# utiasASRL/mm_masking

Hardware: AMD Instinct MI355X
Metric: scan-pairs/s (mask-CNN + 10-iter dICP fwd+bwd) (higher is better)
Workload: dtype bf16; 1 GPU; BASELINE configs[2]: train_icp_weights step fwd+bwd, batch=32 per GPU, 10 dICP iters, point-to-plane Huber, dim=2; 400x3360 polar radar -> GO-CFAR + peaks + polar->Cartesian 640x640 -> U-Net (hand-written NHWC bf16 MFMA kernels, fp32 masters) -> dICP (fp32 points, fp64 normal equations) -> rot+trans+mask_pts loss -> Adam; batch_per_gpu=32, global_batch=32, scan_pts_pad=5120, map_pts=20000, map_pts_pad=20480, icp_iters=10, parallelism=dp1, scene_density=survey (SURVEY.md 8d: 3 500-5 000 valid scan points of 5 120)

## Files before the change

### include/mmk.h

```cpp
#ifndef MMK_H_
#define MMK_H_

#include <stddef.h>
#include <stdint.h>

#ifdef __cplusplus
extern "C" {
#endif

#define MMK_VERSION 502

#define MMK_OK 0
#define MMK_ERR_ARG (-1)
#define MMK_ERR_HIP (-2)
#define MMK_ERR_WORKSPACE (-3)

#define MMK_ICP_PT2PT 0
#define MMK_ICP_PT2PL 1

#define MMK_NN_BRUTE 0
#define MMK_NN_GRID 1

#define MMK_LOSS_NONE 0
#define MMK_LOSS_CAUCHY 1
// ... 36 lines not shown
                     void *workspace, size_t workspace_bytes, void *stream);

size_t mmk_icp_backward_points_workspace_bytes(const mmk_icp_params *p, int32_t with_target);
int mmk_icp_backward_points(const mmk_icp_params *p, const float *source, const float *target,
                            const float *weight, const int32_t *idx_hist, const float *T_hist,
                            const double *delta_hist, const double *A_hist,
                            const int32_t *active_hist, const float *grad_T ,
                            float *grad_weight , float *grad_T_init ,
                            float *grad_source , float *grad_target ,
                            void *workspace, size_t workspace_bytes, void *stream);

#define MMK_ICP_STATUS_UNARMED_KEY 1
int mmk_icp_status(const mmk_icp_params *p, const void *workspace, size_t workspace_bytes,
                   int32_t *status_out, void *stream);

size_t mmk_icp_partials_count(const mmk_icp_params *p);
int mmk_icp_accumulate(const mmk_icp_params *p, const float *source, const float *target,
                       const float *weight , const float *T ,
                       const uint64_t *nn_keys , int32_t *idx_out , double *partials,
                       int32_t *status , void *stream);
int mmk_icp_solve_update(const mmk_icp_params *p, const double *partials, const float *T_in ,
                         float *T_out , double *delta_out , double *A_out ,
                         const int32_t *active_in , int32_t *active_out , void *stream);

int32_t mmk_nn_padded_m(int32_t M);
int mmk_pack_target(const float *target , int32_t B, int32_t M,
                    int32_t tgt_cols, int32_t dim, float *target_planar, void *stream);
size_t mmk_nn_workspace_bytes(int32_t B, int32_t N, int32_t M, int32_t dim);
int mmk_nn_search(const float *source , const float *target_planar,
                  const float *T , int32_t B, int32_t N, int32_t M, int32_t dim,
                  int32_t *idx, float *d2, void *workspace, size_t workspace_bytes,
                  void *stream);

int mmk_nn_profile_begin(int32_t capacity);
int mmk_nn_profile_end(float *ms_out , int32_t max_out, int32_t *n_out );

int mmk_pose_loss_fwd(const float *T_pred , int32_t B, float *out2, void *stream);
int mmk_pose_loss_bwd(const float *T_pred, int32_t B, const float *g_rot, const float *g_trans,
                      float *grad_T , void *stream);
size_t mmk_bce_ws_bytes(void);
int mmk_bce_mean_fwd(const float *x, const float *target, int64_t n, void *ws, size_t ws_bytes,
                     float *out, void *stream);
int mmk_bce_mean_bwd(const float *x, const float *target, int64_t n, const float *grad_out,
                     float *grad_x, void *stream);

int mmk_pose_loss_gt_fwd(const float *T_pred , const float *T_gt , int32_t B, float *out2, void *stream);
int mmk_pose_loss_gt_bwd(const float *T_pred, const float *T_gt, int32_t B, const float *g_rot, const float *g_trans,
                         float *grad_T , void *stream);
int mmk_val_metric(const float *T_pred , const float *T_gt , int32_t B, float *out3, void *stream);
size_t mmk_fft_threshold_ws_bytes(int32_t B);
int mmk_fft_threshold_mask(const float *fft, int32_t B, int64_t hw, void *ws, size_t ws_bytes, float *mask_out,
                           void *stream);
int mmk_bce_fft_threshold_fwd(const float *x, const float *fft, int32_t B, int64_t hw, void *ws, size_t ws_bytes,
                              float *thr_out , float *out, void *stream);
int mmk_bce_fft_threshold_bwd(const float *x, const float *fft, int32_t B, int64_t hw, const float *thr ,
                              const float *grad_out, float *grad_x, void *stream);


int mmk_cfar_mask(const float *raw, int32_t B, int32_t A, int32_t R, int32_t w2,
                  int32_t guard, int32_t mincol, int32_t maxcol, float a_thresh,
                  float b_thresh, int32_t diff, float steep_fact, float *mask,
                  void *stream);

int mmk_cfar_mask_bwd(const float *raw, const float *grad_mask , int32_t B, int32_t A, int32_t R, int32_t w2,
                      int32_t guard, int32_t mincol, int32_t maxcol, float a_thresh, float b_thresh, float steep_fact,
                      float *grad_raw , void *stream);

int mmk_cfar_mask_p(const float *raw, int32_t B, int32_t A, int32_t R, int32_t w2, int32_t guard, int32_t mincol,
                    int32_t maxcol, const float *a_thresh, const float *b_thresh, int32_t per_scan, int32_t diff,
                    float steep_fact, float *mask, void *stream);

size_t mmk_cfar_mask_bwd_p_ws_bytes(int32_t B, int32_t A);
int mmk_cfar_mask_bwd_p(const float *raw, const float *grad_mask , int32_t B, int32_t A, int32_t R, int32_t w2,
                        int32_t guard, int32_t mincol, int32_t maxcol, const float *a_thresh, const float *b_thresh,
                        int32_t per_scan, float steep_fact, float *grad_raw , float *grad_a,
                        float *grad_b , void *workspace, size_t workspace_bytes, void *stream);

size_t mmk_extract_peaks_workspace_bytes(int32_t B, int32_t A, int32_t R, int32_t max_pts);
int mmk_extract_peaks(const float *mask, int32_t B, int32_t A, int32_t R, float res,
                      const float *azimuths , const float *times ,
                      const float *T_ab, int32_t diff, float steep_fact, int32_t max_pts,
                      float *out_pc, int32_t *out_count, void *workspace,
                      size_t workspace_bytes, void *stream);
size_t mmk_extract_peaks_bwd_workspace_bytes(int32_t B, int32_t A, int32_t R, int32_t max_pts);
int mmk_extract_peaks_bwd(const float *mask, int32_t B, int32_t A, int32_t R, float res, const float *azimuths ,
                          const float *T_ab, int32_t diff, float steep_fact, int32_t max_pts,
                          const float *grad_pc , float *grad_mask , void *workspace,
                          size_t workspace_bytes, void *stream);

int mmk_polar_to_cart(const float *polar, const float *azimuths ,
                      const float *range_grid, const float *angle_grid, int32_t B,
                      int32_t A, int32_t R, int32_t W, float radar_resolution,
                      int32_t interpolate_crossover, int32_t fix_wobble, float *cart,
                      void *stream);
int mmk_polar_to_cart_pair(const float *polar, const float *polar2, const float *azimuths,
                           const float *range_grid, const float *angle_grid, int32_t B, int32_t A,
                           int32_t R, int32_t W, float radar_resolution, int32_t interpolate_crossover,
                           int32_t fix_wobble, float *cart, float *cart2, void *stream);

int mmk_cart_to_polar(const double *cart, const double *sin_az, const double *cos_az, const double *range_coords,
                      int32_t B, int32_t A, int32_t R, int32_t H, int32_t W, double cart_resolution, double *polar,
                      void *stream);

size_t mmk_polar_to_cart_bwd_ws_bytes(int32_t B, int32_t A, int32_t R, int32_t W);
int mmk_polar_to_cart_bwd(const float *grad_cart , const float *azimuths , const float *range_grid,
                          const float *angle_grid, int32_t B, int32_t A, int32_t R, int32_t W, float radar_resolution,
                          int32_t interpolate_crossover, int32_t fix_wobble, float *grad_polar , void *ws,
                          size_t ws_bytes, void *stream);

size_t mmk_cart_to_polar_bwd_ws_bytes(int32_t B, int32_t A, int32_t R, int32_t H, int32_t W);
int mmk_cart_to_polar_bwd(const double *grad_polar , const double *sin_az, const double *cos_az,
                          const double *range_coords, int32_t B, int32_t A, int32_t R, int32_t H, int32_t W,
                          double radar_resolution, double cart_resolution, double *grad_cart , void *ws,
                          size_t ws_bytes, void *stream);

int mmk_mask_polar_scan(const float *scan , const float *mask_cart , const double *sin_az,
                        const double *cos_az, const double *range_coords, int32_t B, int32_t A, int32_t R, int32_t H,
                        int32_t W, double cart_resolution, float *out , void *stream);

size_t mmk_mask_polar_scan_bwd_ws_bytes(int32_t B, int32_t A, int32_t R, int32_t H, int32_t W);
int mmk_mask_polar_scan_bwd(const float *grad_out , const float *scan , const float *mask_cart ,
                            const double *sin_az, const double *cos_az, const double *range_coords, int32_t B, int32_t A,
                            int32_t R, int32_t H, int32_t W, double radar_resolution, double cart_resolution,
                            float *grad_scan , float *grad_mask , void *ws, size_t ws_bytes,
                            void *stream);

int mmk_sample_weights_fwd(const float *mask , const float *pc ,
                           int32_t B, int32_t N, int32_t pc_cols, int32_t H, int32_t W,
                           int32_t cart_pixel_width, float cart_resolution,
                           float *weights , void *stream);
size_t mmk_sample_weights_bwd_ws_bytes(int32_t B, int32_t N);
int mmk_sample_weights_bwd(const float *grad_weights , const float *pc, int32_t B,
                           int32_t N, int32_t pc_cols, int32_t H, int32_t W,
                           int32_t cart_pixel_width, float cart_resolution, float *grad_mask,
                           void *ws, size_t ws_bytes, void *stream);
int mmk_sample_weights_bwd_pc(const float *grad_weights , const float *mask , const float *pc,
                              int32_t B, int32_t N, int32_t pc_cols, int32_t H, int32_t W,
                              int32_t cart_pixel_width, float cart_resolution, float *grad_pc, void *stream);

int mmk_host_read_rows(const char *path, int64_t header_bytes, int32_t rows, int32_t row_bytes, int32_t col0,
                       int32_t ncols, int32_t roll, void *dst);
typedef struct mmk_read_job {
    const char *path;
    int64_t header_bytes;
    int32_t rows, row_bytes, col0, ncols, roll, reserved;
    void *dst;
} mmk_read_job;
int mmk_host_read_rows_batch(const mmk_read_job *jobs, int32_t n_jobs, int32_t threads);
int mmk_u8_to_float(const void *in , const float *lut256, int64_t n, float *out, void *stream);

int mmk_weight_stats(const float *weights , const float *pc , int32_t B, int32_t N,
                     int32_t pc_cols, float *partial, float *out, void *stream);

int mmk_bev_raster(const float *pc , int32_t B, int32_t M, int32_t pc_cols,
                   int32_t W, float cart_resolution, float *bev , void *stream);

typedef struct {
    const void *x1;
    const void *x2;
    int32_t C1, C2;
    const void *wpack;
    const float *bias;
    void *y1;
    const void *relu_src1;
    int32_t O1, accumulate1;
    float scale1;
// ... 121 lines not shown
```

### mm_masking_amd/_lib.py

```python
import ctypes
import os
import sys
import subprocess

import torch

_HERE = os.path.dirname(os.path.abspath(__file__))
_ROOT = os.path.dirname(_HERE)
SO_PATH = os.environ.get("MMK_LIB", os.path.join(_HERE, "libmmk_hip.so"))
SOURCES = ["mmk_api.hip", "mmk_icp.hip", "mmk_radar.hip", "mmk_unet.hip", "mmk_unet_driver.hip", "mmk_loader.hip", "mmk_loss.hip"]

_lib = None

c_f32p = ctypes.c_void_p
c_vp = ctypes.c_void_p


class MmkError(RuntimeError):
    pass


class ReadJob(ctypes.Structure):
    _fields_ = [("path", ctypes.c_char_p), ("header_bytes", ctypes.c_int64), ("rows", ctypes.c_int32),
                ("row_bytes", ctypes.c_int32), ("col0", ctypes.c_int32), ("ncols", ctypes.c_int32), ("roll", ctypes.c_int32),
# ... 79 lines not shown
    P = ctypes.POINTER(IcpParams)
    sig = {
        "mmk_version": (ctypes.c_int, []),
        "mmk_last_error": (ctypes.c_char_p, []),
        "mmk_icp_workspace_bytes": (sz, [P]),
        "mmk_icp_forward": (ctypes.c_int, [P] + [c_vp] * 10 + [c_vp, sz, ctypes.POINTER(ctypes.c_int), c_vp]),
        "mmk_icp_backward": (ctypes.c_int, [P] + [c_vp] * 11 + [c_vp, sz, c_vp]),
        "mmk_icp_backward_points_workspace_bytes": (sz, [P, i32]),
        "mmk_icp_backward_points": (ctypes.c_int, [P] + [c_vp] * 13 + [c_vp, sz, c_vp]),
        "mmk_icp_status": (ctypes.c_int, [P, c_vp, sz, c_vp, c_vp]),
        "mmk_pose_loss_fwd": (ctypes.c_int, [c_vp, i32, c_vp, c_vp]),
        "mmk_pose_loss_bwd": (ctypes.c_int, [c_vp, i32, c_vp, c_vp, c_vp, c_vp]),
        "mmk_bce_ws_bytes": (sz, []),
        "mmk_bce_mean_fwd": (ctypes.c_int, [c_vp, c_vp, ctypes.c_int64, c_vp, sz, c_vp, c_vp]),
        "mmk_bce_mean_bwd": (ctypes.c_int, [c_vp, c_vp, ctypes.c_int64, c_vp, c_vp, c_vp]),
        "mmk_pose_loss_gt_fwd": (ctypes.c_int, [c_vp, c_vp, i32, c_vp, c_vp]),
        "mmk_pose_loss_gt_bwd": (ctypes.c_int, [c_vp, c_vp, i32, c_vp, c_vp, c_vp, c_vp]),
        "mmk_val_metric": (ctypes.c_int, [c_vp, c_vp, i32, c_vp, c_vp]),
        "mmk_fft_threshold_ws_bytes": (sz, [i32]),
        "mmk_fft_threshold_mask": (ctypes.c_int, [c_vp, i32, ctypes.c_int64, c_vp, sz, c_vp, c_vp]),
        "mmk_bce_fft_threshold_fwd": (ctypes.c_int, [c_vp, c_vp, i32, ctypes.c_int64, c_vp, sz, c_vp, c_vp, c_vp]),
        "mmk_bce_fft_threshold_bwd": (ctypes.c_int, [c_vp, c_vp, i32, ctypes.c_int64, c_vp, c_vp, c_vp, c_vp]),
        "mmk_icp_partials_count": (sz, [P]),
        "mmk_icp_accumulate": (ctypes.c_int, [P] + [c_vp] * 8 + [c_vp]),
        "mmk_icp_solve_update": (ctypes.c_int, [P] + [c_vp] * 7 + [c_vp]),
        "mmk_nn_padded_m": (i32, [i32]),
        "mmk_pack_target": (ctypes.c_int, [c_vp, i32, i32, i32, i32, c_vp, c_vp]),
        "mmk_nn_workspace_bytes": (sz, [i32, i32, i32, i32]),
        "mmk_nn_search": (ctypes.c_int, [c_vp, c_vp, c_vp, i32, i32, i32, i32, c_vp, c_vp, c_vp, sz, c_vp]),
        "mmk_nn_profile_begin": (ctypes.c_int, [i32]),
        "mmk_nn_profile_end": (ctypes.c_int, [ctypes.POINTER(ctypes.c_float), i32, ctypes.POINTER(ctypes.c_int32)]),
        "mmk_conv3x3_packed_elems": (sz, [i32, i32, i32]),
        "mmk_conv3x3_pack_weights": (ctypes.c_int, [c_vp, i32, i32, i32, c_vp, c_vp]),
        "mmk_conv3x3_pack_weights_batch": (ctypes.c_int, [i32, c_vp, c_vp, c_vp, i32, c_vp, c_vp]),
        "mmk_conv3x3": (ctypes.c_int, [ctypes.POINTER(ConvDesc), c_vp]),
        "mmk_conv3x3_wgrad_unpack_batch": (ctypes.c_int, [i32, c_vp, c_vp, c_vp, c_vp, c_vp, c_vp, c_vp]),
        "mmk_conv3x3_wgrad_slices": (i32, [i32, i32, i32, i32, i32, i32]),
        "mmk_conv3x3_wgrad_partial": (ctypes.c_int, [c_vp, c_vp, i32, i32, c_vp, i32, i32, i32, i32, c_vp, i32, c_vp]),
        "mmk_conv_bwd_fused": (ctypes.c_int, [c_vp, c_vp, c_vp, ctypes.c_float, i32, i32, i32, i32, c_vp, c_vp, i32, c_vp]),
        "mmk_conv8x16_bwd_fused": (ctypes.c_int, [c_vp, c_vp, c_vp, ctypes.c_float, i32, i32, i32, c_vp, c_vp, i32, c_vp]),
        "mmk_conv16x8_bwd_fused": (ctypes.c_int, [c_vp, c_vp, c_vp, c_vp, ctypes.c_float, i32, i32, i32, c_vp, c_vp, c_vp, i32, c_vp]),
        "mmk_conv3x3_pool_fusable": (ctypes.c_int32, [i32, i32, i32, i32, i32]),
        "mmk_channel_minmax": (ctypes.c_int, [c_vp, i32, i32, ctypes.c_int64, c_vp, c_vp, c_vp, c_vp]),
        "mmk_channel_meanstd": (ctypes.c_int, [c_vp, i32, i32, ctypes.c_int64, c_vp, c_vp, c_vp]),
        "mmk_conv_first": (ctypes.c_int, [c_vp, i32, c_vp, c_vp, c_vp, i32, i32, i32, f32, c_vp, c_vp]),
        "mmk_conv_first_wgrad_ws_bytes": (sz, [i32]),
        "mmk_conv_first_wgrad": (ctypes.c_int, [c_vp, i32, c_vp, c_vp, i32, i32, i32, c_vp, c_vp, c_vp, sz, c_vp]),
        "mmk_conv_first_dgrad_ws_bytes": (sz, [i32]),
        "mmk_conv_first_dgrad": (ctypes.c_int, [c_vp, i32, c_vp, c_vp, c_vp, c_vp, i32, i32, i32, c_vp, c_vp, sz, c_vp]),
        "mmk_input_norm_bwd": (ctypes.c_int, [c_vp, c_vp, i32, c_vp, c_vp, i32, i32, i32, i32, c_vp, sz, c_vp]),
        "mmk_maxpool2_fwd": (ctypes.c_int, [c_vp, i32, i32, i32, i32, c_vp, c_vp]),
        "mmk_maxpool2_bwd": (ctypes.c_int, [c_vp, c_vp, i32, i32, i32, i32, f32, f32, c_vp, c_vp]),
        "mmk_maxpool2_fwd_arg": (ctypes.c_int, [c_vp, i32, i32, i32, i32, c_vp, c_vp, c_vp]),
        "mmk_maxpool2_bwd_arg": (ctypes.c_int, [c_vp, c_vp, i32, i32, i32, i32, f32, c_vp, c_vp]),
        "mmk_upsample_fwd": (ctypes.c_int, [c_vp, i32, i32, i32, i32, i32, i32, c_vp, c_vp]),
        "mmk_upsample_bwd": (ctypes.c_int, [c_vp, i32, i32, i32, i32, i32, i32, c_vp, f32, f32, c_vp, c_vp]),
        "mmk_final_fwd": (ctypes.c_int, [c_vp, c_vp, c_vp, ctypes.c_int64, c_vp, c_vp]),
        "mmk_final_bwd": (ctypes.c_int, [c_vp, c_vp, c_vp, c_vp, ctypes.c_int64, f32, f32, c_vp, c_vp, c_vp, c_vp, c_vp]),
        "mmk_mask_normalize": (ctypes.c_int, [c_vp, i32, ctypes.c_int64, c_vp, c_vp, c_vp, c_vp]),
        "mmk_final_bwd_normalized": (ctypes.c_int, [c_vp, c_vp, c_vp, c_vp, c_vp, c_vp, i32, ctypes.c_int64, f32, f32, c_vp, c_vp,
                                                    c_vp, c_vp, c_vp, c_vp, c_vp]),
        "mmk_bn_forward_stats": (ctypes.c_int, [c_vp, ctypes.c_int64, i32, c_vp, c_vp, f32, f32, c_vp, c_vp, c_vp, c_vp, c_vp, c_vp]),
        "mmk_bn_apply": (ctypes.c_int, [c_vp, ctypes.c_int64, i32, c_vp, f32, ctypes.c_uint32, c_vp, c_vp]),
        "mmk_bn_backward": (ctypes.c_int, [c_vp, c_vp, f32, c_vp, ctypes.c_int64, i32, c_vp, c_vp, c_vp, f32, i32, c_vp, c_vp, c_vp,
                                           c_vp, c_vp, c_vp]),
        "mmk_unet_workspace_bytes": (sz, [i32, i32, i32, i32]),
        "mmk_unet_scratch_bytes": (sz, [i32, i32, i32, i32]),
        "mmk_unet_forward": (ctypes.c_int, [ctypes.POINTER(UNetDesc), c_vp]),
        "mmk_unet_backward": (ctypes.c_int, [ctypes.POINTER(UNetDesc), c_vp, ctypes.POINTER(ctypes.c_void_p), c_vp, sz, c_vp]),
        "mmk_unet_backward_buckets": (ctypes.c_int, [ctypes.POINTER(UNetDesc), c_vp, ctypes.POINTER(ctypes.c_void_p), c_vp, sz,
                                                     ctypes.POINTER(ctypes.c_void_p), c_vp]),
        "mmk_unet_backward_input": (ctypes.c_int, [ctypes.POINTER(UNetDesc), c_vp, ctypes.POINTER(ctypes.c_void_p), c_vp, i32, c_vp,
                                                   c_vp, sz, ctypes.POINTER(ctypes.c_void_p), c_vp]),
        "mmk_unet_grad_bucket": (i32, [i32, ctypes.POINTER(i32), ctypes.POINTER(i32)]),
        "mmk_unet_tensor": (ctypes.c_int, [i32, i32, i32, i32, i32, ctypes.POINTER(sz), ctypes.POINTER(i32), ctypes.POINTER(i32),
                                           ctypes.POINTER(i32)]),
        "mmk_cfar_mask": (ctypes.c_int, [c_vp, i32, i32, i32, i32, i32, i32, i32, f32, f32, i32, f32, c_vp, c_vp]),
        "mmk_cfar_mask_bwd": (ctypes.c_int, [c_vp, c_vp, i32, i32, i32, i32, i32, i32, i32, f32, f32, f32, c_vp, c_vp]),
        "mmk_cfar_mask_p": (ctypes.c_int, [c_vp, i32, i32, i32, i32, i32, i32, i32, c_vp, c_vp, i32, i32, f32, c_vp, c_vp]),
        "mmk_cfar_mask_bwd_p_ws_bytes": (sz, [i32, i32]),
        "mmk_cfar_mask_bwd_p": (ctypes.c_int, [c_vp, c_vp, i32, i32, i32, i32, i32, i32, i32, c_vp, c_vp, i32, f32, c_vp, c_vp, c_vp,
                                               c_vp, sz, c_vp]),
        "mmk_extract_peaks_workspace_bytes": (sz, [i32, i32, i32, i32]),
        "mmk_extract_peaks_bwd_workspace_bytes": (sz, [i32, i32, i32, i32]),
        "mmk_extract_peaks_bwd": (ctypes.c_int, [c_vp, i32, i32, i32, f32, c_vp, c_vp, i32, f32, i32, c_vp, c_vp, c_vp, sz, c_vp]),
        "mmk_extract_peaks": (ctypes.c_int, [c_vp, i32, i32, i32, f32, c_vp, c_vp, c_vp, i32, f32, i32, c_vp, c_vp,
                                             c_vp, sz, c_vp]),
        "mmk_polar_to_cart": (ctypes.c_int, [c_vp, c_vp, c_vp, c_vp, i32, i32, i32, i32, f32, i32, i32, c_vp, c_vp]),
        "mmk_polar_to_cart_pair": (ctypes.c_int, [c_vp, c_vp, c_vp, c_vp, c_vp, i32, i32, i32, i32, f32, i32, i32, c_vp, c_vp,
                                                  c_vp]),
        "mmk_cart_to_polar": (ctypes.c_int, [c_vp, c_vp, c_vp, c_vp, i32, i32, i32, i32, i32, ctypes.c_double, c_vp, c_vp]),
        "mmk_polar_to_cart_bwd_ws_bytes": (sz, [i32, i32, i32, i32]),
        "mmk_polar_to_cart_bwd": (ctypes.c_int, [c_vp, c_vp, c_vp, c_vp, i32, i32, i32, i32, f32, i32, i32, c_vp, c_vp, sz, c_vp]),
        "mmk_cart_to_polar_bwd_ws_bytes": (sz, [i32, i32, i32, i32, i32]),
        "mmk_cart_to_polar_bwd": (ctypes.c_int, [c_vp, c_vp, c_vp, c_vp, i32, i32, i32, i32, i32, ctypes.c_double, ctypes.c_double,
                                                 c_vp, c_vp, sz, c_vp]),
        "mmk_mask_polar_scan": (ctypes.c_int, [c_vp, c_vp, c_vp, c_vp, c_vp, i32, i32, i32, i32, i32, ctypes.c_double, c_vp, c_vp]),
        "mmk_mask_polar_scan_bwd_ws_bytes": (sz, [i32, i32, i32, i32, i32]),
        "mmk_mask_polar_scan_bwd": (ctypes.c_int, [c_vp, c_vp, c_vp, c_vp, c_vp, c_vp, i32, i32, i32, i32, i32, ctypes.c_double,
                                                   ctypes.c_double, c_vp, c_vp, c_vp, sz, c_vp]),
        "mmk_sample_weights_fwd": (ctypes.c_int, [c_vp, c_vp, i32, i32, i32, i32, i32, i32, f32, c_vp, c_vp]),
        "mmk_host_read_rows": (ctypes.c_int, [ctypes.c_char_p, ctypes.c_int64, i32, i32, i32, i32, i32, c_vp]),
        "mmk_host_read_rows_batch": (ctypes.c_int, [ctypes.POINTER(ReadJob), i32, i32]),
        "mmk_u8_to_float": (ctypes.c_int, [c_vp, c_vp, ctypes.c_int64, c_vp, c_vp]),
        "mmk_sample_weights_bwd_ws_bytes": (sz, [i32, i32]),
        "mmk_sample_weights_bwd": (ctypes.c_int, [c_vp, c_vp, i32, i32, i32, i32, i32, i32, f32, c_vp, c_vp, sz, c_vp]),
        "mmk_sample_weights_bwd_pc": (ctypes.c_int, [c_vp, c_vp, c_vp, i32, i32, i32, i32, i32, i32, f32, c_vp, c_vp]),
        "mmk_weight_stats": (ctypes.c_int, [c_vp, c_vp, i32, i32, i32, c_vp, c_vp, c_vp]),
        "mmk_bev_raster": (ctypes.c_int, [c_vp, i32, i32, i32, i32, f32, c_vp, c_vp]),
    }
    for name, (res, args) in sig.items():
        fn = getattr(lib, name)
        fn.restype = res
        fn.argtypes = args
    return sig


EXPORTED = None


def lib():
    global _lib, EXPORTED
    if _lib is None:
        if not os.path.exists(SO_PATH):
            raise MmkError("libmmk_hip.so is not built: run `python -c 'import __graft_entry__ as g; g.build()'` "
                           "(hipcc --offload-arch=gfx950).  The HIP path has no CPU fallback.")
        try:
            loaded = ctypes.CDLL(SO_PATH)
        except OSError as e:
            raise MmkError("cannot load %s: %s" % (SO_PATH, e)) from e
        EXPORTED = _declare(loaded)
        _lib = loaded
    return _lib


def check(rc):
    if rc != 0:
        raise MmkError("libmmk_hip: %s (code %d)" % (lib().mmk_last_error().decode(errors="replace"), rc))


def stream_ptr(device=None):
    if device is not None:
        idx = device.index if isinstance(device, torch.device) else int(device)
        if idx is not None and idx != torch.cuda.current_device():
            raise MmkError("tensors live on cuda:%d but the current HIP device is cuda:%d: call torch.cuda.set_device() "
                           "(one process per GPU) or wrap the call in `with torch.cuda.device(...)`"
                           % (idx, torch.cuda.current_device()))
    return ctypes.c_void_p(torch.cuda.current_stream(device).cuda_stream)


def ptr(t, dtype=None, name="tensor"):
    if t is None:
        return ctypes.c_void_p(0)
    if not t.is_cuda:
        raise MmkError("%s must live on a HIP device (got %s); the kernels have no CPU path" % (name, t.device))
    if dtype is not None and t.dtype != dtype:
        raise MmkError("%s must be %s (got %s)" % (name, dtype, t.dtype))
    if not t.is_contiguous():
        raise MmkError("%s must be contiguous" % name)
    return ctypes.c_void_p(t.data_ptr())


def dev_f32(t, device):
    return t.detach().to(device=device, dtype=torch.float32).contiguous()
```

### mm_masking_amd/csrc/mmk_icp.hip

```cpp
#include <math.h>
#include <stdio.h>
#include <stdlib.h>

#include <algorithm>

#include "mmk_common.h"

namespace {

constexpr int NN_THREADS = 256;
constexpr int NN_TILE = 1024;
constexpr float NN_PAD = 3.0e18f;
constexpr int ACC_THREADS = 256;
constexpr int PART_ROWS = 32;

__host__ __device__ constexpr int nacc(int dim) { return dim == 2 ? 9 : 27; }
__host__ __device__ constexpr int npose(int dim) { return dim == 2 ? 6 : 12; }

template <int DIM>
__device__ __forceinline__ void transform_point(const float *T, const float s[3], float p[DIM])
{
    if constexpr (DIM == 2) {
        p[0] = (T[0] * s[0] + T[1] * s[1]) + T[3];
        p[1] = (T[4] * s[0] + T[5] * s[1]) + T[7];
    } else {
        p[0] = ((T[0] * s[0] + T[1] * s[1]) + T[2] * s[2]) + T[3];
        p[1] = ((T[4] * s[0] + T[5] * s[1]) + T[6] * s[2]) + T[7];
        p[2] = ((T[8] * s[0] + T[9] * s[1]) + T[10] * s[2]) + T[11];
    }
}

template <int DIM>
__device__ __forceinline__ float nn_dist(float tx, float ty, float tz, const float p[DIM])
{
    float dx = tx - p[0];
    float dy = ty - p[1];
    float d = __builtin_fmaf(dy, dy, dx * dx);
    if constexpr (DIM == 3) {
        float dz = tz - p[2];
        d = __builtin_fmaf(dz, dz, d);
    }
    return d;
}

__global__ void pack_target_kernel(const float *__restrict__ tgt, int M, int cols, int dim, int Mpad,
                                   float *__restrict__ out, float *__restrict__ dec, int dec_stride)
{
    int j = blockIdx.x * blockDim.x + threadIdx.x;
    int b = blockIdx.y;
    if (j >= Mpad) return;
    for (int c = 0; c < dim; ++c) {
        float v = NN_PAD;
        if (j < M) v = tgt[((size_t)b * M + j) * cols + c];
        out[((size_t)b * dim + c) * Mpad + j] = v;
        if (dec != nullptr && j % dec_stride == 0) dec[((size_t)b * dim + c) * (Mpad / dec_stride) + j / dec_stride] = v;
    }
}

constexpr int PF_CH = 32;

__global__ __launch_bounds__(NN_THREADS) void src_zero_scan_kernel(const float *__restrict__ src, int N, int pts, int nsb,
                                                                  int32_t *__restrict__ allzero, int32_t *__restrict__ zrep)
{
    const int sb = blockIdx.x, b = blockIdx.y;
    int first = N;
    int nonzero = 0;
    for (int q = threadIdx.x; q < pts; q += blockDim.x) {
        const int i = sb * pts + q;
        if (i < N) {
            const float *sp = src + ((size_t)b * N + i) * 3;
            const bool z = sp[0] == 0.f && sp[1] == 0.f && sp[2] == 0.f;
            nonzero |= z ? 0 : 1;
            if (z && i < first) first = i;
        }
    }
    const int any = __syncthreads_or(nonzero);
#pragma unroll
    for (int off = 32; off > 0; off >>= 1) first = min(first, __shfl_down(first, off, 64));
    if ((threadIdx.x & 63) == 0 && first < N) atomicMin(&zrep[b], first);
    if (threadIdx.x == 0) allzero[(size_t)b * nsb + sb] = any ? 0 : 1;
}

__global__ void src_units_kernel(const int32_t *__restrict__ allzero, const int32_t *__restrict__ zrep, int B, int nsb, int pts,
                                 int cap, int32_t *__restrict__ ulist, int32_t *__restrict__ ucnt)
{
    const int c = threadIdx.x;
    int n = 0;
// ... 540 lines not shown
template <int DIM, int TYPE>
struct PointTerms {
    static constexpr int P = (DIM == 2) ? 3 : 6;
    static constexpr int NR = (TYPE == MMK_ICP_PT2PT) ? DIM : 1;
    float s[3];
    float p[DIM];
    float ev[DIM];
    float n[DIM];
    float J[NR][P];
    float er[NR];
    float d2, r2, keep, rho, w, omega;
};

template <int DIM, int TYPE>
__device__ __forceinline__ void point_terms(PointTerms<DIM, TYPE> &t, const float *T, const float *srow,
                                            const float *trow, float omega, int loss, float k, float k2,
                                            float trim2)
{
    constexpr int P = PointTerms<DIM, TYPE>::P;
    constexpr int NR = PointTerms<DIM, TYPE>::NR;
    t.s[0] = srow[0];
    t.s[1] = srow[1];
    t.s[2] = srow[2];
    transform_point<DIM>(T, t.s, t.p);
#pragma unroll
    for (int c = 0; c < DIM; ++c) t.ev[c] = trow[c] - t.p[c];
    float d2 = t.ev[0] * t.ev[0] + t.ev[1] * t.ev[1];
    if constexpr (DIM == 3) d2 = d2 + t.ev[2] * t.ev[2];
    t.d2 = d2;
    t.keep = (d2 < trim2) ? 1.f : 0.f;
    if (TYPE == MMK_ICP_PT2PL) {
#pragma unroll
        for (int c = 0; c < DIM; ++c) t.n[c] = trow[3 + c];
        float e = t.n[0] * t.ev[0] + t.n[1] * t.ev[1];
        if constexpr (DIM == 3) e = e + t.n[2] * t.ev[2];
        t.er[0] = e;
        t.r2 = e * e;
        if (DIM == 2) {
            t.J[0][0] = t.n[0];
            t.J[0][1] = t.n[1];
            t.J[0][2] = t.n[1] * t.p[0] - t.n[0] * t.p[1];
        } else {
            t.J[0][0] = t.n[0];
            t.J[0][1] = t.n[1];
            t.J[0][2] = t.n[DIM - 1];
            t.J[0][P - 3] = t.p[1] * t.n[DIM - 1] - t.p[DIM - 1] * t.n[1];
            t.J[0][P - 2] = t.p[DIM - 1] * t.n[0] - t.p[0] * t.n[DIM - 1];
            t.J[0][P - 1] = t.p[0] * t.n[1] - t.p[1] * t.n[0];
        }
    } else {
        t.r2 = d2;
#pragma unroll
        for (int r = 0; r < NR; ++r) {
            t.er[r] = t.ev[r];
#pragma unroll
            for (int c = 0; c < P; ++c) t.J[r][c] = 0.f;
            t.J[r][r] = 1.f;
        }
        if (DIM == 2) {
            t.J[0][2] = -t.p[1];
            t.J[NR - 1][2] = t.p[0];
        } else {
            const float px = t.p[0], py = t.p[1], pz = t.p[DIM - 1];
            t.J[0][P - 2] = pz;
            t.J[0][P - 1] = -py;
            t.J[1 % NR][P - 3] = -pz;
            t.J[1 % NR][P - 1] = px;
            t.J[2 % NR][P - 3] = py;
            t.J[2 % NR][P - 2] = -px;
        }
    }
    float rho = 1.f;
    if (loss == MMK_LOSS_CAUCHY) {
        rho = 1.0f / (1.0f + t.r2 / k2);
    } else if (loss == MMK_LOSS_HUBER) {
        const float r = sqrtf(t.r2);
        rho = (r <= k) ? 1.f : k / r;
    }
    t.rho = rho;
    t.omega = omega;
    t.w = (omega * t.keep) * rho;
}

template <int DIM, int TYPE>
__global__ __launch_bounds__(ACC_THREADS) void icp_accumulate_kernel(
    const float *__restrict__ src, const float *__restrict__ tgt, int tgt_cols,
    const float *__restrict__ weight, const float *__restrict__ Tk, const int32_t *__restrict__ active,
    const unsigned long long *__restrict__ packed, unsigned long long *__restrict__ packed_next,
    const int32_t *__restrict__ allzero, const int32_t *__restrict__ zrep, int nn_pts, int nn_nsb,
    int32_t *__restrict__ idx_out, int N, int M, int loss, float k,
    float k2, float trim2, double *__restrict__ partials, int32_t *__restrict__ status)
{
    constexpr int P = PointTerms<DIM, TYPE>::P;
    constexpr int NR = PointTerms<DIM, TYPE>::NR;
    constexpr int NACC = nacc(DIM);
    const int b = blockIdx.y;
    if (active != nullptr && active[b] == 0) return;
    const int i = blockIdx.x * ACC_THREADS + threadIdx.x;
    double acc[NACC];
#pragma unroll
    for (int a = 0; a < NACC; ++a) acc[a] = 0.0;

    if (i < N) {
        float T[16];
#pragma unroll
        for (int q = 0; q < 16; ++q) T[q] = Tk[(size_t)b * 16 + q];
        int isrc = i;
        if (allzero != nullptr && allzero[(size_t)b * nn_nsb + i / nn_pts] != 0 && zrep[b] < (i / nn_pts) * nn_pts) isrc = zrep[b];
        const unsigned long long key = packed[(size_t)b * N + isrc];
        if (packed_next != nullptr) packed_next[(size_t)b * N + i] = NN_KEY_INIT;
        const unsigned jraw = (unsigned)(key & 0xffffffffull);
        if ((key == NN_KEY_INIT || jraw >= (unsigned)M) && status != nullptr) atomicOr(status, (int32_t)MMK_ICP_STATUS_UNARMED_KEY);
        const int j = (int)min(jraw, (unsigned)(M - 1));
        idx_out[(size_t)b * N + i] = j;
        const float omega = weight ? weight[(size_t)b * N + i] : 1.f;
        PointTerms<DIM, TYPE> t;
        point_terms<DIM, TYPE>(t, T, src + ((size_t)b * N + i) * 3, tgt + ((size_t)b * M + j) * tgt_cols, omega,
                               loss, k, k2, trim2);
        int a = 0;
#pragma unroll
        for (int m = 0; m < P; ++m) {
#pragma unroll
            for (int n = m; n < P; ++n) {
                double v = 0.0;
#pragma unroll
                for (int r = 0; r < NR; ++r) v += (double)(t.w * t.J[r][m]) * (double)t.J[r][n];
                acc[a++] = v;
            }
        }
#pragma unroll
        for (int m = 0; m < P; ++m) {
            double v = 0.0;
#pragma unroll
            for (int r = 0; r < NR; ++r) v += (double)(t.w * t.J[r][m]) * (double)t.er[r];
            acc[a++] = v;
        }
    }

    __shared__ double red[ACC_THREADS / 64][NACC];
    const int lane = threadIdx.x & 63, wv = threadIdx.x >> 6;
#pragma unroll
    for (int a = 0; a < NACC; ++a) {
        double v = wave_sum(acc[a]);
        if (lane == 0) red[wv][a] = v;
    }
    __syncthreads();
    if (threadIdx.x < NACC) {
        double v = 0.0;
#pragma unroll
        for (int w = 0; w < ACC_THREADS / 64; ++w) v += red[w][threadIdx.x];
        partials[((size_t)b * gridDim.x + blockIdx.x) * NACC + threadIdx.x] = v;
    }
}

template <int P>
__device__ bool chol_solve(const double *A , const double *rhs, double *x, double *ws)
{
    double (*L)[P] = reinterpret_cast<double (*)[P]>(ws);
    double *y = ws + P * P;
    bool ok = true;
    for (int i = 0; i < P; ++i)
        for (int j = 0; j < P; ++j) {
            L[i][j] = 0.0;
            if (!isfinite(A[i * P + j])) ok = false;
        }
    for (int j = 0; j < P && ok; ++j) {
        double d = A[j * P + j];
        for (int q = 0; q < j; ++q) d -= L[j][q] * L[j][q];
        if (!(d > 0.0)) {
            ok = false;
            break;
        }
        d = sqrt(d);
        L[j][j] = d;
        for (int i = j + 1; i < P; ++i) {
            double v = A[i * P + j];
            for (int q = 0; q < j; ++q) v -= L[i][q] * L[j][q];
            L[i][j] = v / d;
        }
    }
    if (!ok) {
        for (int i = 0; i < P; ++i) x[i] = 0.0;
        return false;
    }
    for (int i = 0; i < P; ++i) {
        double v = rhs[i];
        for (int q = 0; q < i; ++q) v -= L[i][q] * y[q];
        y[i] = v / L[i][i];
    }
    for (int i = P - 1; i >= 0; --i) {
        double v = y[i];
        for (int q = i + 1; q < P; ++q) v -= L[q][i] * x[q];
        x[i] = v / L[i][i];
    }
    return true;
}

template <int DIM>
__device__ void se_exp(const double *dl, double E[16])
{
    for (int i = 0; i < 16; ++i) E[i] = 0.0;
    E[0] = E[5] = E[10] = E[15] = 1.0;
    if (DIM == 2) {
        const double x = dl[0], y = dl[1], th = dl[2];
        const double th2 = th * th;
        double a, bb;
        if (th2 < 1e-8) {
            a = 1.0 - th2 / 6.0 + th2 * th2 / 120.0;
            bb = th * (0.5 - th2 / 24.0 + th2 * th2 / 720.0);
        } else {
            a = sin(th) / th;
            bb = (1.0 - cos(th)) / th;
        }
        const double c = cos(th), s = sin(th);
        E[0] = c; E[1] = -s; E[3] = a * x - bb * y;
        E[4] = s; E[5] = c;  E[7] = bb * x + a * y;
    } else {
        const double *rho = dl, *phi = dl + 3;
        const double th2 = phi[0] * phi[0] + phi[1] * phi[1] + phi[2] * phi[2];
        double A_, B_, C_;
        if (th2 < 1e-8) {
            A_ = 1.0 - th2 / 6.0 + th2 * th2 / 120.0;
            B_ = 0.5 - th2 / 24.0 + th2 * th2 / 720.0;
            C_ = 1.0 / 6.0 - th2 / 120.0 + th2 * th2 / 5040.0;
        } else {
            const double th = sqrt(th2);
            A_ = sin(th) / th;
            B_ = (1.0 - cos(th)) / th2;
            C_ = (th - sin(th)) / (th2 * th);
        }
        const double K[9] = {0.0, -phi[2], phi[1], phi[2], 0.0, -phi[0], -phi[1], phi[0], 0.0};
        double K2[9];
        for (int i = 0; i < 3; ++i)
            for (int j = 0; j < 3; ++j) {
                double v = 0.0;
                for (int q = 0; q < 3; ++q) v += K[i * 3 + q] * K[q * 3 + j];
                K2[i * 3 + j] = v;
            }
        for (int i = 0; i < 3; ++i) {
            double tv = 0.0;
            for (int j = 0; j < 3; ++j) {
                const double id = (i == j) ? 1.0 : 0.0;
                E[i * 4 + j] = id + A_ * K[i * 3 + j] + B_ * K2[i * 3 + j];
                tv += (id + B_ * K[i * 3 + j] + C_ * K2[i * 3 + j]) * rho[j];
            }
            E[i * 4 + 3] = tv;
        }
    }
}

template <int DIM>
__global__ __launch_bounds__(64) void icp_solve_kernel(const double *__restrict__ partials, int nblk,
                                                       const float *__restrict__ T_in, float *__restrict__ T_out,
                                                       double *__restrict__ delta_out, double *__restrict__ A_out,
                                                       const int32_t *__restrict__ active_in,
                                                       int32_t *__restrict__ active_out, float tol)
{
    constexpr int P = (DIM == 2) ? 3 : 6;
    constexpr int NACC = nacc(DIM);
    const int b = blockIdx.x;
    const int lane = threadIdx.x;
    __shared__ double acc[NACC];
    __shared__ double stage[PART_ROWS * NACC];
    const bool act = active_in[b] != 0;
    {
        double v = 0.0;
        if (act) {
            const double *base = partials + (size_t)b * nblk * NACC;
            for (int r0 = 0; r0 < nblk; r0 += PART_ROWS) {
                const int nr = min(PART_ROWS, nblk - r0);
                for (int e = lane; e < nr * NACC; e += 64) stage[e] = base[(size_t)r0 * NACC + e];
                __syncthreads();
                if (lane < NACC)
                    for (int q = 0; q < nr; ++q) v += stage[q * NACC + lane];
                __syncthreads();
            }
        }
        if (lane < NACC) acc[lane] = v;
    }
    __syncthreads();
    if (lane != 0) return;
    __shared__ double A[P * P], rhs[P], dl[6], E[16], ws[P * P + P];
    for (int q = 0; q < 6; ++q) dl[q] = 0.0;
    int a = 0;
    for (int m = 0; m < P; ++m)
        for (int n = m; n < P; ++n) {
            A[m * P + n] = acc[a];
            A[n * P + m] = acc[a];
            ++a;
        }
    for (int m = 0; m < P; ++m) rhs[m] = acc[a++];
    for (int q = 0; q < 36; ++q) A_out[(size_t)b * 36 + q] = (q < P * P) ? A[q] : 0.0;
    if (act) chol_solve<P>(A, rhs, dl, ws);
    for (int q = 0; q < 6; ++q) delta_out[(size_t)b * 6 + q] = dl[q];
    if (!act) {
        for (int q = 0; q < 16; ++q) T_out[(size_t)b * 16 + q] = T_in[(size_t)b * 16 + q];
        active_out[b] = 0;
        return;
    }
    se_exp<DIM>(dl, E);
    for (int i = 0; i < 4; ++i)
        for (int j = 0; j < 4; ++j) {
            double v = 0.0;
            for (int q = 0; q < 4; ++q) v += E[i * 4 + q] * (double)T_in[(size_t)b * 16 + q * 4 + j];
            T_out[(size_t)b * 16 + i * 4 + j] = (float)v;
        }
    double nrm = 0.0;
    for (int q = 0; q < P; ++q) nrm += dl[q] * dl[q];
    active_out[b] = (sqrt(nrm) < (double)tol) ? 0 : 1;
}

__global__ __launch_bounds__(256) void icp_init_kernel(unsigned long long *__restrict__ keys, size_t nkeys, int32_t *__restrict__ status,
                                                       int32_t *__restrict__ active0, const float *__restrict__ T_init,
                                                       float *__restrict__ T0, int32_t *__restrict__ zrep, int B, int N)
{
    const size_t i0 = (size_t)blockIdx.x * blockDim.x + threadIdx.x, stride = (size_t)gridDim.x * blockDim.x;
    for (size_t i = i0; i < nkeys; i += stride) keys[i] = ~0ull;
    if (i0 < 16) status[i0] = 0;
    if (i0 < (size_t)B) {
        active0[i0] = 1;
        if (zrep != nullptr) zrep[i0] = N;
    }
    if (i0 < (size_t)B * 16) T0[i0] = T_init[i0];
}

__global__ void fill_i32_kernel(int32_t *p, int n, int32_t v)
{
    int i = blockIdx.x * blockDim.x + threadIdx.x;
    if (i < n) p[i] = v;
}

template <int DIM>
__global__ __launch_bounds__(64) void icp_bwd_pair_kernel(
    const double *__restrict__ Gdir_in, const double *__restrict__ pparts, int nparts,
    const float *__restrict__ Tk, const double *__restrict__ delta, const double *__restrict__ Amat,
    const int32_t *__restrict__ active, double *__restrict__ Gdir_out, double *__restrict__ lam_out)
{
    constexpr int P = (DIM == 2) ? 3 : 6;
    constexpr int NP = npose(DIM);
    const int b = blockIdx.x;
    const int lane = threadIdx.x;
    __shared__ double G[16], Eb[16], X[16], M0[64], R0[64], R1[64];
    __shared__ double stage[PART_ROWS * NP];

    {
        double v = (lane < 16) ? Gdir_in[(size_t)b * 16 + lane] : 0.0;
        const int r = lane >> 2, c = lane & 3;
        int slot = -1;
        if (lane < 16 && r < DIM && c < DIM) slot = r * DIM + c;
        if (lane < 16 && r < DIM && c == 3) slot = DIM * DIM + r;
        const double *base = pparts + (size_t)b * nparts * NP;
        for (int r0 = 0; r0 < nparts; r0 += PART_ROWS) {
            const int nr = min(PART_ROWS, nparts - r0);
            for (int e = lane; e < nr * NP; e += 64) stage[e] = base[(size_t)r0 * NP + e];
            __syncthreads();
            if (slot >= 0)
                for (int q = 0; q < nr; ++q) v += stage[q * NP + slot];
            __syncthreads();
        }
        if (lane < 16) G[lane] = v;
    }
    __syncthreads();
    const bool act = (active != nullptr) && active[b] != 0;
    if (!act) {
        if (lane < 16) Gdir_out[(size_t)b * 16 + lane] = G[lane];
        if (lane < 6 && lam_out) lam_out[(size_t)b * 6 + lane] = 0.0;
        return;
    }
    const double *dl = delta + (size_t)b * 6;
    if (lane < 16) {
        const int r = lane >> 2, c = lane & 3;
        double v = 0.0;
        for (int q = 0; q < 4; ++q) v += G[r * 4 + q] * (double)Tk[(size_t)b * 16 + c * 4 + q];
        Eb[lane] = v;
        double x = 0.0;
        if (DIM == 2) {
            if (r == 0 && c == 3) x = dl[0];
            if (r == 1 && c == 3) x = dl[1];
            if (r == 1 && c == 0) x = dl[2];
            if (r == 0 && c == 1) x = -dl[2];
        } else {
            if (c == 3 && r < 3) x = dl[r];
            if (r == 2 && c == 1) x = dl[3];
            if (r == 1 && c == 2) x = -dl[3];
            if (r == 0 && c == 2) x = dl[4];
            if (r == 2 && c == 0) x = -dl[4];
            if (r == 1 && c == 0) x = dl[5];
            if (r == 0 && c == 1) x = -dl[5];
        }
        X[lane] = x;
    }
    __syncthreads();
    const int i8 = lane >> 3, j8 = lane & 7;
    {
        double m = 0.0;
        const double sc = 1.0 / 64.0;
        if (i8 < 4 && j8 < 4) m = X[j8 * 4 + i8] * sc;
        else if (i8 >= 4 && j8 >= 4) m = X[(j8 - 4) * 4 + (i8 - 4)] * sc;
        else if (i8 < 4 && j8 >= 4) m = Eb[i8 * 4 + (j8 - 4)] * sc;
        M0[lane] = m;
        R0[lane] = ((i8 == j8) ? 1.0 : 0.0) + m / 13.0;
    }
    __syncthreads();
    double *cur = R0, *nxt = R1;
    for (int n = 12; n >= 1; --n) {
        double v = 0.0;
#pragma unroll
        for (int q = 0; q < 8; ++q) v += M0[i8 * 8 + q] * cur[q * 8 + j8];
        nxt[lane] = ((i8 == j8) ? 1.0 : 0.0) + v / (double)n;
        __syncthreads();
        double *t = cur; cur = nxt; nxt = t;
    }
    for (int sq = 0; sq < 6; ++sq) {
        double v = 0.0;
#pragma unroll
        for (int q = 0; q < 8; ++q) v += cur[i8 * 8 + q] * cur[q * 8 + j8];
        nxt[lane] = v;
        __syncthreads();
        double *t = cur; cur = nxt; nxt = t;
    }
    if (lane < 16) {
        const int r = lane >> 2, c = lane & 3;
        double v = 0.0;
        for (int q = 0; q < 4; ++q) v += cur[r * 8 + q] * G[q * 4 + c];
        Gdir_out[(size_t)b * 16 + lane] = v;
    }
    if (lane == 0) {
        auto xb = [&](int r, int c) { return cur[r * 8 + 4 + c]; };
        __shared__ double db[P], A[P * P], lam[P], ws[P * P + P];
        if (DIM == 2) {
            db[0] = xb(0, 3);
            db[1] = xb(1, 3);
            db[2] = xb(1, 0) - xb(0, 1);
        } else {
            db[0] = xb(0, 3);
            db[1] = xb(1, 3);
            db[2] = xb(2, 3);
            db[P - 3] = xb(2, 1) - xb(1, 2);
            db[P - 2] = xb(0, 2) - xb(2, 0);
            db[P - 1] = xb(1, 0) - xb(0, 1);
        }
        for (int q = 0; q < P * P; ++q) A[q] = Amat[(size_t)b * 36 + q];
        chol_solve<P>(A, db, lam, ws);
        for (int q = 0; q < 6; ++q) lam_out[(size_t)b * 6 + q] = (q < P) ? lam[q] : 0.0;
    }
}

__host__ __device__ constexpr int tgt_row_cols(int dim, int type) { return type == MMK_ICP_PT2PL ? 2 * dim : dim; }
__host__ __device__ constexpr int tgt_acc_cols(int c) { return c <= 2 ? 2 : (c <= 4 ? 4 : 8); }

template <int DIM, int TYPE, bool PTS>
__global__ __launch_bounds__(ACC_THREADS) void icp_bwd_point_kernel(
    const float *__restrict__ src, const float *__restrict__ tgt, int tgt_cols,
    const float *__restrict__ weight, const float *__restrict__ Tk, const int32_t *__restrict__ active,
    const int32_t *__restrict__ idx, const double *__restrict__ lam64, const double *__restrict__ delta64, int N,
    int M, int loss, float k, float k2, float trim2, float *__restrict__ gw, double *__restrict__ pparts,
    float *__restrict__ gsrc, float *__restrict__ rows, unsigned *__restrict__ pmax)
{
    constexpr int P = PointTerms<DIM, TYPE>::P;
    constexpr int NR = PointTerms<DIM, TYPE>::NR;
    constexpr int NP = npose(DIM);
    constexpr int C = tgt_row_cols(DIM, TYPE);
    const int b = blockIdx.y;
    const int i = blockIdx.x * ACC_THREADS + threadIdx.x;
    double acc[NP];
#pragma unroll
    for (int a = 0; a < NP; ++a) acc[a] = 0.0;
    const bool act = active[b] != 0;
    unsigned mbits = 0u;

    if (act && i < N) {
        float T[16];
#pragma unroll
        for (int q = 0; q < 16; ++q) T[q] = Tk[(size_t)b * 16 + q];
        float lam[P], dl[P];
#pragma unroll
        for (int q = 0; q < P; ++q) {
            lam[q] = (float)lam64[(size_t)b * 6 + q];
            dl[q] = (float)delta64[(size_t)b * 6 + q];
        }
        const int j = idx[(size_t)b * N + i];
        const float omega = weight ? weight[(size_t)b * N + i] : 1.f;
        PointTerms<DIM, TYPE> t;
        point_terms<DIM, TYPE>(t, T, src + ((size_t)b * N + i) * 3, tgt + ((size_t)b * M + j) * tgt_cols, omega,
                               loss, k, k2, trim2);
        float wbar = 0.f;
        float ebar[NR];
        float Jbar[NR][P];
#pragma unroll
        for (int r = 0; r < NR; ++r) {
            float u = 0.f, v = 0.f;
#pragma unroll
            for (int c = 0; c < P; ++c) {
                u += t.J[r][c] * lam[c];
                v += t.J[r][c] * dl[c];
            }
            const float res = t.er[r] - v;
            wbar += u * res;
            ebar[r] = t.w * u;
#pragma unroll
            for (int c = 0; c < P; ++c) Jbar[r][c] = t.w * (res * lam[c] - u * dl[c]);
        }
        const float gomega = wbar * t.keep * t.rho;
        const float rhobar = wbar * t.omega * t.keep;
        float r2bar = 0.f;
        if (loss == MMK_LOSS_CAUCHY) {
            r2bar = rhobar * (-(t.rho * t.rho) / k2);
        } else if (loss == MMK_LOSS_HUBER) {
            if (sqrtf(t.r2) > k) r2bar = rhobar * (-t.rho / (2.f * t.r2));
        }
#pragma unroll
        for (int r = 0; r < NR; ++r) ebar[r] += 2.f * t.er[r] * r2bar;
        gw[(size_t)b * N + i] += gomega;

        float pbar[DIM];
#pragma unroll
        for (int c = 0; c < DIM; ++c) pbar[c] = 0.f;
        if (TYPE == MMK_ICP_PT2PT) {
#pragma unroll
            for (int c = 0; c < DIM; ++c) pbar[c] -= ebar[c % NR];
            if (DIM == 2) {
                pbar[1] -= Jbar[0][2];
                pbar[0] += Jbar[NR - 1][2];
            } else {
                pbar[DIM - 1] += Jbar[0][P - 2];
                pbar[1] -= Jbar[0][P - 1];
                pbar[DIM - 1] -= Jbar[1 % NR][P - 3];
                pbar[0] += Jbar[1 % NR][P - 1];
                pbar[1] += Jbar[2 % NR][P - 3];
                pbar[0] -= Jbar[2 % NR][P - 2];
            }
        } else {
#pragma unroll
            for (int c = 0; c < DIM; ++c) pbar[c] -= t.n[c] * ebar[0];
            if (DIM == 2) {
                pbar[0] += t.n[1] * Jbar[0][2];
                pbar[1] -= t.n[0] * Jbar[0][2];
            } else {
                const float nx = t.n[0], ny = t.n[1], nz = t.n[DIM - 1];
                const float j3 = Jbar[0][P - 3], j4 = Jbar[0][P - 2], j5 = Jbar[0][P - 1];
                pbar[0] += -nz * j4 + ny * j5;
                pbar[1] += nz * j3 - nx * j5;
                pbar[DIM - 1] += -ny * j3 + nx * j4;
            }
        }
#pragma unroll
        for (int r = 0; r < DIM; ++r) {
#pragma unroll
            for (int c = 0; c < DIM; ++c) acc[r * DIM + c] = (double)pbar[r] * (double)t.s[c];
            acc[DIM * DIM + r] = (double)pbar[r];
        }
        if constexpr (PTS) {
            if (gsrc != nullptr) {
                float *gs = gsrc + ((size_t)b * N + i) * 3;
#pragma unroll
                for (int c = 0; c < DIM; ++c) {
                    float v = T[c] * pbar[0];
#pragma unroll
                    for (int r = 1; r < DIM; ++r) v += T[r * 4 + c] * pbar[r];
                    gs[c] += v;
                }
            }
            if (rows != nullptr) {
                float q[C];
                if constexpr (TYPE == MMK_ICP_PT2PT) {
#pragma unroll
                    for (int c = 0; c < DIM; ++c) q[c] = ebar[c];
                } else {
                    const float eb = ebar[0];
#pragma unroll
                    for (int c = 0; c < DIM; ++c) {
                        q[c] = t.n[c] * eb;
                        q[DIM + c] = eb * t.ev[c] + Jbar[0][c];
                    }
                    if constexpr (DIM == 2) {
                        q[DIM + 0] -= t.p[1] * Jbar[0][2];
                        q[DIM + 1] += t.p[0] * Jbar[0][2];
                    } else {
                        const float px = t.p[0], py = t.p[1], pz = t.p[DIM - 1];
                        const float j3 = Jbar[0][P - 3], j4 = Jbar[0][P - 2], j5 = Jbar[0][P - 1];
                        q[DIM + 0] += j4 * pz - j5 * py;
                        q[DIM + 1] += j5 * px - j3 * pz;
                        q[DIM + DIM - 1] += j3 * py - j4 * px;
                    }
                }
                float *row = rows + ((size_t)b * N + i) * C;
#pragma unroll
                for (int c = 0; c < C; ++c) {
                    row[c] = q[c];
                    mbits = max(mbits, __float_as_uint(fabsf(q[c])));
                }
            }
        }
    }

    __shared__ double red[ACC_THREADS / 64][NP];
    __shared__ unsigned wmax[ACC_THREADS / 64];
    const int lane = threadIdx.x & 63, wv = threadIdx.x >> 6;
    if constexpr (PTS) {
#pragma unroll
        for (int off = 32; off > 0; off >>= 1) mbits = max(mbits, __shfl_xor(mbits, off, 64));
        if (lane == 0) wmax[wv] = mbits;
    }
#pragma unroll
    for (int a = 0; a < NP; ++a) {
        double v = wave_sum(acc[a]);
        if (lane == 0) red[wv][a] = v;
    }
    __syncthreads();
    if constexpr (PTS) {
        if (rows != nullptr && threadIdx.x == 0) {
            unsigned m = 0u;
#pragma unroll
            for (int w = 0; w < ACC_THREADS / 64; ++w) m = max(m, wmax[w]);
            if (m != 0u) atomicMax(&pmax[b], m);
        }
    }
    if (threadIdx.x < NP) {
        double v = 0.0;
#pragma unroll
        for (int w = 0; w < ACC_THREADS / 64; ++w) v += red[w][threadIdx.x];
        pparts[((size_t)b * gridDim.x + blockIdx.x) * NP + threadIdx.x] = v;
    }
}

__global__ void f32_to_f64_kernel(const float *in, double *out, int n)
{
    int i = blockIdx.x * blockDim.x + threadIdx.x;
    if (i < n) out[i] = (double)in[i];
}

template <int DIM>
__global__ void bwd_final_kernel(const double *__restrict__ Gdir, const double *__restrict__ pparts, int nparts,
                                 float *__restrict__ out)
{
    constexpr int NP = npose(DIM);
    __shared__ double stage[PART_ROWS * NP];
    const int b = blockIdx.x, lane = threadIdx.x;
    double v = (lane < 16) ? Gdir[(size_t)b * 16 + lane] : 0.0;
    const int r = lane >> 2, c = lane & 3;
    int slot = -1;
    if (lane < 16 && r < DIM && c < DIM) slot = r * DIM + c;
    if (lane < 16 && r < DIM && c == 3) slot = DIM * DIM + r;
    const double *base = pparts + (size_t)b * nparts * NP;
    for (int r0 = 0; r0 < nparts; r0 += PART_ROWS) {
        const int nr = min(PART_ROWS, nparts - r0);
        for (int e = lane; e < nr * NP; e += blockDim.x) stage[e] = base[(size_t)r0 * NP + e];
        __syncthreads();
        if (slot >= 0)
            for (int q = 0; q < nr; ++q) v += stage[q * NP + slot];
        __syncthreads();
    }
    if (lane < 16) out[(size_t)b * 16 + lane] = (float)v;
}

__device__ __forceinline__ double tgt_fixed_scale(unsigned mbits, int cnt_bits)
{
    if (mbits >= 0x7f800000u) return 0.0;
    if (mbits == 0u) return 1.0;
    return ldexp(1.0, 62 - cnt_bits - ((int)(mbits >> 23) - 126));
}

template <int C>
__global__ __launch_bounds__(ACC_THREADS) void icp_bwd_target_scatter_kernel(
    const float *__restrict__ rows, const int32_t *__restrict__ idx_hist, const int32_t *__restrict__ active_hist,
    const unsigned *__restrict__ pmax, int B, int N, int M, int cnt_bits, unsigned long long *__restrict__ acc)
{
    constexpr int L = tgt_acc_cols(C);
    const int b = blockIdx.y, k = blockIdx.z;
    const double scale = tgt_fixed_scale(pmax[b], cnt_bits);
    if (active_hist[(size_t)k * B + b] == 0 || scale == 0.0) return;
    const int t = blockIdx.x * ACC_THREADS + threadIdx.x, i = t / L, c = t % L;
    const bool valid = i < N;
    const size_t r = ((size_t)k * B + b) * N + i;
    const int j = valid ? idx_hist[r] : -1;
    long long v = 0;
    if (valid && c < C) v = llrint((double)rows[r * C + c] * scale);
    const unsigned long long vmask = __ballot(valid);
    if (vmask == 0ull) return;
    unsigned long long *ab = acc + (size_t)b * M * L;
    const int j0 = __shfl(j, __ffsll(vmask) - 1, 64);
    if (__ballot(valid && j != j0) == 0ull) {
#pragma unroll
        for (int off = 32; off >= L; off >>= 1) v += __shfl_xor(v, off, 64);
        if ((threadIdx.x & 63) < L && v != 0) atomicAdd(&ab[(size_t)j0 * L + c], (unsigned long long)v);
    } else if (v != 0) {
        atomicAdd(&ab[(size_t)j * L + c], (unsigned long long)v);
    }
}

__global__ void icp_bwd_target_final_kernel(const unsigned long long *__restrict__ acc, const unsigned *__restrict__ pmax,
                                            int cnt_bits, int M, int dim, int C, int L, int cols, float *__restrict__ gtgt)
{
    const int j = blockIdx.x * blockDim.x + threadIdx.x, b = blockIdx.y;
    if (j >= M) return;
    const double scale = tgt_fixed_scale(pmax[b], cnt_bits);
    const unsigned long long *a = acc + ((size_t)b * M + j) * L;
    float *out = gtgt + ((size_t)b * M + j) * cols;
    for (int c = 0; c < cols; ++c) {
        const int e = c < dim ? c : (C > dim && c >= 3 && c < 3 + dim ? dim + (c - 3) : -1);
        float v = 0.f;
        if (e >= 0) v = scale == 0.0 ? __builtin_nanf("") : (float)((double)(long long)a[e] / scale);
        out[c] = v;
    }
}

struct NNPlan {
    int Mpad, ntiles, nsb, ntu, tiles_per_unit, total_units, grid, P, ucap;
};


NNPlan nn_plan(int B, int N, int M, int dim)
{
    NNPlan pl;
    pl.P = 2;
    pl.Mpad = (int)mmk::align_up((size_t)M, NN_TILE);
    pl.ntiles = pl.Mpad / NN_TILE;
    pl.nsb = (N + NN_THREADS * pl.P - 1) / (NN_THREADS * pl.P);
    pl.tiles_per_unit = std::min(4, pl.ntiles);
    pl.ntu = (pl.ntiles + pl.tiles_per_unit - 1) / pl.tiles_per_unit;
    const int Bpad = (B + 7) / 8 * 8;
    pl.total_units = Bpad * pl.nsb * pl.ntu;
    pl.ucap = (Bpad / 8) * pl.nsb;
    pl.grid = std::min(pl.total_units, dim == 2 ? 1024 : 768);
    return pl;
}

struct NNProf {
    bool on = false;
    int cap = 0, n = 0;
    hipEvent_t *ev = nullptr;
};
thread_local NNProf g_prof;

int launch_nn(int dim, const float *src, const float *tgtp, const float *Tk, const int32_t *active,
              const int32_t *prev_idx, const int32_t *ulist, const int32_t *ucnt, int B, int N, const NNPlan &pl,
              unsigned long long *packed, int32_t *seed_buf, const int32_t *allzero, const int32_t *zrep, const float *dec,
              hipStream_t st)
{
    const bool rec = g_prof.on && g_prof.n < g_prof.cap;
    if (rec) MMK_CHECK_HIP(hipEventRecord(g_prof.ev[2 * g_prof.n], st));
    if (prev_idx == nullptr && seed_buf != nullptr && pl.Mpad >= 4 * NN_COARSE_STRIDE) {
        const dim3 grid((N + NN_COARSE_THREADS - 1) / NN_COARSE_THREADS, B);
        const int nn_pts = NN_THREADS * pl.P;
        if (dim == 2)
            hipLaunchKernelGGL(nn_coarse_seed_kernel<2>, grid, dim3(NN_COARSE_THREADS), 0, st, src, tgtp, Tk, active, allzero, zrep, nn_pts, pl.nsb, N,
                               pl.Mpad, dec, seed_buf);
        else
            hipLaunchKernelGGL(nn_coarse_seed_kernel<3>, grid, dim3(NN_COARSE_THREADS), 0, st, src, tgtp, Tk, active, allzero, zrep, nn_pts, pl.nsb, N,
                               pl.Mpad, dec, seed_buf);
        MMK_LAUNCH_CHECK();
        prev_idx = seed_buf;
    }
    constexpr float U = 5.9604645e-8f;
    if (dim == 2) {
        hipLaunchKernelGGL((nn_mfma_kernel<2>), dim3(pl.grid), dim3(NN_THREADS), 0, st, src, tgtp, Tk, active, prev_idx, ulist, ucnt,
                           pl.ucap, B, N, pl.Mpad, pl.nsb, pl.ntu, pl.tiles_per_unit, pl.total_units, 360.0f * U, packed);
    } else {
        hipLaunchKernelGGL((nn_mfma_kernel<3>), dim3(pl.grid), dim3(NN_THREADS), 0, st, src, tgtp, Tk, active, prev_idx, ulist, ucnt,
                           pl.ucap, B, N, pl.Mpad, pl.nsb, pl.ntu, pl.tiles_per_unit, pl.total_units, 496.0f * U, packed);
    }
    MMK_LAUNCH_CHECK();
    if (rec) {
        MMK_CHECK_HIP(hipEventRecord(g_prof.ev[2 * g_prof.n + 1], st));
        g_prof.n++;
    }
    return MMK_OK;
}

int check_params(const mmk_icp_params *p)
{
    MMK_REQUIRE(p != nullptr, "mmk_icp: params is NULL");
    MMK_REQUIRE(p->B >= 1 && p->N >= 1 && p->M >= 1, "mmk_icp: B, N, M must be >= 1 (got %d, %d, %d)", p->B, p->N, p->M);
    MMK_REQUIRE(p->dim == 2 || p->dim == 3, "mmk_icp: dim must be 2 or 3 (got %d)", p->dim);
    MMK_REQUIRE(p->tgt_cols == 3 || p->tgt_cols == 6, "mmk_icp: target must have 3 or 6 columns (got %d)", p->tgt_cols);
    MMK_REQUIRE(p->icp_type == MMK_ICP_PT2PT || p->icp_type == MMK_ICP_PT2PL, "mmk_icp: bad icp_type %d", p->icp_type);
    MMK_REQUIRE(p->icp_type != MMK_ICP_PT2PL || p->tgt_cols == 6, "mmk_icp: pt2pl needs target normals (B,M,6)");
    MMK_REQUIRE(p->loss >= MMK_LOSS_NONE && p->loss <= MMK_LOSS_HUBER, "mmk_icp: bad loss %d", p->loss);
    MMK_REQUIRE(p->max_iter >= 1, "mmk_icp: max_iter must be >= 1");
    MMK_REQUIRE(p->loss == MMK_LOSS_NONE || p->loss_k > 0.f, "mmk_icp: loss metric must be > 0");
    MMK_REQUIRE(p->nn_method == MMK_NN_BRUTE || p->nn_method == MMK_NN_GRID, "mmk_icp: bad nn_method %d", p->nn_method);
    return MMK_OK;
}

struct IcpWs {
    float *tgtp;
    unsigned long long *packed;
    int32_t *allzero, *zrep;
    int32_t *ulist, *ucnt;
    int32_t *seed0;
    float *tdec;
    double *partials;
    double *G0, *G1;
    double *lam;
    int32_t *status;
    int32_t *g_counts, *g_cursor, *g_starts;
    float4 *g_sorted;
    size_t bytes;
};

IcpWs carve(const mmk_icp_params *p, void *ws, size_t cap)
{
    const NNPlan pl = nn_plan(p->B, p->N, p->M, p->dim);
    const int nblk = (p->N + ACC_THREADS - 1) / ACC_THREADS;
    mmk::Arena ar(ws, cap);
    IcpWs w;
    w.tgtp = ar.take<float>((size_t)p->B * p->dim * pl.Mpad);
    w.packed = ar.take<unsigned long long>((size_t)2 * p->B * p->N);
    w.allzero = ar.take<int32_t>((size_t)p->B * pl.nsb);
    w.zrep = ar.take<int32_t>((size_t)p->B);
    w.ulist = ar.take<int32_t>((size_t)8 * pl.ucap);
    w.ucnt = ar.take<int32_t>(16);
    w.seed0 = ar.take<int32_t>((size_t)p->B * p->N);
    w.tdec = ar.take<float>((size_t)p->B * p->dim * (pl.Mpad / NN_COARSE_STRIDE));
    w.partials = ar.take<double>((size_t)p->B * nblk * 27);
    w.G0 = ar.take<double>((size_t)p->B * 16);
    w.G1 = ar.take<double>((size_t)p->B * 16);
    w.lam = ar.take<double>((size_t)p->B * 6);
    w.status = ar.take<int32_t>(16);
    w.g_counts = w.g_cursor = w.g_starts = nullptr;
    w.g_sorted = nullptr;
    if (p->nn_method == MMK_NN_GRID) {
        w.g_counts = ar.take<int32_t>((size_t)p->B * GRID_NC * 2);
        w.g_cursor = w.g_counts + (size_t)p->B * GRID_NC;
        w.g_starts = ar.take<int32_t>((size_t)p->B * (GRID_NC + 1));
        w.g_sorted = ar.take<float4>((size_t)p->B * p->M);
    }
    w.bytes = mmk::align_up(ar.off, 256);
    return w;
}

struct IcpPtsWs {
    float *rows;
    unsigned long long *acc;
    unsigned *pmax;
    size_t bytes;
};

IcpPtsWs carve_points(const mmk_icp_params *p, bool with_target, void *ws, size_t cap)
{
    mmk::Arena ar(ws, cap);
    ar.off = carve(p, nullptr, 0).bytes;
    IcpPtsWs w{nullptr, nullptr, nullptr, 0};
    if (with_target) {
        const int C = tgt_row_cols(p->dim, p->icp_type);
        w.rows = ar.take<float>((size_t)p->max_iter * p->B * p->N * C);
        w.acc = ar.take<unsigned long long>((size_t)p->B * p->M * tgt_acc_cols(C));
        w.pmax = ar.take<unsigned>((size_t)p->B);
    }
    w.bytes = mmk::align_up(ar.off, 256);
    return w;
}

template <int DIM, int TYPE>
int run_forward(const mmk_icp_params *p, const float *src, const float *tgt, const float *weight, float *T_hist,
                int32_t *idx_hist, double *delta_hist, double *A_hist, int32_t *active_hist, const IcpWs &w,
                int *iters_run, hipStream_t st)
{
    const int B = p->B, N = p->N, M = p->M;
    const NNPlan pl = nn_plan(B, N, M, DIM);
    const int nblk = (N + ACC_THREADS - 1) / ACC_THREADS;
    const float k = p->loss_k, k2 = p->loss_k * p->loss_k, trim2 = p->trim_dist * p->trim_dist;
    int k_done = 0;
    const bool use_grid = p->nn_method == MMK_NN_GRID;
    const int nn_pts = NN_THREADS * pl.P;
    const bool dedup = !use_grid && pl.nsb <= 0xfff && B < (1 << 19);
    if (dedup) {
        hipLaunchKernelGGL(src_zero_scan_kernel, dim3(pl.nsb, B), dim3(NN_THREADS), 0, st, src, N, nn_pts, pl.nsb, w.allzero, w.zrep);
        MMK_LAUNCH_CHECK();
        hipLaunchKernelGGL(src_units_kernel, dim3(1), dim3(64), 0, st, w.allzero, w.zrep, B, pl.nsb, nn_pts, pl.ucap, w.ulist, w.ucnt);
        MMK_LAUNCH_CHECK();
    }
    const int32_t *az = dedup ? w.allzero : nullptr, *zr = dedup ? w.zrep : nullptr;
    if (use_grid) {
        MMK_CHECK_HIP(hipMemsetAsync(w.g_counts, 0, sizeof(int32_t) * (size_t)B * GRID_NC * 2, st));
        hipLaunchKernelGGL(grid_count_kernel, dim3((M + 255) / 256, B), dim3(256), 0, st, tgt, M, p->tgt_cols, w.g_counts);
        MMK_LAUNCH_CHECK();
        hipLaunchKernelGGL(grid_scan_kernel, dim3(B), dim3(256), 0, st, w.g_counts, w.g_starts);
        MMK_LAUNCH_CHECK();
        hipLaunchKernelGGL(grid_fill_kernel, dim3((M + 255) / 256, B), dim3(256), 0, st, tgt, M, p->tgt_cols, DIM, w.g_starts,
                           w.g_cursor, w.g_sorted);
        MMK_LAUNCH_CHECK();
    }
    for (int it = 0; it < p->max_iter; ++it) {
        const float *Tk = T_hist + (size_t)it * B * 16;
        const int32_t *act = active_hist + (size_t)it * B;
        int32_t *idx = idx_hist + (p->save_state ? (size_t)it * B * N : 0);
        unsigned long long *keys = w.packed + (size_t)(it & 1) * B * N, *keys_next = w.packed + (size_t)((it + 1) & 1) * B * N;
        if (use_grid) {
            const bool rec = g_prof.on && g_prof.n < g_prof.cap;
            if (rec) MMK_CHECK_HIP(hipEventRecord(g_prof.ev[2 * g_prof.n], st));
            const int32_t *prev = (it > 0) ? idx_hist + (p->save_state ? (size_t)(it - 1) * B * N : 0) : nullptr;
            hipLaunchKernelGGL(grid_nn_kernel<DIM>, dim3((N + 255) / 256, B), dim3(256), 0, st, src, Tk, act, w.g_starts,
                               w.g_sorted, N, M, tgt, p->tgt_cols, prev, keys);
            MMK_LAUNCH_CHECK();
            if (rec) {
                MMK_CHECK_HIP(hipEventRecord(g_prof.ev[2 * g_prof.n + 1], st));
                g_prof.n++;
            }
        } else {
            const int32_t *prev = (it > 0) ? idx_hist + (p->save_state ? (size_t)(it - 1) * B * N : 0) : nullptr;
            int rc = launch_nn(DIM, src, w.tgtp, Tk, act, prev, dedup ? w.ulist : nullptr, w.ucnt, B, N, pl, keys, w.seed0, az, zr, w.tdec, st);
            if (rc != MMK_OK) return rc;
        }
        hipLaunchKernelGGL((icp_accumulate_kernel<DIM, TYPE>), dim3(nblk, B), dim3(ACC_THREADS), 0, st, src, tgt,
                           p->tgt_cols, weight, Tk, act, keys, keys_next, az, zr, nn_pts, pl.nsb, idx, N, M, p->loss, k, k2, trim2,
                           w.partials, w.status);
        MMK_LAUNCH_CHECK();
        hipLaunchKernelGGL(icp_solve_kernel<DIM>, dim3(B), dim3(64), 0, st, w.partials, nblk, Tk,
                           T_hist + (size_t)(it + 1) * B * 16, delta_hist + (size_t)it * B * 6,
                           A_hist + (size_t)it * B * 36, act, active_hist + (size_t)(it + 1) * B, p->tolerance);
        MMK_LAUNCH_CHECK();
        k_done = it + 1;
        if (p->check_every > 0 && (k_done % p->check_every) == 0 && k_done < p->max_iter) {
            static thread_local int32_t host_act[1 << 16];
            MMK_REQUIRE(B <= (1 << 16), "mmk_icp_forward: check_every needs B <= 65536");
            MMK_CHECK_HIP(hipMemcpyAsync(host_act, active_hist + (size_t)k_done * B, sizeof(int32_t) * B,
                                         hipMemcpyDeviceToHost, st));
            MMK_CHECK_HIP(hipStreamSynchronize(st));
            bool any = false;
            for (int b = 0; b < B; ++b) any = any || host_act[b] != 0;
            if (!any) break;
        }
    }
    for (int it = k_done; it < p->max_iter; ++it) {
        MMK_CHECK_HIP(hipMemcpyAsync(T_hist + (size_t)(it + 1) * B * 16, T_hist + (size_t)it * B * 16,
                                     sizeof(float) * B * 16, hipMemcpyDeviceToDevice, st));
        MMK_CHECK_HIP(hipMemsetAsync(active_hist + (size_t)(it + 1) * B, 0, sizeof(int32_t) * B, st));
        MMK_CHECK_HIP(hipMemsetAsync(delta_hist + (size_t)it * B * 6, 0, sizeof(double) * B * 6, st));
    }
    if (iters_run) *iters_run = k_done;
    return MMK_OK;
}

template <int DIM, int TYPE>
int run_backward(const mmk_icp_params *p, const float *src, const float *tgt, const float *weight,
                 const int32_t *idx_hist, const float *T_hist, const double *delta_hist, const double *A_hist,
                 const int32_t *active_hist, const float *grad_T, float *gw, float *grad_T_init, float *gsrc, float *gtgt,
                 const IcpWs &w, const IcpPtsWs &pw, hipStream_t st)
{
    const int B = p->B, N = p->N, M = p->M;
    const int nblk = (N + ACC_THREADS - 1) / ACC_THREADS;
    const float k = p->loss_k, k2 = p->loss_k * p->loss_k, trim2 = p->trim_dist * p->trim_dist;
    constexpr int C = tgt_row_cols(DIM, TYPE), L = tgt_acc_cols(C);
    MMK_CHECK_HIP(hipMemsetAsync(gw, 0, sizeof(float) * (size_t)B * N, st));
    if (gsrc) MMK_CHECK_HIP(hipMemsetAsync(gsrc, 0, sizeof(float) * (size_t)B * N * 3, st));
    if (gtgt) {
        MMK_CHECK_HIP(hipMemsetAsync(pw.acc, 0, sizeof(unsigned long long) * (size_t)B * M * L, st));
        MMK_CHECK_HIP(hipMemsetAsync(pw.pmax, 0, sizeof(unsigned) * (size_t)B, st));
    }
    hipLaunchKernelGGL(f32_to_f64_kernel, dim3((B * 16 + 255) / 256), dim3(256), 0, st, grad_T, w.G0, B * 16);
    MMK_LAUNCH_CHECK();
    double *Gin = w.G0, *Gout = w.G1;
    int nparts = 0;
    for (int it = p->max_iter - 1; it >= 0; --it) {
        const float *Tk = T_hist + (size_t)it * B * 16;
        const int32_t *act = active_hist + (size_t)it * B;
        hipLaunchKernelGGL(icp_bwd_pair_kernel<DIM>, dim3(B), dim3(64), 0, st, Gin, w.partials, nparts, Tk,
                           delta_hist + (size_t)it * B * 6, A_hist + (size_t)it * B * 36, act, Gout, w.lam);
        MMK_LAUNCH_CHECK();
        if (gsrc || gtgt)
            hipLaunchKernelGGL((icp_bwd_point_kernel<DIM, TYPE, true>), dim3(nblk, B), dim3(ACC_THREADS), 0, st, src, tgt,
                               p->tgt_cols, weight, Tk, act, idx_hist + (size_t)it * B * N, w.lam,
                               delta_hist + (size_t)it * B * 6, N, M, p->loss, k, k2, trim2, gw, w.partials, gsrc,
                               gtgt ? pw.rows + (size_t)it * B * N * C : static_cast<float *>(nullptr), pw.pmax);
        else
            hipLaunchKernelGGL((icp_bwd_point_kernel<DIM, TYPE, false>), dim3(nblk, B), dim3(ACC_THREADS), 0, st, src, tgt,
                               p->tgt_cols, weight, Tk, act, idx_hist + (size_t)it * B * N, w.lam,
                               delta_hist + (size_t)it * B * 6, N, M, p->loss, k, k2, trim2, gw, w.partials,
                               static_cast<float *>(nullptr), static_cast<float *>(nullptr), static_cast<unsigned *>(nullptr));
        MMK_LAUNCH_CHECK();
        nparts = nblk;
        double *t = Gin; Gin = Gout; Gout = t;
    }
    if (grad_T_init) {
        hipLaunchKernelGGL(bwd_final_kernel<DIM>, dim3(B), dim3(64), 0, st, Gin, w.partials, nparts, grad_T_init);
        MMK_LAUNCH_CHECK();
    }
    if (gtgt) {
        int cnt_bits = 0;
        while (((uint64_t)1 << cnt_bits) < (uint64_t)p->max_iter * (uint64_t)N) ++cnt_bits;
        const unsigned gx = (unsigned)(((size_t)N * L + ACC_THREADS - 1) / ACC_THREADS);
        hipLaunchKernelGGL(icp_bwd_target_scatter_kernel<C>, dim3(gx, B, p->max_iter), dim3(ACC_THREADS), 0, st, pw.rows, idx_hist,
                           active_hist, pw.pmax, B, N, M, cnt_bits, pw.acc);
        MMK_LAUNCH_CHECK();
        hipLaunchKernelGGL(icp_bwd_target_final_kernel, dim3((M + 255) / 256, B), dim3(256), 0, st, pw.acc, pw.pmax, cnt_bits, M, DIM, C,
                           L, p->tgt_cols, gtgt);
        MMK_LAUNCH_CHECK();
    }
    return MMK_OK;
}

int dispatch_backward(const mmk_icp_params *p, const float *src, const float *tgt, const float *weight,
                      const int32_t *idx_hist, const float *T_hist, const double *delta_hist, const double *A_hist,
                      const int32_t *active_hist, const float *grad_T, float *gw, float *grad_T_init, float *gsrc,
                      float *gtgt, const IcpWs &w, const IcpPtsWs &pw, hipStream_t st)
{
    if (p->dim == 2 && p->icp_type == MMK_ICP_PT2PT)
        return run_backward<2, MMK_ICP_PT2PT>(p, src, tgt, weight, idx_hist, T_hist, delta_hist, A_hist, active_hist, grad_T, gw,
                                              grad_T_init, gsrc, gtgt, w, pw, st);
    if (p->dim == 2)
        return run_backward<2, MMK_ICP_PT2PL>(p, src, tgt, weight, idx_hist, T_hist, delta_hist, A_hist, active_hist, grad_T, gw,
                                              grad_T_init, gsrc, gtgt, w, pw, st);
    if (p->icp_type == MMK_ICP_PT2PT)
        return run_backward<3, MMK_ICP_PT2PT>(p, src, tgt, weight, idx_hist, T_hist, delta_hist, A_hist, active_hist, grad_T, gw,
                                              grad_T_init, gsrc, gtgt, w, pw, st);
    return run_backward<3, MMK_ICP_PT2PL>(p, src, tgt, weight, idx_hist, T_hist, delta_hist, A_hist, active_hist, grad_T, gw,
                                          grad_T_init, gsrc, gtgt, w, pw, st);
}

}

extern "C" int32_t mmk_nn_padded_m(int32_t M) { return (int32_t)mmk::align_up((size_t)std::max(M, 1), NN_TILE); }

extern "C" int mmk_pack_target(const float *target, int32_t B, int32_t M, int32_t tgt_cols, int32_t dim,
                               float *target_planar, void *stream)
{
    MMK_REQUIRE(target && target_planar, "mmk_pack_target: NULL pointer");
    MMK_REQUIRE(B >= 1 && M >= 1, "mmk_pack_target: B, M must be >= 1");
    MMK_REQUIRE((dim == 2 || dim == 3) && tgt_cols >= dim, "mmk_pack_target: dim must be 2|3 and <= tgt_cols");
    const int Mpad = mmk_nn_padded_m(M);
    hipLaunchKernelGGL(pack_target_kernel, dim3(Mpad / 256, B), dim3(256), 0, (hipStream_t)stream, target, M, tgt_cols,
                       dim, Mpad, target_planar, static_cast<float *>(nullptr), 1);
    MMK_LAUNCH_CHECK();
    return MMK_OK;
}

extern "C" size_t mmk_nn_workspace_bytes(int32_t B, int32_t N, int32_t M, int32_t dim)
{
    (void)dim;
    if (B < 1 || N < 1 || M < 1) return 0;
    return mmk::align_up((size_t)B * N * sizeof(unsigned long long), 256) + mmk::align_up((size_t)B * N * sizeof(int32_t), 256) + 512;
}

extern "C" int mmk_nn_search(const float *source, const float *target_planar, const float *T, int32_t B, int32_t N,
                             int32_t M, int32_t dim, int32_t *idx, float *d2, void *workspace, size_t workspace_bytes,
                             void *stream)
{
    MMK_REQUIRE(source && target_planar && T && idx && d2, "mmk_nn_search: NULL pointer");
    MMK_REQUIRE(B >= 1 && N >= 1 && M >= 1, "mmk_nn_search: B, N, M must be >= 1");
    MMK_REQUIRE(dim == 2 || dim == 3, "mmk_nn_search: dim must be 2 or 3");
    const NNPlan pl = nn_plan(B, N, M, dim);
    mmk::Arena ar(workspace, workspace_bytes);
    unsigned long long *packed = ar.take<unsigned long long>((size_t)B * N);
    int32_t *seed0 = ar.take<int32_t>((size_t)B * N);
    if (!ar.ok() || workspace == nullptr) {
        mmk::set_error("mmk_nn_search: workspace too small (%zu < %zu)", workspace_bytes, ar.off);
        return MMK_ERR_WORKSPACE;
    }
    hipStream_t st = (hipStream_t)stream;
    MMK_CHECK_HIP(hipMemsetAsync(packed, 0xFF, sizeof(unsigned long long) * (size_t)B * N, st));
    int rc = launch_nn(dim, source, target_planar, T, nullptr, nullptr, nullptr, nullptr, B, N, pl, packed, seed0, nullptr, nullptr, nullptr, st);
    if (rc != MMK_OK) return rc;
    hipLaunchKernelGGL(nn_unpack_kernel, dim3((B * N + 255) / 256), dim3(256), 0, st, packed, B * N, idx, d2);
    MMK_LAUNCH_CHECK();
    return MMK_OK;
}

extern "C" int mmk_nn_profile_begin(int32_t capacity)
{
    MMK_REQUIRE(capacity >= 1 && capacity <= (1 << 20), "mmk_nn_profile_begin: bad capacity %d", capacity);
    if (g_prof.cap < capacity) {
        for (int i = 0; i < 2 * g_prof.cap; ++i) (void)hipEventDestroy(g_prof.ev[i]);
        delete[] g_prof.ev;
        g_prof.ev = new hipEvent_t[2 * (size_t)capacity];
        g_prof.cap = 0;
        for (int i = 0; i < 2 * capacity; ++i) MMK_CHECK_HIP(hipEventCreate(&g_prof.ev[i]));
        g_prof.cap = capacity;
    }
    g_prof.n = 0;
    g_prof.on = true;
    return MMK_OK;
}

extern "C" int mmk_nn_profile_end(float *ms_out, int32_t max_out, int32_t *n_out)
{
    MMK_REQUIRE(n_out != nullptr, "mmk_nn_profile_end: NULL n_out");
    g_prof.on = false;
    int n = g_prof.n;
    if (n > max_out) n = max_out;
    for (int i = 0; i < n; ++i) {
        MMK_CHECK_HIP(hipEventSynchronize(g_prof.ev[2 * i + 1]));
        MMK_CHECK_HIP(hipEventElapsedTime(&ms_out[i], g_prof.ev[2 * i], g_prof.ev[2 * i + 1]));
    }
    *n_out = g_prof.n;
    g_prof.n = 0;
    return MMK_OK;
}

extern "C" size_t mmk_icp_workspace_bytes(const mmk_icp_params *p)
{
    if (check_params(p) != MMK_OK) return 0;
    return carve(p, nullptr, 0).bytes;
}

extern "C" int mmk_icp_forward(const mmk_icp_params *p, const float *source, const float *target,
                               const float *weight, const float *T_init, float *T_out, int32_t *idx_hist,
                               float *T_hist, double *delta_hist, double *A_hist, int32_t *active_hist,
                               void *workspace, size_t workspace_bytes, int *iters_run, void *stream)
{
    int rc = check_params(p);
    if (rc != MMK_OK) return rc;
    MMK_REQUIRE(source && target && T_init && T_out && idx_hist && T_hist && delta_hist && A_hist && active_hist,
                "mmk_icp_forward: NULL pointer");
    const IcpWs w = carve(p, workspace, workspace_bytes);
    if (workspace == nullptr || w.bytes > workspace_bytes) {
        mmk::set_error("mmk_icp_forward: workspace too small (%zu < %zu)", workspace_bytes, w.bytes);
        return MMK_ERR_WORKSPACE;
    }
    hipStream_t st = (hipStream_t)stream;
    const int B = p->B;
    {
        const int Mpad = mmk_nn_padded_m(p->M);
        hipLaunchKernelGGL(pack_target_kernel, dim3(Mpad / 256, B), dim3(256), 0, st, target, p->M, p->tgt_cols, p->dim, Mpad, w.tgtp,
                           w.tdec, NN_COARSE_STRIDE);
        MMK_LAUNCH_CHECK();
    }
    {
        const size_t nkeys = (size_t)2 * B * p->N;
        const unsigned blocks = (unsigned)std::min<size_t>(std::max<size_t>((nkeys + 255) / 256, (size_t)(B * 16 + 255) / 256), 2048);
        hipLaunchKernelGGL(icp_init_kernel, dim3(blocks), dim3(256), 0, st, w.packed, nkeys, w.status, active_hist, T_init, T_hist, w.zrep, B,
                           p->N);
        MMK_LAUNCH_CHECK();
    }
    if (p->dim == 2 && p->icp_type == MMK_ICP_PT2PT)
        rc = run_forward<2, MMK_ICP_PT2PT>(p, source, target, weight, T_hist, idx_hist, delta_hist, A_hist, active_hist, w, iters_run, st);
    else if (p->dim == 2)
        rc = run_forward<2, MMK_ICP_PT2PL>(p, source, target, weight, T_hist, idx_hist, delta_hist, A_hist, active_hist, w, iters_run, st);
    else if (p->icp_type == MMK_ICP_PT2PT)
        rc = run_forward<3, MMK_ICP_PT2PT>(p, source, target, weight, T_hist, idx_hist, delta_hist, A_hist, active_hist, w, iters_run, st);
    else
        rc = run_forward<3, MMK_ICP_PT2PL>(p, source, target, weight, T_hist, idx_hist, delta_hist, A_hist, active_hist, w, iters_run, st);
    if (rc != MMK_OK) return rc;
    MMK_CHECK_HIP(hipMemcpyAsync(T_out, T_hist + (size_t)p->max_iter * B * 16, sizeof(float) * B * 16,
                                 hipMemcpyDeviceToDevice, st));
    return MMK_OK;
}

extern "C" int mmk_icp_status(const mmk_icp_params *p, const void *workspace, size_t workspace_bytes, int32_t *status_out,
                              void *stream)
{
    int rc = check_params(p);
    if (rc != MMK_OK) return rc;
    MMK_REQUIRE(status_out != nullptr, "mmk_icp_status: NULL status_out");
    const IcpWs w = carve(p, const_cast<void *>(workspace), workspace_bytes);
    if (workspace == nullptr || w.bytes > workspace_bytes) {
        mmk::set_error("mmk_icp_status: workspace too small (%zu < %zu)", workspace_bytes, w.bytes);
        return MMK_ERR_WORKSPACE;
    }
    MMK_CHECK_HIP(hipMemcpyAsync(status_out, w.status, sizeof(int32_t), hipMemcpyDefault, (hipStream_t)stream));
    return MMK_OK;
}

extern "C" size_t mmk_icp_partials_count(const mmk_icp_params *p)
{
    if (check_params(p) != MMK_OK) return 0;
    return (size_t)p->B * ((p->N + ACC_THREADS - 1) / ACC_THREADS) * nacc(p->dim);
}

namespace {
template <int DIM, int TYPE>
int run_accumulate(const mmk_icp_params *p, const float *src, const float *tgt, const float *weight, const float *T,
                   const unsigned long long *keys, int32_t *idx, double *partials, int32_t *status, hipStream_t st)
{
    const int nblk = (p->N + ACC_THREADS - 1) / ACC_THREADS;
    hipLaunchKernelGGL((icp_accumulate_kernel<DIM, TYPE>), dim3(nblk, p->B), dim3(ACC_THREADS), 0, st, src, tgt, p->tgt_cols, weight,
                       T, static_cast<const int32_t *>(nullptr), keys, static_cast<unsigned long long *>(nullptr),
                       static_cast<const int32_t *>(nullptr), static_cast<const int32_t *>(nullptr), 1, 1, idx, p->N, p->M, p->loss,
                       p->loss_k, p->loss_k * p->loss_k, p->trim_dist * p->trim_dist, partials, status);
    MMK_LAUNCH_CHECK();
    return MMK_OK;
}

template <int DIM>
int run_solve_update(const mmk_icp_params *p, const double *partials, const float *T_in, float *T_out, double *delta, double *A,
                     const int32_t *active_in, int32_t *active_out, hipStream_t st)
{
    const int nblk = (p->N + ACC_THREADS - 1) / ACC_THREADS;
    hipLaunchKernelGGL(icp_solve_kernel<DIM>, dim3(p->B), dim3(64), 0, st, partials, nblk, T_in, T_out, delta, A, active_in, active_out,
                       p->tolerance);
    MMK_LAUNCH_CHECK();
    return MMK_OK;
}
}

extern "C" int mmk_icp_accumulate(const mmk_icp_params *p, const float *source, const float *target, const float *weight,
                                  const float *T, const uint64_t *nn_keys, int32_t *idx_out, double *partials, int32_t *status,
                                  void *stream)
{
    int rc = check_params(p);
    if (rc != MMK_OK) return rc;
    MMK_REQUIRE(source && target && T && nn_keys && idx_out && partials && status, "mmk_icp_accumulate: NULL pointer");
    hipStream_t st = (hipStream_t)stream;
    const unsigned long long *keys = reinterpret_cast<const unsigned long long *>(nn_keys);
    if (p->dim == 2 && p->icp_type == MMK_ICP_PT2PT) return run_accumulate<2, MMK_ICP_PT2PT>(p, source, target, weight, T, keys, idx_out, partials, status, st);
    if (p->dim == 2) return run_accumulate<2, MMK_ICP_PT2PL>(p, source, target, weight, T, keys, idx_out, partials, status, st);
    if (p->icp_type == MMK_ICP_PT2PT) return run_accumulate<3, MMK_ICP_PT2PT>(p, source, target, weight, T, keys, idx_out, partials, status, st);
    return run_accumulate<3, MMK_ICP_PT2PL>(p, source, target, weight, T, keys, idx_out, partials, status, st);
}

extern "C" int mmk_icp_solve_update(const mmk_icp_params *p, const double *partials, const float *T_in, float *T_out,
                                    double *delta_out, double *A_out, const int32_t *active_in, int32_t *active_out, void *stream)
{
    int rc = check_params(p);
    if (rc != MMK_OK) return rc;
    MMK_REQUIRE(partials && T_in && T_out && delta_out && A_out && active_in && active_out, "mmk_icp_solve_update: NULL pointer");
    if (p->dim == 2) return run_solve_update<2>(p, partials, T_in, T_out, delta_out, A_out, active_in, active_out, (hipStream_t)stream);
    return run_solve_update<3>(p, partials, T_in, T_out, delta_out, A_out, active_in, active_out, (hipStream_t)stream);
}

extern "C" int mmk_icp_backward(const mmk_icp_params *p, const float *source, const float *target,
                                const float *weight, const int32_t *idx_hist, const float *T_hist,
                                const double *delta_hist, const double *A_hist, const int32_t *active_hist,
                                const float *grad_T, float *grad_weight, float *grad_T_init, void *workspace,
                                size_t workspace_bytes, void *stream)
{
    int rc = check_params(p);
    if (rc != MMK_OK) return rc;
    MMK_REQUIRE(p->save_state, "mmk_icp_backward: forward must have run with save_state = 1");
    MMK_REQUIRE(source && target && idx_hist && T_hist && delta_hist && A_hist && active_hist && grad_T && grad_weight,
                "mmk_icp_backward: NULL pointer");
    const IcpWs w = carve(p, workspace, workspace_bytes);
    if (workspace == nullptr || w.bytes > workspace_bytes) {
        mmk::set_error("mmk_icp_backward: workspace too small (%zu < %zu)", workspace_bytes, w.bytes);
        return MMK_ERR_WORKSPACE;
    }
    return dispatch_backward(p, source, target, weight, idx_hist, T_hist, delta_hist, A_hist, active_hist, grad_T, grad_weight,
                             grad_T_init, nullptr, nullptr, w, IcpPtsWs{nullptr, nullptr, nullptr, 0}, (hipStream_t)stream);
}

extern "C" size_t mmk_icp_backward_points_workspace_bytes(const mmk_icp_params *p, int32_t with_target)
{
    if (check_params(p) != MMK_OK) return 0;
    return carve_points(p, with_target != 0, nullptr, 0).bytes;
}

extern "C" int mmk_icp_backward_points(const mmk_icp_params *p, const float *source, const float *target,
                                       const float *weight, const int32_t *idx_hist, const float *T_hist,
                                       const double *delta_hist, const double *A_hist, const int32_t *active_hist,
                                       const float *grad_T, float *grad_weight, float *grad_T_init, float *grad_source,
                                       float *grad_target, void *workspace, size_t workspace_bytes, void *stream)
{
    int rc = check_params(p);
    if (rc != MMK_OK) return rc;
    MMK_REQUIRE(p->save_state, "mmk_icp_backward_points: forward must have run with save_state = 1");
    MMK_REQUIRE(source && target && idx_hist && T_hist && delta_hist && A_hist && active_hist && grad_T && grad_weight,
                "mmk_icp_backward_points: NULL pointer");
    MMK_REQUIRE(grad_target == nullptr || p->max_iter <= 65535,
                "mmk_icp_backward_points: the target gradient needs max_iter <= 65535 (got %d)", p->max_iter);
    const IcpPtsWs pw = carve_points(p, grad_target != nullptr, workspace, workspace_bytes);
    MMK_REQUIRE(workspace != nullptr && pw.bytes <= workspace_bytes, "mmk_icp_backward_points: workspace too small (%zu < %zu bytes)",
                workspace_bytes, pw.bytes);
// ... 5 lines not shown
```

### mm_masking_amd/csrc/mmk_radar.hip

```cpp
#include <math.h>

#include "mmk_common.h"

namespace {

constexpr int RT = 256;

template <int NTHR = RT>
__device__ __forceinline__ double block_excl_scan(double v, double *sm, double *total)
{
    const int lane = threadIdx.x & 63, wv = threadIdx.x >> 6;
    double inc = v;
#pragma unroll
    for (int off = 1; off < 64; off <<= 1) {
        double o = __shfl_up(inc, off, 64);
        if (lane >= off) inc += o;
    }
    if (lane == 63) sm[wv] = inc;
    __syncthreads();
    double base = 0.0, tot = 0.0;
#pragma unroll
    for (int w = 0; w < NTHR / 64; ++w) {
        if (w < wv) base += sm[w];
        tot += sm[w];
    }
    __syncthreads();
    *total = tot;
    return base + inc - v;
}

__device__ __forceinline__ int block_excl_scan_i(int v, int *sm, int *total)
{
    const int lane = threadIdx.x & 63, wv = threadIdx.x >> 6;
    int inc = v;
#pragma unroll
    for (int off = 1; off < 64; off <<= 1) {
        int o = __shfl_up(inc, off, 64);
        if (lane >= off) inc += o;
    }
    if (lane == 63) sm[wv] = inc;
    __syncthreads();
    int base = 0, tot = 0;
#pragma unroll
    for (int w = 0; w < RT / 64; ++w) {
        if (w < wv) base += sm[w];
        tot += sm[w];
    }
    __syncthreads();
    *total = tot;
    return base + inc - v;
}

constexpr int CFAR_T = 512;

struct CfarThVal {
    static constexpr bool per_row = false, params = false;
    float a, b;
    __device__ __forceinline__ int scan_of(int) const { return 0; }
    __device__ __forceinline__ float a_of(int) const { return a; }
    __device__ __forceinline__ float b_of(int) const { return b; }
};
struct CfarThPtr {
    static constexpr bool per_row = true, params = true;
    const float *a, *b;
    int stride, A;
    double *part;
    __device__ __forceinline__ int scan_of(int row) const { return row / A; }
    __device__ __forceinline__ float a_of(int scan) const { return a[scan * stride]; }
    __device__ __forceinline__ float b_of(int scan) const { return b[scan * stride]; }
};

template <class TH>
__global__ __launch_bounds__(CFAR_T) void cfar_mask_kernel(const float *__restrict__ raw, int R, int w2, int guard,
                                                       int mincol, int maxcol, TH thr, int diff,
                                                       float steep, float *__restrict__ mask)
{
    const float a_th = thr.a_of(blockIdx.y), b_th = thr.b_of(blockIdx.y);
    extern __shared__ __attribute__((aligned(16))) unsigned char smem[];
    double *cs = reinterpret_cast<double *>(smem);
    float *row = reinterpret_cast<float *>(cs + (R + 1));
    __shared__ double wsum[CFAR_T / 64];
    const size_t base = ((size_t)blockIdx.y * gridDim.x + blockIdx.x) * R;
    for (int c = threadIdx.x; c < R; c += CFAR_T) row[c] = raw[base + c];
    __syncthreads();
    const int L = (R + CFAR_T - 1) / CFAR_T;
    const int c0 = min(R, (int)threadIdx.x * L), c1 = min(R, c0 + L);
    double s = 0.0;
    for (int c = c0; c < c1; ++c) s += (double)row[c];
    double tot;
    double run = block_excl_scan<CFAR_T>(s, wsum, &tot);
    for (int c = c0; c < c1; ++c) {
        cs[c] = run;
        run += (double)row[c];
    }
    if (threadIdx.x == CFAR_T - 1) cs[R] = tot;
    __syncthreads();
    auto cell = [&](int c) -> float {
        float th = 1000.0f;
        if (c >= mincol && c < maxcol) {
            const float left = (float)(cs[c - guard] - cs[c - w2 - guard]);
            const float right = (float)(cs[min(R, c + w2 + guard + 1)] - cs[min(R, c + guard + 1)]);
            const float stat = fmaxf(left, right) / (float)w2;
            th = a_th * stat + b_th;
        }
        const float x = row[c];
        float m;
        if (diff) {
            m = 0.5f * tanhf(steep * (x - th) + 2.5f) + 0.5f;
            m = (fabsf(m) > 0.99f) ? m : 0.0f;
        } else {
            m = (x > th) ? 1.0f : 0.0f;
        }
        return m;
    };
    for (int c = threadIdx.x; c < R; c += CFAR_T) mask[base + c] = cell(c);
}

template <int NPRE, class TH>
__global__ __launch_bounds__(CFAR_T) void cfar_mask_rows_kernel(const float *__restrict__ raw, int rows, int R, int w2, int guard,
                                                                int mincol, int maxcol, TH thr, int diff,
                                                                float steep, float *__restrict__ mask)
{
    extern __shared__ __attribute__((aligned(16))) unsigned char smem[];
    double *cs = reinterpret_cast<double *>(smem);
    float *row = reinterpret_cast<float *>(cs + (R + 1));
    __shared__ double wsum[CFAR_T / 64];
    float nx[NPRE];
    int r = blockIdx.x;
    if (r >= rows) return;
    auto fetch = [&](int rr) {
        const float *src = raw + (size_t)rr * R;
#pragma unroll
        for (int i = 0; i < NPRE; ++i) {
            const int c = threadIdx.x + i * CFAR_T;
            nx[i] = src[c < R ? c : R - 1];
        }
    };
    auto stage = [&]() {
#pragma unroll
        for (int i = 0; i < NPRE; ++i) {
            const int c = threadIdx.x + i * CFAR_T;
            if (c < R) row[c] = nx[i];
        }
    };
    fetch(r);
    stage();
    __syncthreads();
    const int L = (R + CFAR_T - 1) / CFAR_T;
    const int c0 = min(R, (int)threadIdx.x * L), c1 = min(R, c0 + L);
    float a_th = thr.a_of(thr.scan_of(r)), b_th = thr.b_of(thr.scan_of(r));
    while (true) {
        const int rn = r + gridDim.x;
        fetch(rn < rows ? rn : r);
        double s = 0.0;
        for (int c = c0; c < c1; ++c) s += (double)row[c];
        double tot;
        double run = block_excl_scan<CFAR_T>(s, wsum, &tot);
        for (int c = c0; c < c1; ++c) {
            cs[c] = run;
            run += (double)row[c];
        }
        if (threadIdx.x == CFAR_T - 1) cs[R] = tot;
        __syncthreads();
        float *out = mask + (size_t)r * R;
        for (int c = threadIdx.x; c < R; c += CFAR_T) {
            float th = 1000.0f;
            if (c >= mincol && c < maxcol) {
                const float left = (float)(cs[c - guard] - cs[c - w2 - guard]);
                const float right = (float)(cs[min(R, c + w2 + guard + 1)] - cs[min(R, c + guard + 1)]);
                const float stat = fmaxf(left, right) / (float)w2;
                th = a_th * stat + b_th;
            }
            const float x = row[c];
            float m;
            if (diff) {
                m = 0.5f * tanhf(steep * (x - th) + 2.5f) + 0.5f;
                m = (fabsf(m) > 0.99f) ? m : 0.0f;
            } else {
                m = (x > th) ? 1.0f : 0.0f;
            }
            out[c] = m;
        }
        if (rn >= rows) break;
        __syncthreads();
        stage();
        __syncthreads();
        r = rn;
        if (TH::per_row) {
            a_th = thr.a_of(thr.scan_of(r));
            b_th = thr.b_of(thr.scan_of(r));
        }
    }
}

__device__ __forceinline__ float peak_value(const float *__restrict__ mrow, int j, int R, float res, int diff,
                                            float steep)
{
    const float a0 = (res * (float)j) * mrow[j];
    const float a1 = (res * (float)(j + 1)) * mrow[j + 1];
    float z0, z1;
    if (diff) {
        z0 = 1.0f - tanhf(steep * a0);
        z1 = 1.0f - tanhf(steep * a1);
    } else {
        z0 = (a0 == 0.0f) ? 1.0f : 0.0f;
        z1 = (a1 == 0.0f) ? 1.0f : 0.0f;
    }
    return a0 * z1 + a1 * z0;
}

__device__ __forceinline__ const float *stage_row(const float *__restrict__ grow, int R, float *lrow)
{
    if ((R & 3) == 0 && ((uintptr_t)grow & 15) == 0) {
        for (int c = threadIdx.x * 4; c < R; c += RT * 4) *reinterpret_cast<float4 *>(lrow + c) = *reinterpret_cast<const float4 *>(grow + c);
    } else {
        for (int c = threadIdx.x; c < R; c += RT) lrow[c] = grow[c];
    }
    __syncthreads();
    return lrow;
}

__global__ __launch_bounds__(RT) void peaks_count_kernel(const float *__restrict__ mask, int R, float res, int diff,
                                                         float steep, int32_t *__restrict__ row_count)
{
    extern __shared__ __attribute__((aligned(16))) float lrow_dyn[];
    __shared__ int sm[RT / 64];
    const int rowid = blockIdx.y * gridDim.x + blockIdx.x;
    const float *mrow = stage_row(mask + (size_t)rowid * R, R, lrow_dyn);
    int cnt = 0;
    for (int j = threadIdx.x; j < R - 1; j += RT) cnt += (peak_value(mrow, j, R, res, diff, steep) != 0.0f) ? 1 : 0;
    int tot;
    block_excl_scan_i(cnt, sm, &tot);
    if (threadIdx.x == 0) row_count[rowid] = tot;
}

__global__ __launch_bounds__(RT) void peaks_scan_kernel(const int32_t *__restrict__ row_count, int A,
                                                        int32_t *__restrict__ row_off, int32_t *__restrict__ total)
{
    __shared__ int sm[RT / 64];
    const int b = blockIdx.x;
    const int L = (A + RT - 1) / RT;
    const int a0 = min(A, (int)threadIdx.x * L), a1 = min(A, a0 + L);
    int s = 0;
    for (int a = a0; a < a1; ++a) s += row_count[b * A + a];
    int tot;
    int run = block_excl_scan_i(s, sm, &tot);
    for (int a = a0; a < a1; ++a) {
        row_off[b * A + a] = run;
        run += row_count[b * A + a];
    }
    if (threadIdx.x == 0) total[b] = tot;
}

__global__ __launch_bounds__(RT) void peaks_emit_kernel(const float *__restrict__ mask, int R, float res, int diff,
                                                        float steep, const int32_t *__restrict__ row_off, int cap,
                                                        float *__restrict__ mval, int32_t *__restrict__ mrow_out)
{
    extern __shared__ __attribute__((aligned(16))) float lrow_dyn[];
    __shared__ int sm[RT / 64];
    const int a = blockIdx.x, b = blockIdx.y, A = gridDim.x;
    const int rowid = b * A + a;
    const float *mrow = stage_row(mask + (size_t)rowid * R, R, lrow_dyn);
    const int L = (R - 1 + RT - 1) / RT;
    const int j0 = min(R - 1, (int)threadIdx.x * L), j1 = min(R - 1, j0 + L);
    int cnt = 0;
    for (int j = j0; j < j1; ++j) cnt += (peak_value(mrow, j, R, res, diff, steep) != 0.0f) ? 1 : 0;
    int tot;
    int g = row_off[rowid] + block_excl_scan_i(cnt, sm, &tot);
    if (cnt != 0) {
        for (int j = j0; j < j1; ++j) {
            const float v = peak_value(mrow, j, R, res, diff, steep);
            if (v != 0.0f) {
                if (g < cap) {
                    mval[(size_t)b * cap + g] = v;
                    mrow_out[(size_t)b * cap + g] = a;
                }
                ++g;
            }
        }
    }
}

__global__ void peaks_pair_kernel(const float *__restrict__ mval, const int32_t *__restrict__ mrow, int cap,
                                  const int32_t *__restrict__ total, const float *__restrict__ az,
                                  const float *__restrict__ T_ab, int A, int max_pts, float *__restrict__ out_pc,
                                  int32_t *__restrict__ out_count)
{
    const int k = blockIdx.x * blockDim.x + threadIdx.x;
    const int b = blockIdx.y;
    const int npts = total[b] / 2;
    if (k == 0) out_count[b] = npts;
    if (k >= max_pts) return;
    float x = 0.f, y = 0.f, z = 0.f;
    if (k < npts && 2 * k + 1 < cap) {
        const size_t m = (size_t)b * cap + 2 * k;
        const float rho = (mval[m + 1] + mval[m]) / 2.0f;
        const float phi = (az[b * A + mrow[m + 1]] + az[b * A + mrow[m]]) / 2.0f;
        x = rho * cosf(phi);
        y = rho * sinf(phi);
        if (T_ab) {
            const float *T = T_ab + (size_t)b * 16;
            const float xx = ((T[0] * x + T[1] * y) + T[2] * z) + T[3];
            const float yy = ((T[4] * x + T[5] * y) + T[6] * z) + T[7];
            const float zz = ((T[8] * x + T[9] * y) + T[10] * z) + T[11];
            x = xx; y = yy; z = zz;
        }
    }
    float *o = out_pc + ((size_t)b * max_pts + k) * 3;
    o[0] = x; o[1] = y; o[2] = z;
}

__device__ __forceinline__ float tap_polar(const float *__restrict__ img, int A, int R, int yi, int xi, int wrap)
{
    const int rows = wrap ? A + 2 : A;
    if (xi < 0 || xi >= R || yi < 0 || yi >= rows) return 0.0f;
    int r = yi;
    if (wrap) r = (yi == 0) ? (A - 1) : ((yi == A + 1) ? 0 : yi - 1);
    return img[(size_t)r * R + xi];
}

struct CartTaps {
    int xi, yi;
    double wx, wy;
    bool inimg;
};

__device__ __forceinline__ CartTaps cart_taps(double s_az, double c_az, double rc, int H, int W, double cart_resolution)
{
    const double sx = s_az * rc, sy = c_az * rc;
    double u = sx / cart_resolution, v = -sy / cart_resolution;
    u = u / (double)(W - 1) * 2.0;
    v = v / (double)(H - 1) * 2.0;
    const double ix = ((u + 1.0) / 2.0) * (double)(W - 1), iy = ((v + 1.0) / 2.0) * (double)(H - 1);
    const double x0 = floor(ix), y0 = floor(iy);
    CartTaps t;
    t.wx = ix - x0;
    t.wy = iy - y0;
    t.xi = (int)fmin(fmax(x0, -2.0), (double)W);
    t.yi = (int)fmin(fmax(y0, -2.0), (double)H);
    t.inimg = t.xi >= -1 && t.xi < W && t.yi >= -1 && t.yi < H;
    return t;
}

template <typename T>
__device__ __forceinline__ double cart_blend(const T *__restrict__ img, const CartTaps &t, int H, int W)
{
    const double ex = 1.0 - t.wx, sy1 = 1.0 - t.wy;
    auto tap = [&](int y, int x) -> double {
        return (x >= 0 && x < W && y >= 0 && y < H) ? (double)img[(size_t)y * W + x] : 0.0;
    };
    const double t0 = tap(t.yi, t.xi), t1 = tap(t.yi, t.xi + 1), t2 = tap(t.yi + 1, t.xi), t3 = tap(t.yi + 1, t.xi + 1);
    return fma(t3, t.wy * t.wx, fma(t2, t.wy * ex, fma(t1, sy1 * t.wx, t0 * (sy1 * ex))));
}

__global__ __launch_bounds__(256) void cart_to_polar_kernel(const double *__restrict__ cart, const double *__restrict__ sin_az,
                                                            const double *__restrict__ cos_az, const double *__restrict__ range_coords,
                                                            int A, int R, int H, int W, double cart_resolution,
                                                            double *__restrict__ polar)
{
    const int r = blockIdx.x * blockDim.x + threadIdx.x;
    if (r >= R) return;
// ... 745 lines not shown

__global__ __launch_bounds__(256) void mask_polar_scan_bwd_kernel(const float *__restrict__ gout, const float *__restrict__ scan,
                                                                  const float *__restrict__ mask, const double *__restrict__ sin_az,
                                                                  const double *__restrict__ cos_az,
                                                                  const double *__restrict__ range_coords, int A, int R, int H, int W,
                                                                  double cart_resolution, float *__restrict__ grad_scan,
                                                                  const unsigned *__restrict__ pmax, int cnt_bits,
                                                                  unsigned long long *__restrict__ acc)
{
    const int r = blockIdx.x * blockDim.x + threadIdx.x;
    const int a = blockIdx.y, b = blockIdx.z;
    const bool valid = r < R;
    const CartTaps t = cart_taps(sin_az[(size_t)b * A + a], cos_az[(size_t)b * A + a], range_coords[valid ? r : R - 1], H, W,
                                 cart_resolution);
    const size_t cell = ((size_t)b * A + a) * R + (valid ? r : R - 1);
    const float go = gout[cell];
    if (grad_scan != nullptr && valid) grad_scan[cell] = go * (float)cart_blend(mask + (size_t)b * H * W, t, H, W);
    if (acc == nullptr) return;
    const double scale = fixed_scale<double>(pmax[b], cnt_bits);
    if (scale == 0.0) return;
    const double g = (valid && t.inimg) ? (double)(go * scan[cell]) : 0.0;
    cart_scatter_cell(g, valid, t, H, W, scale, acc + (size_t)b * H * W);
}

__global__ __launch_bounds__(256) void mask_polar_scan_final_kernel(const unsigned long long *__restrict__ acc,
                                                                    const unsigned *__restrict__ pmax, int cnt_bits, size_t n,
                                                                    float *__restrict__ out)
{
    const int b = blockIdx.y;
    const double scale = fixed_scale<double>(pmax[b], cnt_bits);
    for (size_t i = (size_t)blockIdx.x * 256 + threadIdx.x; i < n; i += (size_t)gridDim.x * 256) {
        const long long a = (long long)acc[(size_t)b * n + i];
        out[(size_t)b * n + i] = scale == 0.0 ? __builtin_nanf("") : (float)((double)a / scale);
    }
}

int ceil_log2(double x)
{
    int bits = 0;
    while (bits < 62 && (double)(1ull << bits) < x) ++bits;
    return bits;
}

struct ResampleBwdWs {
    unsigned *pmax;
    unsigned long long *acc;
    size_t bytes;
};

ResampleBwdWs carve_resample_bwd(int B, size_t acc_words, void *ws, size_t cap_bytes)
{
    mmk::Arena ar(ws, cap_bytes);
    ResampleBwdWs w;
    w.pmax = ar.take<unsigned>((size_t)B);
    w.acc = ar.take<unsigned long long>(acc_words);
    w.bytes = mmk::align_up(ar.off, 256);
    return w;
}

inline int stream_blocks(size_t n) { return (int)std::min<size_t>((n + 2047) / 2048, 2048); }

}

extern "C" int mmk_cfar_mask(const float *raw, int32_t B, int32_t A, int32_t R, int32_t w2, int32_t guard,
                             int32_t mincol, int32_t maxcol, float a_thresh, float b_thresh, int32_t diff,
                             float steep_fact, float *mask, void *stream)
{
    MMK_REQUIRE(raw && mask, "mmk_cfar_mask: NULL pointer");
    MMK_REQUIRE(B >= 1 && A >= 1 && R >= 1, "mmk_cfar_mask: raw_scans must be 3D with non-empty dims");
    MMK_REQUIRE(w2 >= 1 && guard >= 0, "mmk_cfar_mask: bad window (w2=%d guard=%d)", w2, guard);
    MMK_REQUIRE(mincol >= w2 + guard && maxcol <= R, "mmk_cfar_mask: column range [%d,%d) outside the row", mincol, maxcol);
    const size_t smem = (size_t)(R + 1) * sizeof(double) + (size_t)R * sizeof(float);
    MMK_REQUIRE(smem <= 160 * 1024 - 64, "mmk_cfar_mask: R=%d does not fit the 160 KB LDS row buffer", R);
    if (smem > 64 * 1024)
        MMK_CHECK_HIP(hipFuncSetAttribute((const void *)cfar_mask_kernel<CfarThVal>, hipFuncAttributeMaxDynamicSharedMemorySize, (int)smem));
    const int rows = A * B;
    if (R <= 8 * CFAR_T && smem <= 40 * 1024) {
        int dev = 0, cus = 256;
        if (hipGetDevice(&dev) == hipSuccess) {
            int v = 0;
            if (hipDeviceGetAttribute(&v, hipDeviceAttributeMultiprocessorCount, dev) == hipSuccess && v > 0) cus = v;
        }
        const int grid = std::min(rows, 4 * cus);
        hipLaunchKernelGGL((cfar_mask_rows_kernel<8, CfarThVal>), dim3(grid), dim3(CFAR_T), smem, (hipStream_t)stream, raw, rows, R, w2,
                           guard, mincol, maxcol, CfarThVal{a_thresh, b_thresh}, diff, steep_fact, mask);
    } else {
        hipLaunchKernelGGL(cfar_mask_kernel<CfarThVal>, dim3(A, B), dim3(CFAR_T), smem, (hipStream_t)stream, raw, R, w2, guard, mincol,
                           maxcol, CfarThVal{a_thresh, b_thresh}, diff, steep_fact, mask);
    }
    MMK_LAUNCH_CHECK();
    return MMK_OK;
}

extern "C" int mmk_cfar_mask_p(const float *raw, int32_t B, int32_t A, int32_t R, int32_t w2, int32_t guard, int32_t mincol,
                               int32_t maxcol, const float *a_thresh, const float *b_thresh, int32_t per_scan, int32_t diff,
                               float steep_fact, float *mask, void *stream)
{
    MMK_REQUIRE(raw && mask, "mmk_cfar_mask_p: NULL pointer");
    MMK_REQUIRE(a_thresh && b_thresh, "mmk_cfar_mask_p: NULL threshold pointer");
    MMK_REQUIRE(B >= 1 && A >= 1 && R >= 1, "mmk_cfar_mask_p: raw_scans must be 3D with non-empty dims");
    MMK_REQUIRE(w2 >= 1 && guard >= 0, "mmk_cfar_mask_p: bad window (w2=%d guard=%d)", w2, guard);
    MMK_REQUIRE(mincol >= w2 + guard && maxcol <= R, "mmk_cfar_mask_p: column range [%d,%d) outside the row", mincol, maxcol);
    const size_t smem = (size_t)(R + 1) * sizeof(double) + (size_t)R * sizeof(float);
    MMK_REQUIRE(smem <= 160 * 1024 - 64, "mmk_cfar_mask_p: R=%d does not fit the 160 KB LDS row buffer", R);
    if (smem > 64 * 1024)
        MMK_CHECK_HIP(hipFuncSetAttribute((const void *)cfar_mask_kernel<CfarThPtr>, hipFuncAttributeMaxDynamicSharedMemorySize, (int)smem));
    const CfarThPtr thr{a_thresh, b_thresh, per_scan ? 1 : 0, A, nullptr};
    const int rows = A * B;
    if (R <= 8 * CFAR_T && smem <= 40 * 1024) {
        int dev = 0, cus = 256;
        if (hipGetDevice(&dev) == hipSuccess) {
            int v = 0;
            if (hipDeviceGetAttribute(&v, hipDeviceAttributeMultiprocessorCount, dev) == hipSuccess && v > 0) cus = v;
        }
        const int grid = std::min(rows, 4 * cus);
        hipLaunchKernelGGL((cfar_mask_rows_kernel<8, CfarThPtr>), dim3(grid), dim3(CFAR_T), smem, (hipStream_t)stream, raw, rows, R, w2, guard,
                           mincol, maxcol, thr, diff, steep_fact, mask);
    } else {
        hipLaunchKernelGGL(cfar_mask_kernel<CfarThPtr>, dim3(A, B), dim3(CFAR_T), smem, (hipStream_t)stream, raw, R, w2, guard, mincol,
                           maxcol, thr, diff, steep_fact, mask);
    }
    MMK_LAUNCH_CHECK();
    return MMK_OK;
}

extern "C" size_t mmk_cfar_mask_bwd_p_ws_bytes(int32_t B, int32_t A)
{
    if (B < 1 || A < 1) return 0;
    return mmk::align_up((size_t)B * A * 2 * sizeof(double), 256);
}

extern "C" int mmk_cfar_mask_bwd_p(const float *raw, const float *grad_mask, int32_t B, int32_t A, int32_t R, int32_t w2,
                                   int32_t guard, int32_t mincol, int32_t maxcol, const float *a_thresh, const float *b_thresh,
                                   int32_t per_scan, float steep_fact, float *grad_raw, float *grad_a, float *grad_b,
                                   void *workspace, size_t workspace_bytes, void *stream)
{
    MMK_REQUIRE(raw && grad_mask && grad_a && grad_b, "mmk_cfar_mask_bwd_p: NULL pointer");
    MMK_REQUIRE(a_thresh && b_thresh, "mmk_cfar_mask_bwd_p: NULL threshold pointer");
    MMK_REQUIRE(B >= 1 && A >= 1 && R >= 1, "mmk_cfar_mask_bwd_p: raw_scans must be 3D with non-empty dims");
    MMK_REQUIRE(w2 >= 1 && guard >= 0, "mmk_cfar_mask_bwd_p: bad window (w2=%d guard=%d)", w2, guard);
    MMK_REQUIRE(mincol >= w2 + guard && maxcol <= R, "mmk_cfar_mask_bwd_p: column range [%d,%d) outside the row", mincol, maxcol);
    const size_t smem = (size_t)(R + 1) * sizeof(double) + (size_t)R * sizeof(float);
    MMK_REQUIRE(smem <= 160 * 1024 - 64, "mmk_cfar_mask_bwd_p: R=%d does not fit the 160 KB LDS row buffer", R);
    const size_t need = mmk_cfar_mask_bwd_p_ws_bytes(B, A);
    if (workspace == nullptr || need > workspace_bytes) {
        mmk::set_error("mmk_cfar_mask_bwd_p: workspace too small (%zu < %zu)", workspace_bytes, need);
        return MMK_ERR_WORKSPACE;
    }
    hipStream_t st = (hipStream_t)stream;
    double *part = static_cast<double *>(workspace);
    const CfarThPtr thr{a_thresh, b_thresh, per_scan ? 1 : 0, A, part};
    if (R <= 8 * CFAR_T) {
        hipLaunchKernelGGL((cfar_mask_bwd_kernel<8, CfarThPtr>), dim3(A, B), dim3(CFAR_T), smem, st, raw, grad_mask, R, w2, guard, mincol,
                           maxcol, thr, steep_fact, grad_raw);
    } else {
        constexpr int NLONG = 27;
        if (smem > 64 * 1024)
            MMK_CHECK_HIP(hipFuncSetAttribute((const void *)(cfar_mask_bwd_kernel<NLONG, CfarThPtr>), hipFuncAttributeMaxDynamicSharedMemorySize,
                                              (int)smem));
        hipLaunchKernelGGL((cfar_mask_bwd_kernel<NLONG, CfarThPtr>), dim3(A, B), dim3(CFAR_T), smem, st, raw, grad_mask, R, w2, guard,
                           mincol, maxcol, thr, steep_fact, grad_raw);
    }
    MMK_LAUNCH_CHECK();
    hipLaunchKernelGGL(cfar_param_sum_kernel, dim3(per_scan ? B : 1), dim3(RT), 0, st, part, per_scan ? A : A * B, grad_a, grad_b);
    MMK_LAUNCH_CHECK();
    return MMK_OK;
}

extern "C" size_t mmk_extract_peaks_workspace_bytes(int32_t B, int32_t A, int32_t R, int32_t max_pts)
{
    (void)R;
    if (B < 1 || A < 1 || max_pts < 1) return 0;
    return carve_peaks(B, A, max_pts, nullptr, 0).bytes;
}

extern "C" int mmk_extract_peaks(const float *mask, int32_t B, int32_t A, int32_t R, float res, const float *azimuths,
                                 const float *times, const float *T_ab, int32_t diff, float steep_fact,
                                 int32_t max_pts, float *out_pc, int32_t *out_count, void *workspace,
                                 size_t workspace_bytes, void *stream)
{
    (void)times;
    MMK_REQUIRE(mask && azimuths && out_pc && out_count, "mmk_extract_peaks: NULL pointer");
    MMK_REQUIRE(B >= 1 && A >= 1 && R >= 2 && max_pts >= 1, "mmk_extract_peaks: bad shape");
    const PeakWs w = carve_peaks(B, A, max_pts, workspace, workspace_bytes);
    if (workspace == nullptr || w.bytes > workspace_bytes) {
        mmk::set_error("mmk_extract_peaks: workspace too small (%zu < %zu)", workspace_bytes, w.bytes);
        return MMK_ERR_WORKSPACE;
    }
    hipStream_t st = (hipStream_t)stream;
    const size_t row_lds = (size_t)R * sizeof(float);
    MMK_REQUIRE(row_lds <= 64 * 1024 - 64, "mmk_extract_peaks: R=%d does not fit the LDS row buffer", R);
    hipLaunchKernelGGL(peaks_count_kernel, dim3(A, B), dim3(RT), row_lds, st, mask, R, res, diff, steep_fact, w.row_count);
    MMK_LAUNCH_CHECK();
    hipLaunchKernelGGL(peaks_scan_kernel, dim3(B), dim3(RT), 0, st, w.row_count, A, w.row_off, w.total);
    MMK_LAUNCH_CHECK();
    hipLaunchKernelGGL(peaks_emit_kernel, dim3(A, B), dim3(RT), row_lds, st, mask, R, res, diff, steep_fact, w.row_off, w.cap,
                       w.mval, w.mrow);
    MMK_LAUNCH_CHECK();
    hipLaunchKernelGGL(peaks_pair_kernel, dim3((max_pts + 255) / 256, B), dim3(256), 0, st, w.mval, w.mrow, w.cap,
                       w.total, azimuths, T_ab, A, max_pts, out_pc, out_count);
    MMK_LAUNCH_CHECK();
    return MMK_OK;
}

extern "C" int mmk_cfar_mask_bwd(const float *raw, const float *grad_mask, int32_t B, int32_t A, int32_t R, int32_t w2,
                                 int32_t guard, int32_t mincol, int32_t maxcol, float a_thresh, float b_thresh,
                                 float steep_fact, float *grad_raw, void *stream)
{
    MMK_REQUIRE(raw && grad_mask && grad_raw, "mmk_cfar_mask_bwd: NULL pointer");
    MMK_REQUIRE(B >= 1 && A >= 1 && R >= 1, "mmk_cfar_mask_bwd: raw_scans must be 3D with non-empty dims");
    MMK_REQUIRE(w2 >= 1 && guard >= 0, "mmk_cfar_mask_bwd: bad window (w2=%d guard=%d)", w2, guard);
    MMK_REQUIRE(mincol >= w2 + guard && maxcol <= R, "mmk_cfar_mask_bwd: column range [%d,%d) outside the row", mincol, maxcol);
    const size_t smem = (size_t)(R + 1) * sizeof(double) + (size_t)R * sizeof(float);
    MMK_REQUIRE(smem <= 160 * 1024 - 64, "mmk_cfar_mask_bwd: R=%d does not fit the 160 KB LDS row buffer", R);
    hipStream_t st = (hipStream_t)stream;
    if (R <= 8 * CFAR_T) {
        hipLaunchKernelGGL((cfar_mask_bwd_kernel<8, CfarThVal>), dim3(A, B), dim3(CFAR_T), smem, st, raw, grad_mask, R, w2, guard, mincol,
                           maxcol, CfarThVal{a_thresh, b_thresh}, steep_fact, grad_raw);
    } else {
        constexpr int NLONG = 27;
        static_assert((size_t)NLONG * CFAR_T * 12 >= 160 * 1024, "cfar_mask_bwd_kernel<NLONG> must hold every row the LDS admits");
        if (smem > 64 * 1024)
            MMK_CHECK_HIP(hipFuncSetAttribute((const void *)(cfar_mask_bwd_kernel<NLONG, CfarThVal>), hipFuncAttributeMaxDynamicSharedMemorySize,
                                              (int)smem));
        hipLaunchKernelGGL((cfar_mask_bwd_kernel<NLONG, CfarThVal>), dim3(A, B), dim3(CFAR_T), smem, st, raw, grad_mask, R, w2, guard,
                           mincol, maxcol, CfarThVal{a_thresh, b_thresh}, steep_fact, grad_raw);
    }
    MMK_LAUNCH_CHECK();
    return MMK_OK;
}

extern "C" size_t mmk_extract_peaks_bwd_workspace_bytes(int32_t B, int32_t A, int32_t R, int32_t max_pts)
{
    (void)R;
    if (B < 1 || A < 1 || max_pts < 1) return 0;
    return carve_peaks_bwd(B, A, max_pts, nullptr, 0).bytes;
}

extern "C" int mmk_extract_peaks_bwd(const float *mask, int32_t B, int32_t A, int32_t R, float res, const float *azimuths,
                                     const float *T_ab, int32_t diff, float steep_fact, int32_t max_pts, const float *grad_pc,
                                     float *grad_mask, void *workspace, size_t workspace_bytes, void *stream)
{
    MMK_REQUIRE(mask && azimuths && grad_pc && grad_mask, "mmk_extract_peaks_bwd: NULL pointer");
    MMK_REQUIRE(B >= 1 && A >= 1 && R >= 2 && max_pts >= 1, "mmk_extract_peaks_bwd: bad shape");
    const PeakBwdWs w = carve_peaks_bwd(B, A, max_pts, workspace, workspace_bytes);
    if (workspace == nullptr || w.bytes > workspace_bytes) {
        mmk::set_error("mmk_extract_peaks_bwd: workspace too small (%zu < %zu)", workspace_bytes, w.bytes);
        return MMK_ERR_WORKSPACE;
    }
    hipStream_t st = (hipStream_t)stream;
    const size_t row_lds = (size_t)R * sizeof(float);
    MMK_REQUIRE(row_lds <= 64 * 1024 - 64, "mmk_extract_peaks_bwd: R=%d does not fit the LDS row buffer", R);
    if (2 * row_lds > 64 * 1024)
        MMK_CHECK_HIP(hipFuncSetAttribute((const void *)peaks_bwd_rows_kernel, hipFuncAttributeMaxDynamicSharedMemorySize,
                                          (int)(2 * row_lds)));
    hipLaunchKernelGGL(peaks_count_kernel, dim3(A, B), dim3(RT), row_lds, st, mask, R, res, diff, steep_fact, w.f.row_count);
    MMK_LAUNCH_CHECK();
    hipLaunchKernelGGL(peaks_scan_kernel, dim3(B), dim3(RT), 0, st, w.f.row_count, A, w.f.row_off, w.f.total);
    MMK_LAUNCH_CHECK();
    hipLaunchKernelGGL(peaks_emit_kernel, dim3(A, B), dim3(RT), row_lds, st, mask, R, res, diff, steep_fact, w.f.row_off, w.f.cap,
                       w.f.mval, w.f.mrow);
    MMK_LAUNCH_CHECK();
    hipLaunchKernelGGL(peaks_bwd_points_kernel, dim3((max_pts + 255) / 256, B), dim3(256), 0, st, w.f.mrow, w.f.cap, w.f.total,
                       azimuths, T_ab, A, max_pts, grad_pc, w.gv);
    MMK_LAUNCH_CHECK();
    hipLaunchKernelGGL(peaks_bwd_rows_kernel, dim3(A, B), dim3(RT), 2 * row_lds, st, mask, R, res, diff, steep_fact, w.f.row_off,
                       w.f.cap, w.gv, grad_mask);
    MMK_LAUNCH_CHECK();
    return MMK_OK;
}

extern "C" int mmk_polar_to_cart(const float *polar, const float *azimuths, const float *range_grid,
                                 const float *angle_grid, int32_t B, int32_t A, int32_t R, int32_t W,
                                 float radar_resolution, int32_t interpolate_crossover, int32_t fix_wobble, float *cart,
                                 void *stream)
{
    MMK_REQUIRE(polar && azimuths && range_grid && angle_grid && cart, "mmk_polar_to_cart: NULL pointer");
    MMK_REQUIRE(B >= 1 && A >= 2 && R >= 2 && W >= 1, "mmk_polar_to_cart: bad shape");
    MMK_REQUIRE((size_t)A * 4 <= 64 * 1024, "mmk_polar_to_cart: too many azimuths (%d)", A);
    const float half_res = (float)((double)radar_resolution / 2.0);
    hipLaunchKernelGGL(polar_to_cart_kernel, dim3(((W + 31) / 32) * ((W + 7) / 8), B), dim3(256), (size_t)A * 4, (hipStream_t)stream,
                       polar, azimuths, range_grid, angle_grid, A, R, W, radar_resolution, half_res,
                       interpolate_crossover ? 1 : 0, fix_wobble ? 1 : 0, cart, (const float *)nullptr, (float *)nullptr);
// ... 251 lines not shown
```

### mm_masking_amd/radar_utils.py

```python
import ctypes

import numpy as np
import torch

from . import _lib

__all__ = ["load_pc_from_file", "load_radar", "cfar_mask", "extract_pc", "extract_pc_padded", "extract_weights",
           "extract_bev_from_pts", "mean_peaks_parallel_fast", "pol_2_cart", "radar_polar_to_cartesian",
           "radar_polar_to_cartesian_diff", "radar_cartesian_to_polar", "mask_polar_scan", "point_to_cart_idx",
           "form_cart_range_angle_grid", "form_polar_range_grid"]


def _hip_device(t):
    if t.is_cuda:
        return t.device
    if not torch.cuda.is_available():
        raise _lib.MmkError("radar_utils needs an MI355X/HIP device: the operators are HIP kernels with no CPU path")
    return torch.device("cuda", torch.cuda.current_device())


def _back(out, like):
    return out if like.is_cuda else out.to(like.device)


_ws_cache = {}


def _workspace(nbytes, device):
    key = (device.index, torch.cuda.current_stream(device).cuda_stream, "radar")
    buf = _ws_cache.get(key)
    if buf is None or buf.numel() < nbytes:
        buf = torch.empty(max(int(nbytes), 1), dtype=torch.uint8, device=device)
        _ws_cache[key] = buf
    return buf


def load_pc_from_file(file_path, to_type=None, to_device="cpu"):
    pc = np.fromfile(file_path, dtype=np.float32)
    pc = torch.from_numpy(pc.reshape((len(pc) // 6, 6))).to(to_device)
    return pc if to_type is None else pc.type(to_type)


def load_radar(raw_img):
    raw = np.asarray(raw_img)
    timestamps = np.frombuffer(raw[:, :8].tobytes(), dtype=np.int64) * 1000
    azimuths = np.frombuffer(raw[:, 8:10].tobytes(), dtype=np.uint16) * (2 * np.pi / 5600)
    fft_data = np.divide(raw[:, 11:], 255.0, dtype=np.float32)
    return fft_data, azimuths, timestamps


def form_cart_range_angle_grid(cart_resolution=0.2384, cart_pixel_width=640, dtype=None, device="cpu"):
    if (cart_pixel_width % 2) == 0:
        cart_min_range = (cart_pixel_width / 2 - 0.5) * cart_resolution
    else:
        cart_min_range = cart_pixel_width / 2 * cart_resolution
    kw = {} if dtype is None else {"dtype": dtype}
    coords = torch.linspace(-cart_min_range, cart_min_range, cart_pixel_width, **kw)
    Y, X = torch.meshgrid(coords, -1 * coords, indexing="xy")
    sample_range = torch.sqrt(Y * Y + X * X)
    sample_angle = torch.arctan2(Y, X)
    sample_angle = sample_angle + torch.where(sample_angle < 0, 2.0 * torch.pi, 0.0)
    return sample_range.to(device), sample_angle.to(device)


def form_polar_range_grid(polar_resolution=0.2384, polar_pixel_shape=(400, 3360), dtype=None, device="cpu"):
    polar_range = (polar_pixel_shape[1] - 1) * polar_resolution
    kw = {} if dtype is None else {"dtype": dtype}
    range_coords = torch.linspace(0.0, polar_range, polar_pixel_shape[1], **kw).to(device)
    return range_coords.unsqueeze(0).expand(polar_pixel_shape[0], -1)


_grid_cache = {}


def _device_grids(width, device):
    key = (width, device.type, device.index)
    g = _grid_cache.get(key)
    if g is None:
        r, a = form_cart_range_angle_grid(cart_pixel_width=width, dtype=torch.float32)
        g = (r.contiguous().to(device), a.contiguous().to(device))
        _grid_cache[key] = g
    return g


def point_to_cart_idx(pc, cart_resolution=0.2384, cart_pixel_width=640, min_to_plus_1=False):
    grid_pc_u = -pc[:, :, 0] / cart_resolution
    grid_pc_v = pc[:, :, 1] / cart_resolution
    if min_to_plus_1:
        grid_pc = torch.stack((grid_pc_v, grid_pc_u), axis=2)
        return grid_pc / (cart_pixel_width - 1) * 2
# ... 232 lines not shown
        for need, like, val in zip(ctx.needs_input_grad[:3], ctx.like, (gx, ga, gb)):
            if not need:
                grads.append(None)
                continue
            dtype, device, shape = like
            if val.numel() != int(np.prod(shape)):
                val = val.sum()
            grads.append(val.reshape(shape).to(device=device, dtype=dtype))
        return tuple(grads) + (None,) * 4


def cfar_mask(raw_scans, res, width=101, minr=2.0, maxr=80.0, guard=5,
              a_thresh=1.0, b_thresh=0.09, diff=True, steep_fact=10.0):
    assert raw_scans.ndim == 3, "raw_scans must be 3D"
    tensors = torch.is_tensor(a_thresh) or torch.is_tensor(b_thresh)
    n = _cfar_threshold_sizes(a_thresh, b_thresh, raw_scans.shape[0]) if tensors else 0
    dev = _hip_device(raw_scans)
    w2, mincol, maxcol = cfar_cols(raw_scans.shape[2], res, width, minr, maxr, guard)
    if tensors:
        if diff and torch.is_grad_enabled() and any(torch.is_tensor(t) and t.requires_grad for t in (raw_scans, a_thresh, b_thresh)):
            return _CfarMaskP.apply(raw_scans, a_thresh, b_thresh, dev, (w2, guard, mincol, maxcol), steep_fact, n)
        x = _lib.dev_f32(raw_scans, dev)
        a, b = _cfar_threshold_dev(a_thresh, n, dev), _cfar_threshold_dev(b_thresh, n, dev)
        return _back(_cfar_forward_p(x, w2, guard, mincol, maxcol, a, b, diff, steep_fact), raw_scans)
    if diff and torch.is_grad_enabled() and raw_scans.requires_grad:
        return _CfarMask.apply(raw_scans, dev, (w2, guard, mincol, maxcol), a_thresh, b_thresh, steep_fact)
    x = _lib.dev_f32(raw_scans, dev)
    return _back(_cfar_forward(x, w2, guard, mincol, maxcol, a_thresh, b_thresh, diff, steep_fact), raw_scans)


def _peaks_forward(m, res, az, tm, Tab, diff, steep_fact, max_pts):
    B, A, R = m.shape
    dev = m.device
    L = _lib.lib()
    nbytes = L.mmk_extract_peaks_workspace_bytes(B, A, R, int(max_pts))
    ws = _workspace(nbytes, dev)
    pc = torch.empty(B, int(max_pts), 3, dtype=torch.float32, device=dev)
    cnt = torch.empty(B, dtype=torch.int32, device=dev)
    _lib.check(L.mmk_extract_peaks(_lib.ptr(m), B, A, R, float(res), _lib.ptr(az), _lib.ptr(tm), _lib.ptr(Tab),
                                   1 if diff else 0, float(steep_fact), int(max_pts), _lib.ptr(pc), _lib.ptr(cnt),
                                   _lib.ptr(ws), ws.numel(), _lib.stream_ptr(dev)))
    return pc, cnt


class _ExtractPeaks(torch.autograd.Function):

    @staticmethod
    def forward(ctx, thres_mask, m, res, az, tm, Tab, diff, steep_fact, max_pts):
        pc, cnt = _peaks_forward(m, res, az, tm, Tab, diff, steep_fact, max_pts)
        ctx.save_for_backward(m, az, Tab)
        ctx.args = (float(res), 1 if diff else 0, float(steep_fact), int(max_pts))
        ctx.like = (thres_mask.dtype, thres_mask.device)
        ctx.mark_non_differentiable(cnt)
        return pc, cnt

    @staticmethod
    def backward(ctx, gpc, _gcnt):
        m, az, Tab = ctx.saved_tensors
        res, diff, steep_fact, max_pts = ctx.args
        B, A, R = m.shape
        dev = m.device
        gpc = _lib.dev_f32(gpc, dev)
        L = _lib.lib()
        nbytes = L.mmk_extract_peaks_bwd_workspace_bytes(B, A, R, max_pts)
        ws = _workspace(nbytes, dev)
        gm = torch.empty_like(m)
        _lib.check(L.mmk_extract_peaks_bwd(_lib.ptr(m), B, A, R, res, _lib.ptr(az), _lib.ptr(Tab), diff, steep_fact, max_pts,
                                           _lib.ptr(gpc), _lib.ptr(gm), _lib.ptr(ws), ws.numel(), _lib.stream_ptr(dev)))
        return (gm.to(device=ctx.like[1], dtype=ctx.like[0]),) + (None,) * 8


def extract_pc_padded(thres_mask, res, azimuth_angles, azimuth_times, max_pts, T_ab=None, diff=True,
                      steep_fact=10.0):
    dev = _hip_device(thres_mask)
    m = _lib.dev_f32(thres_mask, dev)
    az = _lib.dev_f32(azimuth_angles, dev)
    tm = _lib.dev_f32(azimuth_times, dev) if azimuth_times is not None else None
    Tab = _lib.dev_f32(T_ab, dev).reshape(-1, 16) if T_ab is not None else None
    if torch.is_grad_enabled() and thres_mask.requires_grad:
        return _ExtractPeaks.apply(thres_mask, m, res, az, tm, Tab, diff, steep_fact, max_pts)
    return _peaks_forward(m, res, az, tm, Tab, diff, steep_fact, max_pts)


def extract_pc(thres_mask, res, azimuth_angles, azimuth_times, T_ab=None, diff=True, steep_fact=10.0):
    B, A, R = thres_mask.shape
    cap = (A * (R - 1) + 1) // 2
    cap = min(cap, 1 << 20)
    pc, cnt = extract_pc_padded(thres_mask, res, azimuth_angles, azimuth_times, cap, T_ab=T_ab, diff=diff,
                                steep_fact=steep_fact)
    counts = cnt.cpu().tolist()
    return [_back(pc[b, :min(n, cap)].clone(), thres_mask) for b, n in enumerate(counts)]


def _polar_to_cart_forward(x, az, W, radar_resolution, interpolate_crossover, fix_wobble):
    B, A, R = x.shape
    rg, ag = _device_grids(W, x.device)
    out = torch.empty(B, W, W, dtype=torch.float32, device=x.device)
    _lib.check(_lib.lib().mmk_polar_to_cart(_lib.ptr(x), _lib.ptr(az), _lib.ptr(rg), _lib.ptr(ag), B, A, R, W,
                                            float(radar_resolution), 1 if interpolate_crossover else 0,
                                            1 if fix_wobble else 0, _lib.ptr(out), _lib.stream_ptr(x.device)))
    return out


class _PolarToCart(torch.autograd.Function):

    @staticmethod
    def forward(ctx, fft_data, dev, az, W, radar_resolution, interpolate_crossover, fix_wobble):
        x = _lib.dev_f32(fft_data, dev)
        out = _polar_to_cart_forward(x, az, W, radar_resolution, interpolate_crossover, fix_wobble)
        ctx.save_for_backward(az)
        ctx.args = (tuple(x.shape), W, float(radar_resolution), 1 if interpolate_crossover else 0, 1 if fix_wobble else 0)
        ctx.like = (fft_data.dtype, fft_data.device)
        return _back(out, fft_data)

    @staticmethod
    def backward(ctx, g):
        (az,) = ctx.saved_tensors
        (B, A, R), W, radar_resolution, crossover, wobble = ctx.args
        dev = az.device
        g = _lib.dev_f32(g, dev)
        rg, ag = _device_grids(W, dev)
        L = _lib.lib()
        nbytes = int(L.mmk_polar_to_cart_bwd_ws_bytes(B, A, R, W))
        ws = _workspace(nbytes, dev)
        gx = torch.empty(B, A, R, dtype=torch.float32, device=dev)
        _lib.check(L.mmk_polar_to_cart_bwd(_lib.ptr(g), _lib.ptr(az), _lib.ptr(rg), _lib.ptr(ag), B, A, R, W, radar_resolution,
                                           crossover, wobble, _lib.ptr(gx), _lib.ptr(ws), ws.numel(), _lib.stream_ptr(dev)))
        return (gx.to(device=ctx.like[1], dtype=ctx.like[0]),) + (None,) * 6


def radar_polar_to_cartesian_diff(fft_data, azimuths, radar_resolution, cart_resolution=0.2384, cart_pixel_width=640,
                                  interpolate_crossover=True, fix_wobble=True):
    dev = _hip_device(fft_data)
    az = _lib.dev_f32(azimuths, dev)
    W = int(cart_pixel_width)
    if torch.is_grad_enabled() and fft_data.requires_grad:
        return _PolarToCart.apply(fft_data, dev, az, W, radar_resolution, interpolate_crossover, fix_wobble)
    x = _lib.dev_f32(fft_data, dev)
    return _back(_polar_to_cart_forward(x, az, W, radar_resolution, interpolate_crossover, fix_wobble), fft_data)


def _polar_to_cart_pair(img_a, img_b, azimuths, radar_resolution, cart_pixel_width=640):
    dev = _hip_device(img_a)
    a, b = _lib.dev_f32(img_a, dev), _lib.dev_f32(img_b, dev)
    az = _lib.dev_f32(azimuths, dev)
    assert a.shape == b.shape
    B, A, R = a.shape
    W = int(cart_pixel_width)
    rg, ag = _device_grids(W, dev)
    out_a = torch.empty(B, W, W, dtype=torch.float32, device=dev)
    out_b = torch.empty(B, W, W, dtype=torch.float32, device=dev)
    _lib.check(_lib.lib().mmk_polar_to_cart_pair(_lib.ptr(a), _lib.ptr(b), _lib.ptr(az), _lib.ptr(rg), _lib.ptr(ag), B, A, R, W,
                                                 float(radar_resolution), 1, 1, _lib.ptr(out_a), _lib.ptr(out_b),
                                                 _lib.stream_ptr(dev)))
    return _back(out_a, img_a), _back(out_b, img_b)


class _SampleWeights(torch.autograd.Function):

    @staticmethod
    def forward(ctx, mask, pc, cart_resolution, cart_pixel_width=640):
        B, H, W = mask.shape
        N, cols = pc.shape[1], pc.shape[2]
        out = torch.empty(B, N, dtype=torch.float32, device=mask.device)
        _lib.check(_lib.lib().mmk_sample_weights_fwd(_lib.ptr(mask, torch.float32, "mask"), _lib.ptr(pc), B, N, cols,
                                                     H, W, int(cart_pixel_width), float(cart_resolution), _lib.ptr(out),
# ... 75 lines not shown
```

### mm_masking_amd/train_icp_weights.py

```python
import time

import torch

from . import radar_utils as ru
from . import synthetic
from .icp_weight_policy import LearnICPWeightPolicy


def default_params(device=None):
    if device is None:
        device = torch.device("cuda" if torch.cuda.is_available() else "cpu")
    return {
        "device": device, "float_type": torch.float32, "gt_eye": True, "pos_std": 2.0, "rot_std": 0.6,
        "log_transform": False, "normalize": ["minmax"], "batch_size_train": 16, "batch_size_test": 32,
        "icp_type": "pt2pt", "learning_rate": 1e-4, "leaky": False, "dropout": 0.05, "batch_norm": False,
        "init_weights": True, "a_thresh": 1.0, "b_thresh": 0.09, "loss_icp_rot_weight": 1.0,
        "loss_icp_trans_weight": 1.0, "loss_fft_mask_weight": 0.0, "loss_map_pts_mask_weight": 1.0,
        "loss_cfar_mask_weight": 0.0, "num_pts_weight": 0.0, "optimizer": "adam", "icp_loss_only_iter": -1,
        "max_iter": 10, "network_input_type": "cartesian", "network_output_type": "cartesian",
        "binary_inference": False, "norm_weights": True, "fft_input": True, "cfar_input": False,
        "range_input": False, "num_epochs": 30,
    }


def loss_weights_from(params):
    return {"icp_rot": params["loss_icp_rot_weight"], "icp_trans": params["loss_icp_trans_weight"],
            "fft": params["loss_fft_mask_weight"], "mask_pts": params["loss_map_pts_mask_weight"],
            "cfar": params["loss_cfar_mask_weight"], "num_pts": params["num_pts_weight"]}


def prepare_batch(raw, params, max_loc_pts=5120, polar_res=0.0596):
    fft = raw["fft_polar"]
    az = raw["azimuths"]
    cfar = ru.cfar_mask(fft, polar_res, a_thresh=params["a_thresh"], b_thresh=params["b_thresh"], diff=False)
    pc, _ = ru.extract_pc_padded(cfar, polar_res, az, raw["az_times"], max_loc_pts, diff=False)
    if params.get("network_input_type", "cartesian") == "cartesian":
        fft_img, cfar_img = ru._polar_to_cart_pair(fft, cfar, az, polar_res)
    else:
        fft_img, cfar_img = fft, cfar
    loc_data = {"raw_pc": pc, "filtered_pc": pc, "fft_data": fft_img, "fft_cfar": cfar_img, "timestamp": 0}
    if params.get("mask_target") == "scan":
        loc_data.update({"fft_polar": fft, "azimuths": az, "az_times": raw["az_times"]})
    map_data = {"pc": raw["map_pc"], "timestamp": 0}
    T_data = {"T_ml_init": raw["T_init"], "T_ml_gt": raw["T_gt"]}
    return {"loc_data": loc_data, "map_data": map_data, "transforms": T_data}


_CONST_CACHE = {}


def _const(kind, device, dtype):
    key = (kind, device, dtype)
    t = _CONST_CACHE.get(key)
    if t is None:
        t = torch.zeros(1, dtype=dtype, device=device) if kind == "zero" else torch.eye(4, dtype=dtype, device=device)
        _CONST_CACHE[key] = t
    return t


_BCE_WS = {}


class _PoseLossFn(torch.autograd.Function):

    @staticmethod
    def forward(ctx, T_pred):
        from . import _lib
        T = T_pred.contiguous().float()
        out = torch.empty(2, dtype=torch.float32, device=T.device)
        _lib.check(_lib.lib().mmk_pose_loss_fwd(_lib.ptr(T), T.shape[0], _lib.ptr(out), _lib.stream_ptr(T.device)))
        ctx.save_for_backward(T)
        return out[0], out[1]

    @staticmethod
    def backward(ctx, g_rot, g_trans):
        from . import _lib
        (T,) = ctx.saved_tensors
        gT = torch.empty_like(T)
        gr = None if g_rot is None else g_rot.contiguous().float()
        gt = None if g_trans is None else g_trans.contiguous().float()
        _lib.check(_lib.lib().mmk_pose_loss_bwd(_lib.ptr(T), T.shape[0], _lib.ptr(gr), _lib.ptr(gt), _lib.ptr(gT), _lib.stream_ptr(T.device)))
        return gT


class _BceMeanFn(torch.autograd.Function):

    @staticmethod
    def forward(ctx, mask, target):
        from . import _lib
        L = _lib.lib()
        x, t = mask.contiguous().float(), target.contiguous().float()
        if x.shape != t.shape:
            raise _shape_mismatch(x, t)
        key = (x.device.index, torch.cuda.current_stream(x.device).cuda_stream)
        ws = _BCE_WS.get(key)
        if ws is None:
            ws = _BCE_WS[key] = torch.empty(int(L.mmk_bce_ws_bytes()), dtype=torch.uint8, device=x.device)
        out = torch.empty((), dtype=torch.float32, device=x.device)
        _lib.check(L.mmk_bce_mean_fwd(_lib.ptr(x), _lib.ptr(t), x.numel(), _lib.ptr(ws), ws.numel(), _lib.ptr(out), _lib.stream_ptr(x.device)))
        ctx.save_for_backward(x, t)
        return out

    @staticmethod
    def backward(ctx, g):
        from . import _lib
        x, t = ctx.saved_tensors
        gx = torch.empty_like(x)
        _lib.check(_lib.lib().mmk_bce_mean_bwd(_lib.ptr(x), _lib.ptr(t), x.numel(), _lib.ptr(g.contiguous().float()), _lib.ptr(gx),
                                               _lib.stream_ptr(x.device)))
        return gx, None


class _PoseLossGtFn(torch.autograd.Function):

    @staticmethod
    def forward(ctx, T_pred, T_gt):
        from . import _lib
        T = T_pred.contiguous().float()
# ... 383 lines not shown
```

Baseline: 3299 pairs/s.

## Fuse ICP solve into accumulate via last-block tickets and fuse CFAR with peak extraction

The ICP accumulate and backward point kernels now use a per-batch atomic ticket, so the last block to finish performs the normal-equation solve (or the backward pair/final step) in place. This removes the separate small solve and pair kernel launches for each iteration. Separately, the CFAR row kernel now writes per-row peak staging directly, so peak extraction skips the full mask re-scan. The cost is extra fences and atomics, a larger workspace for tickets and staging, and a serialized tail in the last block. Environment variables can turn either path off.

Measured after the change: 3280 pairs/s. No clear change (-0.6%).

```diff
diff --git a/include/mmk.h b/include/mmk.h
--- a/include/mmk.h
+++ b/include/mmk.h
@@ -142,6 +142,11 @@
                       const float *T_ab, int32_t diff, float steep_fact, int32_t max_pts,
                       float *out_pc, int32_t *out_count, void *workspace,
                       size_t workspace_bytes, void *stream);
+size_t mmk_cfar_peaks_workspace_bytes(int32_t B, int32_t A, int32_t R, int32_t max_pts);
+int mmk_cfar_peaks(const float *raw, int32_t B, int32_t A, int32_t R, int32_t w2, int32_t guard, int32_t mincol,
+                   int32_t maxcol, float a_thresh, float b_thresh, int32_t diff, float steep_fact, float res,
+                   const float *azimuths , const float *T_ab, int32_t max_pts, float *mask ,
+                   float *out_pc, int32_t *out_count, void *workspace, size_t workspace_bytes, void *stream);
 size_t mmk_extract_peaks_bwd_workspace_bytes(int32_t B, int32_t A, int32_t R, int32_t max_pts);
 int mmk_extract_peaks_bwd(const float *mask, int32_t B, int32_t A, int32_t R, float res, const float *azimuths ,
                           const float *T_ab, int32_t diff, float steep_fact, int32_t max_pts,
diff --git a/mm_masking_amd/_lib.py b/mm_masking_amd/_lib.py
--- a/mm_masking_amd/_lib.py
+++ b/mm_masking_amd/_lib.py
@@ -185,6 +185,9 @@
         "mmk_cfar_mask_bwd_p": (ctypes.c_int, [c_vp, c_vp, i32, i32, i32, i32, i32, i32, i32, c_vp, c_vp, i32, f32, c_vp, c_vp, c_vp,
                                                c_vp, sz, c_vp]),
         "mmk_extract_peaks_workspace_bytes": (sz, [i32, i32, i32, i32]),
+        "mmk_cfar_peaks_workspace_bytes": (sz, [i32, i32, i32, i32]),
+        "mmk_cfar_peaks": (ctypes.c_int, [c_vp, i32, i32, i32, i32, i32, i32, i32, f32, f32, i32, f32, f32, c_vp, c_vp, i32, c_vp, c_vp,
+                                          c_vp, c_vp, sz, c_vp]),
         "mmk_extract_peaks_bwd_workspace_bytes": (sz, [i32, i32, i32, i32]),
         "mmk_extract_peaks_bwd": (ctypes.c_int, [c_vp, i32, i32, i32, f32, c_vp, c_vp, i32, f32, i32, c_vp, c_vp, c_vp, sz, c_vp]),
         "mmk_extract_peaks": (ctypes.c_int, [c_vp, i32, i32, i32, f32, c_vp, c_vp, c_vp, i32, f32, i32, c_vp, c_vp,
diff --git a/mm_masking_amd/csrc/mmk_icp.hip b/mm_masking_amd/csrc/mmk_icp.hip
--- a/mm_masking_amd/csrc/mmk_icp.hip
+++ b/mm_masking_amd/csrc/mmk_icp.hip
@@ -3,6 +3,7 @@
 #include <stdlib.h>
 
 #include <algorithm>
+#include <type_traits>
 
 #include "mmk_common.h"
 
@@ -709,20 +710,51 @@
     t.w = (omega * t.keep) * rho;
 }
 
-template <int DIM, int TYPE>
+__device__ __forceinline__ bool pair_ticket_is_last(int32_t *ticket, int nblk, bool writer_wave)
+{
+    __shared__ int s_last;
+    if (writer_wave) {
+        __builtin_amdgcn_fence(__ATOMIC_RELEASE, "agent");
+        asm volatile("s_waitcnt vmcnt(0)" ::: "memory");
+    }
+    __syncthreads();
+    if (threadIdx.x == 0) {
+        const int t = __hip_atomic_fetch_add(ticket, 1, __ATOMIC_RELAXED, __HIP_MEMORY_SCOPE_AGENT);
+        const int last = (t == nblk - 1) ? 1 : 0;
+        if (last) __builtin_amdgcn_fence(__ATOMIC_ACQUIRE, "agent");
+        asm volatile("s_waitcnt vmcnt(0)" ::: "memory");
+        s_last = last;
+    }
+    __syncthreads();
+    return s_last != 0;
+}
+
+template <int DIM, int NT>
+__device__ __forceinline__ void icp_solve_step(const double *partials, int nblk, int b, const float *T_in, float *T_out,
+                                               double *delta_out, double *A_out, bool act, int32_t *active_out, float tol);
+
+template <int DIM, int TYPE, bool FUSED>
 __global__ __launch_bounds__(ACC_THREADS) void icp_accumulate_kernel(
     const float *__restrict__ src, const float *__restrict__ tgt, int tgt_cols,
     const float *__restrict__ weight, const float *__restrict__ Tk, const int32_t *__restrict__ active,
     const unsigned long long *__restrict__ packed, unsigned long long *__restrict__ packed_next,
     const int32_t *__restrict__ allzero, const int32_t *__restrict__ zrep, int nn_pts, int nn_nsb,
     int32_t *__restrict__ idx_out, int N, int M, int loss, float k,
-    float k2, float trim2, double *__restrict__ partials, int32_t *__restrict__ status)
+    float k2, float trim2, double *partials, int32_t *__restrict__ status, int32_t *__restrict__ tickets,
+    float *__restrict__ T_out, double *__restrict__ delta_out, double *__restrict__ A_out, int32_t *__restrict__ active_out,
+    float tol)
 {
     constexpr int P = PointTerms<DIM, TYPE>::P;
     constexpr int NR = PointTerms<DIM, TYPE>::NR;
     constexpr int NACC = nacc(DIM);
     const int b = blockIdx.y;
-    if (active != nullptr && active[b] == 0) return;
+    if (active != nullptr && active[b] == 0) {
+        if constexpr (FUSED) {
+            if (blockIdx.x == 0)
+                icp_solve_step<DIM, ACC_THREADS>(partials, (int)gridDim.x, b, Tk, T_out, delta_out, A_out, false, active_out, tol);
+        }
+        return;
+    }
     const int i = blockIdx.x * ACC_THREADS + threadIdx.x;
     double acc[NACC];
 #pragma unroll
@@ -777,6 +809,11 @@
 #pragma unroll
         for (int w = 0; w < ACC_THREADS / 64; ++w) v += red[w][threadIdx.x];
         partials[((size_t)b * gridDim.x + blockIdx.x) * NACC + threadIdx.x] = v;
+    }
+    if constexpr (FUSED) {
+        static_assert(NACC <= 64, "the partials are stored by wave 0");
+        if (!pair_ticket_is_last(tickets + b, (int)gridDim.x, wv == 0)) return;
+        icp_solve_step<DIM, ACC_THREADS>(partials, (int)gridDim.x, b, Tk, T_out, delta_out, A_out, true, active_out, tol);
     }
 }
 
@@ -876,27 +913,22 @@
     }
 }
 
-template <int DIM>
-__global__ __launch_bounds__(64) void icp_solve_kernel(const double *__restrict__ partials, int nblk,
-                                                       const float *__restrict__ T_in, float *__restrict__ T_out,
-                                                       double *__restrict__ delta_out, double *__restrict__ A_out,
-                                                       const int32_t *__restrict__ active_in,
-                                                       int32_t *__restrict__ active_out, float tol)
+template <int DIM, int NT>
+__device__ __forceinline__ void icp_solve_step(const double *partials, int nblk, int b, const float *T_in, float *T_out,
+                                               double *delta_out, double *A_out, bool act, int32_t *active_out, float tol)
 {
     constexpr int P = (DIM == 2) ? 3 : 6;
     constexpr int NACC = nacc(DIM);
-    const int b = blockIdx.x;
     const int lane = threadIdx.x;
     __shared__ double acc[NACC];
     __shared__ double stage[PART_ROWS * NACC];
-    const bool act = active_in[b] != 0;
     {
         double v = 0.0;
         if (act) {
             const double *base = partials + (size_t)b * nblk * NACC;
             for (int r0 = 0; r0 < nblk; r0 += PART_ROWS) {
                 const int nr = min(PART_ROWS, nblk - r0);
-                for (int e = lane; e < nr * NACC; e += 64) stage[e] = base[(size_t)r0 * NACC + e];
+                for (int e = lane; e < nr * NACC; e += NT) stage[e] = base[(size_t)r0 * NACC + e];
                 __syncthreads();
                 if (lane < NACC)
                     for (int q = 0; q < nr; ++q) v += stage[q * NACC + lane];
@@ -937,12 +969,24 @@
     active_out[b] = (sqrt(nrm) < (double)tol) ? 0 : 1;
 }
 
+template <int DIM>
+__global__ __launch_bounds__(64) void icp_solve_kernel(const double *__restrict__ partials, int nblk,
+                                                       const float *__restrict__ T_in, float *__restrict__ T_out,
+                                                       double *__restrict__ delta_out, double *__restrict__ A_out,
+                                                       const int32_t *__restrict__ active_in,
+                                                       int32_t *__restrict__ active_out, float tol)
+{
+    icp_solve_step<DIM, 64>(partials, nblk, blockIdx.x, T_in, T_out, delta_out, A_out, active_in[blockIdx.x] != 0, active_out, tol);
+}
+
 __global__ __launch_bounds__(256) void icp_init_kernel(unsigned long long *__restrict__ keys, size_t nkeys, int32_t *__restrict__ status,
                                                        int32_t *__restrict__ active0, const float *__restrict__ T_init,
-                                                       float *__restrict__ T0, int32_t *__restrict__ zrep, int B, int N)
+                                                       float *__restrict__ T0, int32_t *__restrict__ zrep, int B, int N,
+                                                       int32_t *__restrict__ tickets, size_t ntickets)
 {
     const size_t i0 = (size_t)blockIdx.x * blockDim.x + threadIdx.x, stride = (size_t)gridDim.x * blockDim.x;
     for (size_t i = i0; i < nkeys; i += stride) keys[i] = ~0ull;
+    for (size_t i = i0; i < ntickets; i += stride) tickets[i] = 0;
     if (i0 < 16) status[i0] = 0;
     if (i0 < (size_t)B) {
         active0[i0] = 1;
@@ -957,21 +1001,21 @@
     if (i < n) p[i] = v;
 }
 
-template <int DIM>
-__global__ __launch_bounds__(64) void icp_bwd_pair_kernel(
-    const double *__restrict__ Gdir_in, const double *__restrict__ pparts, int nparts,
-    const float *__restrict__ Tk, const double *__restrict__ delta, const double *__restrict__ Amat,
-    const int32_t *__restrict__ active, double *__restrict__ Gdir_out, double *__restrict__ lam_out)
+template <int DIM, int NT>
+__device__ __forceinline__ void icp_bwd_pair_step(const double *Gdir_in, const float *G32, const double *pparts, int nparts, int b,
+                                                  const float *Tk, const double *delta, const double *Amat, const int32_t *active,
+                                                  double *Gdir_out, double *lam_out)
 {
     constexpr int P = (DIM == 2) ? 3 : 6;
     constexpr int NP = npose(DIM);
-    const int b = blockIdx.x;
     const int lane = threadIdx.x;
+    const bool in64 = NT == 64 || lane < 64;
     __shared__ double G[16], Eb[16], X[16], M0[64], R0[64], R1[64];
     __shared__ double stage[PART_ROWS * NP];
 
     {
-        double v = (lane < 16) ? Gdir_in[(size_t)b * 16 + lane] : 0.0;
+        double v = 0.0;
+        if (lane < 16) v = (G32 != nullptr) ? (double)G32[(size_t)b * 16 + lane] : Gdir_in[(size_t)b * 16 + lane];
         const int r = lane >> 2, c = lane & 3;
         int slot = -1;
         if (lane < 16 && r < DIM && c < DIM) slot = r * DIM + c;
@@ -979,7 +1023,7 @@
         const double *base = pparts + (size_t)b * nparts * NP;
         for (int r0 = 0; r0 < nparts; r0 += PART_ROWS) {
             const int nr = min(PART_ROWS, nparts - r0);
-            for (int e = lane; e < nr * NP; e += 64) stage[e] = base[(size_t)r0 * NP + e];
+            for (int e = lane; e < nr * NP; e += NT) stage[e] = base[(size_t)r0 * NP + e];
             __syncthreads();
             if (slot >= 0)
                 for (int q = 0; q < nr; ++q) v += stage[q * NP + slot];
@@ -1018,8 +1062,8 @@
         X[lane] = x;
     }
     __syncthreads();
-    const int i8 = lane >> 3, j8 = lane & 7;
-    {
+    const int i8 = (lane >> 3) & 7, j8 = lane & 7;
+    if (in64) {
         double m = 0.0;
         const double sc = 1.0 / 64.0;
         if (i8 < 4 && j8 < 4) m = X[j8 * 4 + i8] * sc;
@@ -1031,18 +1075,22 @@
     __syncthreads();
     double *cur = R0, *nxt = R1;
     for (int n = 12; n >= 1; --n) {
-        double v = 0.0;
-#pragma unroll
-        for (int q = 0; q < 8; ++q) v += M0[i8 * 8 + q] * cur[q * 8 + j8];
-        nxt[lane] = ((i8 == j8) ? 1.0 : 0.0) + v / (double)n;
+        if (in64) {
+            double v = 0.0;
+#pragma unroll
+            for (int q = 0; q < 8; ++q) v += M0[i8 * 8 + q] * cur[q * 8 + j8];
+            nxt[lane] = ((i8 == j8) ? 1.0 : 0.0) + v / (double)n;
+        }
         __syncthreads();
         double *t = cur; cur = nxt; nxt = t;
     }
     for (int sq = 0; sq < 6; ++sq) {
-        double v = 0.0;
-#pragma unroll
-        for (int q = 0; q < 8; ++q) v += cur[i8 * 8 + q] * cur[q * 8 + j8];
-        nxt[lane] = v;
+        if (in64) {
+            double v = 0.0;
+#pragma unroll
+            for (int q = 0; q < 8; ++q) v += cur[i8 * 8 + q] * cur[q * 8 + j8];
+            nxt[lane] = v;
+        }
         __syncthreads();
         double *t = cur; cur = nxt; nxt = t;
     }
@@ -1073,16 +1121,42 @@
     }
 }
 
+template <int DIM>
+__global__ __launch_bounds__(64) void icp_bwd_pair_kernel(
+    const double *__restrict__ Gdir_in, const float *__restrict__ G32, const double *__restrict__ pparts, int nparts,
+    const float *__restrict__ Tk, const double *__restrict__ delta, const double *__restrict__ Amat,
+    const int32_t *__restrict__ active, double *__restrict__ Gdir_out, double *__restrict__ lam_out,
+    int32_t *__restrict__ tickets, int niter)
+{
+    if (tickets != nullptr)
+        for (int q = threadIdx.x; q < niter; q += 64) tickets[(size_t)q * gridDim.x + blockIdx.x] = 0;
+    icp_bwd_pair_step<DIM, 64>(Gdir_in, G32, pparts, nparts, blockIdx.x, Tk, delta, Amat, active, Gdir_out, lam_out);
+}
+
 __host__ __device__ constexpr int tgt_row_cols(int dim, int type) { return type == MMK_ICP_PT2PL ? 2 * dim : dim; }
 __host__ __device__ constexpr int tgt_acc_cols(int c) { return c <= 2 ? 2 : (c <= 4 ? 4 : 8); }
 
-template <int DIM, int TYPE, bool PTS>
+struct BwdTail {
+    int32_t *tickets;
+    int final;
+    const double *Gdir_in;
+    const float *Tk;
+    const double *delta, *Amat;
+    const int32_t *active;
+    double *Gdir_out, *lam_out;
+    float *grad_T_init;
+};
+
+template <int DIM>
+__device__ __forceinline__ void bwd_final_step(const double *Gdir, const double *pparts, int nparts, int b, float *out);
+
+template <int DIM, int TYPE, bool PTS, bool FUSED>
 __global__ __launch_bounds__(ACC_THREADS) void icp_bwd_point_kernel(
     const float *__restrict__ src, const float *__restrict__ tgt, int tgt_cols,
     const float *__restrict__ weight, const float *__restrict__ Tk, const int32_t *__restrict__ active,
     const int32_t *__restrict__ idx, const double *__restrict__ lam64, const double *__restrict__ delta64, int N,
-    int M, int loss, float k, float k2, float trim2, float *__restrict__ gw, double *__restrict__ pparts,
-    float *__restrict__ gsrc, float *__restrict__ rows, unsigned *__restrict__ pmax)
+    int M, int loss, float k, float k2, float trim2, float *__restrict__ gw, double *pparts,
+    float *__restrict__ gsrc, float *__restrict__ rows, unsigned *__restrict__ pmax, BwdTail tail)
 {
     constexpr int P = PointTerms<DIM, TYPE>::P;
     constexpr int NR = PointTerms<DIM, TYPE>::NR;
@@ -1249,6 +1323,15 @@
         for (int w = 0; w < ACC_THREADS / 64; ++w) v += red[w][threadIdx.x];
         pparts[((size_t)b * gridDim.x + blockIdx.x) * NP + threadIdx.x] = v;
     }
+    if constexpr (FUSED) {
+        static_assert(NP <= 64, "the parts are stored by wave 0");
+        if (!pair_ticket_is_last(tail.tickets + b, (int)gridDim.x, wv == 0)) return;
+        if (tail.final)
+            bwd_final_step<DIM>(tail.Gdir_in, pparts, (int)gridDim.x, b, tail.grad_T_init);
+        else
+            icp_bwd_pair_step<DIM, ACC_THREADS>(tail.Gdir_in, nullptr, pparts, (int)gridDim.x, b, tail.Tk, tail.delta, tail.Amat,
+                                                tail.active, tail.Gdir_out, tail.lam_out);
+    }
 }
 
 __global__ void f32_to_f64_kernel(const float *in, double *out, int n)
@@ -1258,12 +1341,11 @@
 }
 
 template <int DIM>
-__global__ void bwd_final_kernel(const double *__restrict__ Gdir, const double *__restrict__ pparts, int nparts,
-                                 float *__restrict__ out)
+__device__ __forceinline__ void bwd_final_step(const double *Gdir, const double *pparts, int nparts, int b, float *out)
 {
     constexpr int NP = npose(DIM);
     __shared__ double stage[PART_ROWS * NP];
-    const int b = blockIdx.x, lane = threadIdx.x;
+    const int lane = threadIdx.x;
     double v = (lane < 16) ? Gdir[(size_t)b * 16 + lane] : 0.0;
     const int r = lane >> 2, c = lane & 3;
     int slot = -1;
@@ -1279,6 +1361,13 @@
         __syncthreads();
     }
     if (lane < 16) out[(size_t)b * 16 + lane] = (float)v;
+}
+
+template <int DIM>
+__global__ void bwd_final_kernel(const double *__restrict__ Gdir, const double *__restrict__ pparts, int nparts,
+                                 float *__restrict__ out)
+{
+    bwd_final_step<DIM>(Gdir, pparts, nparts, blockIdx.x, out);
 }
 
 __device__ __forceinline__ double tgt_fixed_scale(unsigned mbits, int cnt_bits)
@@ -1410,6 +1499,12 @@
     return MMK_OK;
 }
 
+bool icp_chain_fused()
+{
+    const char *e = getenv("MMK_ICP_CHAIN");
+    return !(e != nullptr && e[0] == '0');
+}
+
 struct IcpWs {
     float *tgtp;
     unsigned long long *packed;
@@ -1420,6 +1515,7 @@
     double *partials;
     double *G0, *G1;
     double *lam;
+    int32_t *tickets;
     int32_t *status;
     int32_t *g_counts, *g_cursor, *g_starts;
     float4 *g_sorted;
@@ -1443,7 +1539,8 @@
     w.partials = ar.take<double>((size_t)p->B * nblk * 27);
     w.G0 = ar.take<double>((size_t)p->B * 16);
     w.G1 = ar.take<double>((size_t)p->B * 16);
-    w.lam = ar.take<double>((size_t)p->B * 6);
+    w.lam = ar.take<double>((size_t)2 * p->B * 6);
+    w.tickets = ar.take<int32_t>((size_t)p->max_iter * p->B);
     w.status = ar.take<int32_t>(16);
     w.g_counts = w.g_cursor = w.g_starts = nullptr;
     w.g_sorted = nullptr;
@@ -1492,6 +1589,7 @@
     const bool use_grid = p->nn_method == MMK_NN_GRID;
     const int nn_pts = NN_THREADS * pl.P;
     const bool dedup = !use_grid && pl.nsb <= 0xfff && B < (1 << 19);
+    const bool chain = icp_chain_fused();
     if (dedup) {
         hipLaunchKernelGGL(src_zero_scan_kernel, dim3(pl.nsb, B), dim3(NN_THREADS), 0, st, src, N, nn_pts, pl.nsb, w.allzero, w.zrep);
         MMK_LAUNCH_CHECK();
@@ -1530,14 +1628,24 @@
             int rc = launch_nn(DIM, src, w.tgtp, Tk, act, prev, dedup ? w.ulist : nullptr, w.ucnt, B, N, pl, keys, w.seed0, az, zr, w.tdec, st);
             if (rc != MMK_OK) return rc;
         }
-        hipLaunchKernelGGL((icp_accumulate_kernel<DIM, TYPE>), dim3(nblk, B), dim3(ACC_THREADS), 0, st, src, tgt,
-                           p->tgt_cols, weight, Tk, act, keys, keys_next, az, zr, nn_pts, pl.nsb, idx, N, M, p->loss, k, k2, trim2,
-                           w.partials, w.status);
-        MMK_LAUNCH_CHECK();
-        hipLaunchKernelGGL(icp_solve_kernel<DIM>, dim3(B), dim3(64), 0, st, w.partials, nblk, Tk,
-                           T_hist + (size_t)(it + 1) * B * 16, delta_hist + (size_t)it * B * 6,
-                           A_hist + (size_t)it * B * 36, act, active_hist + (size_t)(it + 1) * B, p->tolerance);
-        MMK_LAUNCH_CHECK();
+        float *T_next = T_hist + (size_t)(it + 1) * B * 16;
+        double *delta_it = delta_hist + (size_t)it * B * 6, *A_it = A_hist + (size_t)it * B * 36;
+        int32_t *act_next = active_hist + (size_t)(it + 1) * B;
+        if (chain) {
+            hipLaunchKernelGGL((icp_accumulate_kernel<DIM, TYPE, true>), dim3(nblk, B), dim3(ACC_THREADS), 0, st, src, tgt,
+                               p->tgt_cols, weight, Tk, act, keys, keys_next, az, zr, nn_pts, pl.nsb, idx, N, M, p->loss, k, k2, trim2,
+                               w.partials, w.status, w.tickets + (size_t)it * B, T_next, delta_it, A_it, act_next, p->tolerance);
+            MMK_LAUNCH_CHECK();
+        } else {
+            hipLaunchKernelGGL((icp_accumulate_kernel<DIM, TYPE, false>), dim3(nblk, B), dim3(ACC_THREADS), 0, st, src, tgt,
+                               p->tgt_cols, weight, Tk, act, keys, keys_next, az, zr, nn_pts, pl.nsb, idx, N, M, p->loss, k, k2, trim2,
+                               w.partials, w.status, static_cast<int32_t *>(nullptr), static_cast<float *>(nullptr),
+                               static_cast<double *>(nullptr), static_cast<double *>(nullptr), static_cast<int32_t *>(nullptr), 0.f);
+            MMK_LAUNCH_CHECK();
+            hipLaunchKernelGGL(icp_solve_kernel<DIM>, dim3(B), dim3(64), 0, st, w.partials, nblk, Tk, T_next, delta_it, A_it, act,
+                               act_next, p->tolerance);
+            MMK_LAUNCH_CHECK();
+        }
         k_done = it + 1;
         if (p->check_every > 0 && (k_done % p->check_every) == 0 && k_done < p->max_iter) {
             static thread_local int32_t host_act[1 << 16];
@@ -1576,33 +1684,64 @@
         MMK_CHECK_HIP(hipMemsetAsync(pw.acc, 0, sizeof(unsigned long long) * (size_t)B * M * L, st));
         MMK_CHECK_HIP(hipMemsetAsync(pw.pmax, 0, sizeof(unsigned) * (size_t)B, st));
     }
-    hipLaunchKernelGGL(f32_to_f64_kernel, dim3((B * 16 + 255) / 256), dim3(256), 0, st, grad_T, w.G0, B * 16);
-    MMK_LAUNCH_CHECK();
-    double *Gin = w.G0, *Gout = w.G1;
-    int nparts = 0;
-    for (int it = p->max_iter - 1; it >= 0; --it) {
+    auto launch_point = [&](int it, auto fused, const double *lam, const BwdTail &tail) {
+        constexpr bool F = decltype(fused)::value;
         const float *Tk = T_hist + (size_t)it * B * 16;
         const int32_t *act = active_hist + (size_t)it * B;
-        hipLaunchKernelGGL(icp_bwd_pair_kernel<DIM>, dim3(B), dim3(64), 0, st, Gin, w.partials, nparts, Tk,
-                           delta_hist + (size_t)it * B * 6, A_hist + (size_t)it * B * 36, act, Gout, w.lam);
+        if (gsrc || gtgt)
+            hipLaunchKernelGGL((icp_bwd_point_kernel<DIM, TYPE, true, F>), dim3(nblk, B), dim3(ACC_THREADS), 0, st, src, tgt,
+                               p->tgt_cols, weight, Tk, act, idx_hist + (size_t)it * B * N, lam,
+                               delta_hist + (size_t)it * B * 6, N, M, p->loss, k, k2, trim2, gw, w.partials, gsrc,
+                               gtgt ? pw.rows + (size_t)it * B * N * C : static_cast<float *>(nullptr), pw.pmax, tail);
+        else
+            hipLaunchKernelGGL((icp_bwd_point_kernel<DIM, TYPE, false, F>), dim3(nblk, B), dim3(ACC_THREADS), 0, st, src, tgt,
+                               p->tgt_cols, weight, Tk, act, idx_hist + (size_t)it * B * N, lam,
+                               delta_hist + (size_t)it * B * 6, N, M, p->loss, k, k2, trim2, gw, w.partials,
+                               static_cast<float *>(nullptr), static_cast<float *>(nullptr), static_cast<unsigned *>(nullptr), tail);
+    };
+    const BwdTail no_tail{};
+    double *Gin = w.G0, *Gout = w.G1;
+    if (icp_chain_fused()) {
+        const int last = p->max_iter - 1;
+        double *lam_cur = w.lam, *lam_nxt = w.lam + (size_t)B * 6;
+        hipLaunchKernelGGL(icp_bwd_pair_kernel<DIM>, dim3(B), dim3(64), 0, st, static_cast<const double *>(nullptr), grad_T, w.partials, 0,
+                           T_hist + (size_t)last * B * 16, delta_hist + (size_t)last * B * 6, A_hist + (size_t)last * B * 36,
+                           active_hist + (size_t)last * B, Gout, lam_cur, w.tickets, p->max_iter);
         MMK_LAUNCH_CHECK();
-        if (gsrc || gtgt)
-            hipLaunchKernelGGL((icp_bwd_point_kernel<DIM, TYPE, true>), dim3(nblk, B), dim3(ACC_THREADS), 0, st, src, tgt,
-                               p->tgt_cols, weight, Tk, act, idx_hist + (size_t)it * B * N, w.lam,
-                               delta_hist + (size_t)it * B * 6, N, M, p->loss, k, k2, trim2, gw, w.partials, gsrc,
-                               gtgt ? pw.rows + (size_t)it * B * N * C : static_cast<float *>(nullptr), pw.pmax);
-        else
-            hipLaunchKernelGGL((icp_bwd_point_kernel<DIM, TYPE, false>), dim3(nblk, B), dim3(ACC_THREADS), 0, st, src, tgt,
-                               p->tgt_cols, weight, Tk, act, idx_hist + (size_t)it * B * N, w.lam,
-                               delta_hist + (size_t)it * B * 6, N, M, p->loss, k, k2, trim2, gw, w.partials,
-                               static_cast<float *>(nullptr), static_cast<float *>(nullptr), static_cast<unsigned *>(nullptr));
+        for (int it = last; it >= 0; --it) {
+            double *t = Gin; Gin = Gout; Gout = t;
+            if (it > 0) {
+                const BwdTail tail{w.tickets + (size_t)it * B, 0, Gin, T_hist + (size_t)(it - 1) * B * 16,
+                                   delta_hist + (size_t)(it - 1) * B * 6, A_hist + (size_t)(it - 1) * B * 36,
+                                   active_hist + (size_t)(it - 1) * B, Gout, lam_nxt, nullptr};
+                launch_point(it, std::true_type{}, lam_cur, tail);
+            } else if (grad_T_init) {
+                const BwdTail tail{w.tickets, 1, Gin, nullptr, nullptr, nullptr, nullptr, nullptr, nullptr, grad_T_init};
+                launch_point(it, std::true_type{}, lam_cur, tail);
+            } else {
+                launch_point(it, std::false_type{}, lam_cur, no_tail);
+            }
+            MMK_LAUNCH_CHECK();
+            double *l = lam_cur; lam_cur = lam_nxt; lam_nxt = l;
+        }
+    } else {
+        hipLaunchKernelGGL(f32_to_f64_kernel, dim3((B * 16 + 255) / 256), dim3(256), 0, st, grad_T, w.G0, B * 16);
         MMK_LAUNCH_CHECK();
-        nparts = nblk;
-        double *t = Gin; Gin = Gout; Gout = t;
-    }
-    if (grad_T_init) {
-        hipLaunchKernelGGL(bwd_final_kernel<DIM>, dim3(B), dim3(64), 0, st, Gin, w.partials, nparts, grad_T_init);
-        MMK_LAUNCH_CHECK();
+        int nparts = 0;
+        for (int it = p->max_iter - 1; it >= 0; --it) {
+            hipLaunchKernelGGL(icp_bwd_pair_kernel<DIM>, dim3(B), dim3(64), 0, st, Gin, static_cast<const float *>(nullptr), w.partials,
+                               nparts, T_hist + (size_t)it * B * 16, delta_hist + (size_t)it * B * 6, A_hist + (size_t)it * B * 36,
+                               active_hist + (size_t)it * B, Gout, w.lam, static_cast<int32_t *>(nullptr), 0);
+            MMK_LAUNCH_CHECK();
+            launch_point(it, std::false_type{}, w.lam, no_tail);
+            MMK_LAUNCH_CHECK();
+            nparts = nblk;
+            double *t = Gin; Gin = Gout; Gout = t;
+        }
+        if (grad_T_init) {
+            hipLaunchKernelGGL(bwd_final_kernel<DIM>, dim3(B), dim3(64), 0, st, Gin, w.partials, nparts, grad_T_init);
+            MMK_LAUNCH_CHECK();
+        }
     }
     if (gtgt) {
         int cnt_bits = 0;
@@ -1747,7 +1886,7 @@
         const size_t nkeys = (size_t)2 * B * p->N;
         const unsigned blocks = (unsigned)std::min<size_t>(std::max<size_t>((nkeys + 255) / 256, (size_t)(B * 16 + 255) / 256), 2048);
         hipLaunchKernelGGL(icp_init_kernel, dim3(blocks), dim3(256), 0, st, w.packed, nkeys, w.status, active_hist, T_init, T_hist, w.zrep, B,
-                           p->N);
+                           p->N, w.tickets, (size_t)p->max_iter * B);
         MMK_LAUNCH_CHECK();
     }
     if (p->dim == 2 && p->icp_type == MMK_ICP_PT2PT)
@@ -1791,10 +1930,12 @@
                    const unsigned long long *keys, int32_t *idx, double *partials, int32_t *status, hipStream_t st)
 {
     const int nblk = (p->N + ACC_THREADS - 1) / ACC_THREADS;
-    hipLaunchKernelGGL((icp_accumulate_kernel<DIM, TYPE>), dim3(nblk, p->B), dim3(ACC_THREADS), 0, st, src, tgt, p->tgt_cols, weight,
+    hipLaunchKernelGGL((icp_accumulate_kernel<DIM, TYPE, false>), dim3(nblk, p->B), dim3(ACC_THREADS), 0, st, src, tgt, p->tgt_cols, weight,
                        T, static_cast<const int32_t *>(nullptr), keys, static_cast<unsigned long long *>(nullptr),
                        static_cast<const int32_t *>(nullptr), static_cast<const int32_t *>(nullptr), 1, 1, idx, p->N, p->M, p->loss,
-                       p->loss_k, p->loss_k * p->loss_k, p->trim_dist * p->trim_dist, partials, status);
+                       p->loss_k, p->loss_k * p->loss_k, p->trim_dist * p->trim_dist, partials, status,
+                       static_cast<int32_t *>(nullptr), static_cast<float *>(nullptr), static_cast<double *>(nullptr),
+                       static_cast<double *>(nullptr), static_cast<int32_t *>(nullptr), 0.f);
     MMK_LAUNCH_CHECK();
     return MMK_OK;
 }
diff --git a/mm_masking_amd/csrc/mmk_radar.hip b/mm_masking_amd/csrc/mmk_radar.hip
--- a/mm_masking_amd/csrc/mmk_radar.hip
+++ b/mm_masking_amd/csrc/mmk_radar.hip
@@ -1,4 +1,5 @@
 #include <math.h>
+#include <stdlib.h>
 
 #include "mmk_common.h"
 
@@ -29,6 +30,7 @@
     return base + inc - v;
 }
 
+template <int NTHR = RT>
 __device__ __forceinline__ int block_excl_scan_i(int v, int *sm, int *total)
 {
     const int lane = threadIdx.x & 63, wv = threadIdx.x >> 6;
@@ -42,7 +44,7 @@
     __syncthreads();
     int base = 0, tot = 0;
 #pragma unroll
-    for (int w = 0; w < RT / 64; ++w) {
+    for (int w = 0; w < NTHR / 64; ++w) {
         if (w < wv) base += sm[w];
         tot += sm[w];
     }
@@ -116,15 +118,19 @@
     for (int c = threadIdx.x; c < R; c += CFAR_T) mask[base + c] = cell(c);
 }
 
-template <int NPRE, class TH>
+__device__ __forceinline__ float peak_value(const float *__restrict__ mrow, int j, int R, float res, int diff, float steep);
+
+template <int NPRE, class TH, bool PEAKS>
 __global__ __launch_bounds__(CFAR_T) void cfar_mask_rows_kernel(const float *__restrict__ raw, int rows, int R, int w2, int guard,
                                                                 int mincol, int maxcol, TH thr, int diff,
-                                                                float steep, float *__restrict__ mask)
+                                                                float steep, float *__restrict__ mask, float res,
+                                                                int32_t *__restrict__ row_count, float *__restrict__ pstage)
 {
     extern __shared__ __attribute__((aligned(16))) unsigned char smem[];
     double *cs = reinterpret_cast<double *>(smem);
     float *row = reinterpret_cast<float *>(cs + (R + 1));
     __shared__ double wsum[CFAR_T / 64];
+    __shared__ int psum[CFAR_T / 64];
     float nx[NPRE];
     int r = blockIdx.x;
     if (r >= rows) return;
@@ -180,6 +186,24 @@
                 m = (x > th) ? 1.0f : 0.0f;
             }
             out[c] = m;
+            if (PEAKS) row[c] = m;
+        }
+        if (PEAKS) {
+            __syncthreads();
+            const int LP = (R - 1 + CFAR_T - 1) / CFAR_T;
+            const int j0 = min(R - 1, (int)threadIdx.x * LP), j1 = min(R - 1, j0 + LP);
+            int cnt = 0;
+            for (int j = j0; j < j1; ++j) cnt += (peak_value(row, j, R, res, diff, steep) != 0.0f) ? 1 : 0;
+            int tot;
+            int g = block_excl_scan_i<CFAR_T>(cnt, psum, &tot);
+            if (threadIdx.x == 0) row_count[r] = tot;
+            if (cnt != 0) {
+                float *ps = pstage + (size_t)r * (R - 1);
+                for (int j = j0; j < j1; ++j) {
+                    const float v = peak_value(row, j, R, res, diff, steep);
+                    if (v != 0.0f) ps[g++] = v;
+                }
+            }
         }
         if (rn >= rows) break;
         __syncthreads();
@@ -277,6 +301,23 @@
                 }
                 ++g;
             }
+        }
+    }
+}
+
+__global__ __launch_bounds__(RT) void peaks_gather_kernel(const float *__restrict__ pstage, int R, const int32_t *__restrict__ row_count,
+                                                          const int32_t *__restrict__ row_off, int cap, float *__restrict__ mval,
+                                                          int32_t *__restrict__ mrow_out)
+{
+    const int a = blockIdx.x, b = blockIdx.y, A = gridDim.x;
+    const int rowid = b * A + a;
+    const int n = row_count[rowid], off = row_off[rowid];
+    const float *ps = pstage + (size_t)rowid * (R - 1);
+    for (int t = threadIdx.x; t < n; t += RT) {
+        const int g = off + t;
+        if (g < cap) {
+            mval[(size_t)b * cap + g] = ps[t];
+            mrow_out[(size_t)b * cap + g] = a;
         }
     }
 }
@@ -1188,8 +1229,9 @@
             if (hipDeviceGetAttribute(&v, hipDeviceAttributeMultiprocessorCount, dev) == hipSuccess && v > 0) cus = v;
         }
         const int grid = std::min(rows, 4 * cus);
-        hipLaunchKernelGGL((cfar_mask_rows_kernel<8, CfarThVal>), dim3(grid), dim3(CFAR_T), smem, (hipStream_t)stream, raw, rows, R, w2,
-                           guard, mincol, maxcol, CfarThVal{a_thresh, b_thresh}, diff, steep_fact, mask);
+        hipLaunchKernelGGL((cfar_mask_rows_kernel<8, CfarThVal, false>), dim3(grid), dim3(CFAR_T), smem, (hipStream_t)stream, raw, rows, R, w2,
+                           guard, mincol, maxcol, CfarThVal{a_thresh, b_thresh}, diff, steep_fact, mask, 0.f,
+                           static_cast<int32_t *>(nullptr), static_cast<float *>(nullptr));
     } else {
         hipLaunchKernelGGL(cfar_mask_kernel<CfarThVal>, dim3(A, B), dim3(CFAR_T), smem, (hipStream_t)stream, raw, R, w2, guard, mincol,
                            maxcol, CfarThVal{a_thresh, b_thresh}, diff, steep_fact, mask);
@@ -1220,8 +1262,8 @@
             if (hipDeviceGetAttribute(&v, hipDeviceAttributeMultiprocessorCount, dev) == hipSuccess && v > 0) cus = v;
         }
         const int grid = std::min(rows, 4 * cus);
-        hipLaunchKernelGGL((cfar_mask_rows_kernel<8, CfarThPtr>), dim3(grid), dim3(CFAR_T), smem, (hipStream_t)stream, raw, rows, R, w2, guard,
-                           mincol, maxcol, thr, diff, steep_fact, mask);
+        hipLaunchKernelGGL((cfar_mask_rows_kernel<8, CfarThPtr, false>), dim3(grid), dim3(CFAR_T), smem, (hipStream_t)stream, raw, rows, R, w2, guard,
+                           mincol, maxcol, thr, diff, steep_fact, mask, 0.f, static_cast<int32_t *>(nullptr), static_cast<float *>(nullptr));
     } else {
         hipLaunchKernelGGL(cfar_mask_kernel<CfarThPtr>, dim3(A, B), dim3(CFAR_T), smem, (hipStream_t)stream, raw, R, w2, guard, mincol,
                            maxcol, thr, diff, steep_fact, mask);
@@ -1305,6 +1347,68 @@
     MMK_LAUNCH_CHECK();
     hipLaunchKernelGGL(peaks_pair_kernel, dim3((max_pts + 255) / 256, B), dim3(256), 0, st, w.mval, w.mrow, w.cap,
                        w.total, azimuths, T_ab, A, max_pts, out_pc, out_count);
+    MMK_LAUNCH_CHECK();
+    return MMK_OK;
+}
+
+namespace {
+inline bool cfar_rows_persistent(int R)
+{
+    const size_t smem = (size_t)(R + 1) * sizeof(double) + (size_t)R * sizeof(float);
+    return R <= 8 * CFAR_T && smem <= 40 * 1024;
+}
+inline size_t cfar_peaks_stage_off(int B, int A, int max_pts) { return carve_peaks(B, A, max_pts, nullptr, 0).bytes; }
+}
+
+extern "C" size_t mmk_cfar_peaks_workspace_bytes(int32_t B, int32_t A, int32_t R, int32_t max_pts)
+{
+    if (B < 1 || A < 1 || R < 2 || max_pts < 1) return 0;
+    size_t n = cfar_peaks_stage_off(B, A, max_pts);
+    if (cfar_rows_persistent(R)) n += mmk::align_up((size_t)B * A * (R - 1) * sizeof(float), 256);
+    return n;
+}
+
+extern "C" int mmk_cfar_peaks(const float *raw, int32_t B, int32_t A, int32_t R, int32_t w2, int32_t guard, int32_t mincol,
+                              int32_t maxcol, float a_thresh, float b_thresh, int32_t diff, float steep_fact, float res,
+                              const float *azimuths, const float *T_ab, int32_t max_pts, float *mask, float *out_pc,
+                              int32_t *out_count, void *workspace, size_t workspace_bytes, void *stream)
+{
+    MMK_REQUIRE(raw && mask && azimuths && out_pc && out_count, "mmk_cfar_peaks: NULL pointer");
+    MMK_REQUIRE(B >= 1 && A >= 1 && R >= 2 && max_pts >= 1, "mmk_cfar_peaks: bad shape");
+    MMK_REQUIRE(w2 >= 1 && guard >= 0, "mmk_cfar_peaks: bad window (w2=%d guard=%d)", w2, guard);
+    MMK_REQUIRE(mincol >= w2 + guard && maxcol <= R, "mmk_cfar_peaks: column range [%d,%d) outside the row", mincol, maxcol);
+    const size_t need = mmk_cfar_peaks_workspace_bytes(B, A, R, max_pts);
+    if (workspace == nullptr || need > workspace_bytes) {
+        mmk::set_error("mmk_cfar_peaks: workspace too small (%zu < %zu)", workspace_bytes, need);
+        return MMK_ERR_WORKSPACE;
+    }
+    const char *sw = getenv("MMK_CFAR_PEAKS");
+    if (!cfar_rows_persistent(R) || (sw != nullptr && sw[0] == '0')) {
+        const int rc = mmk_cfar_mask(raw, B, A, R, w2, guard, mincol, maxcol, a_thresh, b_thresh, diff, steep_fact, mask, stream);
+        if (rc != MMK_OK) return rc;
+        return mmk_extract_peaks(mask, B, A, R, res, azimuths, nullptr, T_ab, diff, steep_fact, max_pts, out_pc, out_count, workspace,
+                                 workspace_bytes, stream);
+    }
+    const PeakWs w = carve_peaks(B, A, max_pts, workspace, workspace_bytes);
+    float *pstage = reinterpret_cast<float *>(static_cast<unsigned char *>(workspace) + cfar_peaks_stage_off(B, A, max_pts));
+    hipStream_t st = (hipStream_t)stream;
+    const size_t smem = (size_t)(R + 1) * sizeof(double) + (size_t)R * sizeof(float);
+    const int rows = A * B;
+    int dev = 0, cus = 256;
+    if (hipGetDevice(&dev) == hipSuccess) {
+        int v = 0;
+        if (hipDeviceGetAttribute(&v, hipDeviceAttributeMultiprocessorCount, dev) == hipSuccess && v > 0) cus = v;
+    }
+    const int grid = std::min(rows, 4 * cus);
+    hipLaunchKernelGGL((cfar_mask_rows_kernel<8, CfarThVal, true>), dim3(grid), dim3(CFAR_T), smem, st, raw, rows, R, w2, guard, mincol,
+                       maxcol, CfarThVal{a_thresh, b_thresh}, diff, steep_fact, mask, res, w.row_count, pstage);
+    MMK_LAUNCH_CHECK();
+    hipLaunchKernelGGL(peaks_scan_kernel, dim3(B), dim3(RT), 0, st, w.row_count, A, w.row_off, w.total);
+    MMK_LAUNCH_CHECK();
+    hipLaunchKernelGGL(peaks_gather_kernel, dim3(A, B), dim3(RT), 0, st, pstage, R, w.row_count, w.row_off, w.cap, w.mval, w.mrow);
+    MMK_LAUNCH_CHECK();
+    hipLaunchKernelGGL(peaks_pair_kernel, dim3((max_pts + 255) / 256, B), dim3(256), 0, st, w.mval, w.mrow, w.cap, w.total, azimuths,
+                       T_ab, A, max_pts, out_pc, out_count);
     MMK_LAUNCH_CHECK();
     return MMK_OK;
 }
diff --git a/mm_masking_amd/radar_utils.py b/mm_masking_amd/radar_utils.py
--- a/mm_masking_amd/radar_utils.py
+++ b/mm_masking_amd/radar_utils.py
@@ -5,7 +5,7 @@
 
 from . import _lib
 
-__all__ = ["load_pc_from_file", "load_radar", "cfar_mask", "extract_pc", "extract_pc_padded", "extract_weights",
+__all__ = ["load_pc_from_file", "load_radar", "cfar_mask", "extract_pc", "extract_pc_padded", "cfar_mask_and_pc_padded", "extract_weights",
            "extract_bev_from_pts", "mean_peaks_parallel_fast", "pol_2_cart", "radar_polar_to_cartesian",
            "radar_polar_to_cartesian_diff", "radar_cartesian_to_polar", "mask_polar_scan", "point_to_cart_idx",
            "form_cart_range_angle_grid", "form_polar_range_grid"]
@@ -404,6 +404,31 @@
     return _peaks_forward(m, res, az, tm, Tab, diff, steep_fact, max_pts)
 
 
+def cfar_mask_and_pc_padded(raw_scans, res, azimuth_angles, azimuth_times, max_pts, T_ab=None, width=101, minr=2.0, maxr=80.0,
+                            guard=5, a_thresh=1.0, b_thresh=0.09, diff=False, steep_fact=10.0):
+    assert raw_scans.ndim == 3, "raw_scans must be 3D"
+    tensors = torch.is_tensor(a_thresh) or torch.is_tensor(b_thresh)
+    if tensors or (diff and torch.is_grad_enabled() and raw_scans.requires_grad):
+        mask = cfar_mask(raw_scans, res, width, minr, maxr, guard, a_thresh, b_thresh, diff, steep_fact)
+        pc, cnt = extract_pc_padded(mask, res, azimuth_angles, azimuth_times, max_pts, T_ab=T_ab, diff=diff, steep_fact=steep_fact)
+        return mask, pc, cnt
+    dev = _hip_device(raw_scans)
+    B, A, R = raw_scans.shape
+    w2, mincol, maxcol = cfar_cols(R, res, width, minr, maxr, guard)
+    x = _lib.dev_f32(raw_scans, dev)
+    az = _lib.dev_f32(azimuth_angles, dev)
+    Tab = _lib.dev_f32(T_ab, dev).reshape(-1, 16) if T_ab is not None else None
+    L = _lib.lib()
+    ws = _workspace(L.mmk_cfar_peaks_workspace_bytes(B, A, R, int(max_pts)), dev)
+    mask = torch.empty_like(x)
+    pc = torch.empty(B, int(max_pts), 3, dtype=torch.float32, device=dev)
+    cnt = torch.empty(B, dtype=torch.int32, device=dev)
+    _lib.check(L.mmk_cfar_peaks(_lib.ptr(x), B, A, R, w2, guard, mincol, max(mincol, maxcol), float(a_thresh), float(b_thresh),
+                                1 if diff else 0, float(steep_fact), float(res), _lib.ptr(az), _lib.ptr(Tab), int(max_pts),
+                                _lib.ptr(mask), _lib.ptr(pc), _lib.ptr(cnt), _lib.ptr(ws), ws.numel(), _lib.stream_ptr(dev)))
+    return _back(mask, raw_scans), pc, cnt
+
+
 def extract_pc(thres_mask, res, azimuth_angles, azimuth_times, T_ab=None, diff=True, steep_fact=10.0):
     B, A, R = thres_mask.shape
     cap = (A * (R - 1) + 1) // 2
diff --git a/mm_masking_amd/train_icp_weights.py b/mm_masking_amd/train_icp_weights.py
--- a/mm_masking_amd/train_icp_weights.py
+++ b/mm_masking_amd/train_icp_weights.py
@@ -32,8 +32,8 @@
 def prepare_batch(raw, params, max_loc_pts=5120, polar_res=0.0596):
     fft = raw["fft_polar"]
     az = raw["azimuths"]
-    cfar = ru.cfar_mask(fft, polar_res, a_thresh=params["a_thresh"], b_thresh=params["b_thresh"], diff=False)
-    pc, _ = ru.extract_pc_padded(cfar, polar_res, az, raw["az_times"], max_loc_pts, diff=False)
+    cfar, pc, _ = ru.cfar_mask_and_pc_padded(fft, polar_res, az, raw["az_times"], max_loc_pts, a_thresh=params["a_thresh"],
+                                             b_thresh=params["b_thresh"], diff=False)
     if params.get("network_input_type", "cartesian") == "cartesian":
         fft_img, cfar_img = ru._polar_to_cart_pair(fft, cfar, az, polar_res)
     else:
```
